# NilanEkanayake/TiTok-Video

Measured on AMD Instinct MI355X. Metric: video clips/sec encode+decode (whole node), higher is better.
Workload: dtype bf16

## Files before the change

### include/titok_hip.h

```cpp
#ifndef TITOK_HIP_H
#define TITOK_HIP_H

#include <stdint.h>

#ifdef __cplusplus
extern "C" {
#endif

#define TTV_OK 0
#define TTV_ERR_INVALID 1
#define TTV_ERR_LAUNCH 2
#define TTV_ERR_UNSUPPORTED 3

#define TTV_BF16 0
#define TTV_F32 1

#define TTV_ENCODER 0
#define TTV_DECODER 1

#define TTV_MAX_FSQ 8
#define TTV_MAX_TOKEN 64
#define TTV_MAX_CLIPS_PER_LAUNCH 64

const char* ttv_error_string(void);
// ... 18 lines not shown
int64_t ttv_vq_workspace_bytes(int rows);
int ttv_vq_l2_argmin(const void* z, int dtype, int ldz, const void* codebook, int ldc, const float* cnorm, int rows, int N, int C,
                     int32_t* indices, float* best_dist, void* workspace, int64_t workspace_bytes, void* stream);
int ttv_vq_lookup(const void* codebook, int dtype, int ldc, const int32_t* indices, int rows, int C, void* codes, int ldo, void* stream);
int ttv_vq_lookup_backward(const void* dcodes, int dtype, int ld, const int32_t* indices, int rows, int C, float* dcodebook, int ldc, void* stream);

int ttv_quant_rows_fp8(const void* in, int dtype, int ld_in, const float* gain, float eps, void* out, int ld_out, float* scales, int rows,
                       int width, void* stream);
int ttv_linear_fp8(const void* xq, int ldx, const float* x_scale, const void* wq, int ldw, const float* w_scale, void* y, int ldy, int M, int N,
                   int K, int epilogue, const float* rope_cs, int d_model, int gqa_dim, void* stream);

int ttv_split3_pack(const float* w, int ldw, void* out, int ldo, int rows, int K, void* stream);
int ttv_linear_split3(const float* x, int ldx, const void* w_image, int ldw, const float* bias, float* y, int ldy, int M, int N, int K, void* stream);

int64_t ttv_mx_scale_bytes_per_row(int width);
int ttv_quant_mx_fp8(const void* in, int dtype, int ld_in, void* out, int ld_out, void* mx, float* row_scales, int rows, int width, void* stream);
int ttv_linear_fp8_mx(const void* xq, int ldx, const void* x_mx, const float* x_row_scale, const void* wq, int ldw, const void* w_mx,
                      const float* w_row_scale, void* y, int ldy, int M, int N, int K, int epilogue, const float* rope_cs, int d_model,
                      int gqa_dim, const void* resid, int ldr, float alpha, void* stream);


int ttv_rmsnorm(const void* in, int in_dtype, int ld_in, const int32_t* src_rows, void* out, int out_dtype, int ld_out,
                const int32_t* dst_rows, const float* gain, int rows, int width, float eps, void* stream);

int ttv_rope_apply(void* x, int dtype, int ld, int rows, int heads, const float* rope_cs, void* stream);

int ttv_linear(const void* x, int ldx, const void* w, int ldw, const void* bias, const float* add_scalar, void* y, int ldy,
               int M, int N, int K, int dtype, void* stream);

int ttv_linear_qkv_rope(const void* x, int ldx, const void* w, int ldw, void* y, int ldy, int M, int d_model, int gqa_dim,
                        const float* rope_cs, int dtype, void* stream);
int ttv_linear_geglu(const void* x, int ldx, const void* w, int ldw, void* y, int ldy, int M, int I, int K, int dtype,
                     void* stream);
int ttv_linear_residual(const void* x, int ldx, const void* w, int ldw, const void* resid, int ldr, float alpha, void* y,
                        int ldy, int y_f32, int M, int N, int K, int dtype, void* stream);

int ttv_linear_residual_norm(const void* x, int ldx, const void* w, int ldw, const void* resid, int ldr, float alpha,
                             const float* gain, float eps, void* y, int ldy, int M, int N, int K, int dtype, void* stream);

int64_t ttv_mlp_pack_bytes(int inner, int next_qkv_rows);
int ttv_mlp_pack(const void* w12_folded, const void* w3, const void* out_proj, const void* next_qkv_folded, int next_qkv_rows, int inner,
                 int width, int dtype, void* mlp_packed, void* stream);
int ttv_mlp_fused(const void* x, int ldx, const void* mlp_packed, int inner, void* y, int ldy, const float* post_gain, float alpha,
                  float eps, int M, int width, int dtype, void* stream);
typedef struct ttv_next_qkv {
  void* qkv; int32_t ld;
  const float* rope_cs;
  int32_t rows;
  int32_t rope_q_end, rope_k_begin, rope_k_end;
} ttv_next_qkv;
int ttv_layer_tail_fused(const void* ao, int ldao, const float* attn_post_gain, float attn_alpha, const void* x, int ldx,
                         const void* mlp_packed, int inner, void* y, int ldy, const float* ffd_post_gain, float ffd_alpha, float eps,
                         int M, int width, int dtype, const ttv_next_qkv* next, void* stream);

int ttv_fill_const_rows(void* x, int dtype, int ld, const int32_t* rows_map, int rows, int width, const float* mask_token,
                        const float* gain, float eps, void* stream);
int ttv_decoder_embed(const void* codes, int token_size, const void* w, const void* bias, const float* mask_token, const float* gain,
                      void* x, int dtype, int ld, const int32_t* rows_map, int rows, int width, float eps, void* stream);

#define TTV_ATTN_GATE 1
#define TTV_ATTN_PAIRED 2
#define TTV_ATTN_QSCALED 4
#define TTV_ATTN_ALLFULL 8
#define TTV_ATTN_PIPE 16
#define TTV_ATTN_SPLIT3 32
#define TTV_ATTN_SPLIT_OUT 64
#define TTV_ATTN_SPLIT_IN 128
int ttv_attention(const void* qkvg, int ld, void* out, int ldo, const int32_t* cu_seqlens, const int32_t* qblocks,
                  int n_qblocks, int q_heads, int kv_heads, int head_dim, int flags, int dtype, void* stream);
int ttv_attention64(const void* qkvg, int ld, void* out, int ldo, const int32_t* cu_seqlens, const int32_t* items, int n_items,
                    int q_heads, int kv_heads, int head_dim, int flags, int dtype, void* stream);

int ttv_patch_gather(const void* const* clips, const int32_t* clip_desc, int clip0, int n_clips, int patch_t, int patch_h,
                     int patch_w, int channels, void* patches, int ld, int dtype, int max_patches_per_clip, void* stream);
int ttv_patch_scatter(const void* patches, int ld, const int32_t* clip_desc, int clip0, int n_clips, int patch_t, int patch_h,
                      int patch_w, int channels, void* const* clips, int dtype, int max_patches_per_clip, void* stream);

typedef struct ttv_tower_dims {
  int32_t kind;
  int32_t dtype;
  int32_t width;
  int32_t layers;
  int32_t q_heads, kv_heads, head_dim;
  int32_t inner;
  int32_t patch_t, patch_h, patch_w;
  int32_t pix_channels;
  int32_t token_size;
  float eps;
  float alpha;
} ttv_tower_dims;

typedef struct ttv_layer_weights {
  const float* pre_ln;
  const void* to_qkv;
  const void* out_proj;
  const float* ffd_norm;
  const void* w12;
  const void* w3;
  const float* attn_post_ln;
  const float* ffd_post_ln;
  const void* to_qkv_pn;
  const void* w12_pn;
  const void* mlp_pack;
  int32_t mlp_pack_qkv_rows;
  int32_t qkv_q_prescaled;
  const void* to_qkv_qs;
// ... 214 lines not shown
  const void* pool_proj_w; const void* pool_proj_b;
  const float* pool_norm2_w; const float* pool_norm2_b;
  const void* pool_fc1_w; const void* pool_fc1_b;
  const void* pool_fc2_w; const void* pool_fc2_b;
} ttv_vjepa_weights;

int ttv_jedi_preprocess(void* const* clips, const int32_t* dims, int n_clips, int dtype, void* out, void* stream);
int64_t ttv_vjepa_workspace_bytes(int n);
int ttv_vjepa_features(const ttv_vjepa_weights* w, const void* x, int n, float* feats, int finetuned, void* workspace,
                       int64_t workspace_bytes, void* stream);

#define TTV_VJEPA_EPI_STORE 0
#define TTV_VJEPA_EPI_GELU 1
#define TTV_VJEPA_EPI_RESID 2
int ttv_vjepa_layernorm(const float* x, int ldx, int rows, int width, const float* w1, const float* b1, float eps1, const float* w2,
                        const float* b2, float eps2, float* y32, int ld32, void* y16, int ld16, void* stream);
int ttv_vjepa_linear(const void* x, int ldx, const void* w, int ldw, const void* bias, int M, int N, int K, int epilogue,
                     const float* resid, int ldr, int resid_rows, void* y, int ldy, void* stream);
int ttv_vjepa_pool_attention(const void* q, const void* kv, int n, int rows, void* out, void* stream);

#define TTV_KC_ATTENTION 1
#define TTV_KC_GEMM_QKV 2
#define TTV_KC_GEMM_GEGLU 3
#define TTV_KC_GEMM_RESID 4
#define TTV_KC_GEMM_STORE 5
#define TTV_KC_RMSNORM 6
#define TTV_KC_PATCH 7
#define TTV_KC_ROWS 8
int ttv_prof_begin(int kernel_class, int max_records);
enum {
  TTV_DBG_NO_STORES = 1,
  TTV_DBG_K256_NO_PANEL_DMA = 2,
  TTV_DBG_MLP_NO_WEIGHT_DMA = 2,
  TTV_DBG_K256_NO_TILE_RELOAD = 4,
  TTV_DBG_MLP_NO_GEGLU = 4,
  TTV_DBG_K256_NO_EPILOGUE_MATH = 8,
  TTV_DBG_MLP_TILES8 = 8,
  TTV_DBG_MLP_NO_P2 = 16,
  TTV_DBG_MLP_PAIRS_ONLY = 32,
  TTV_DBG_MLP_TILES4 = 64,
  TTV_DBG_GEMM_TILE160 = 128,
  TTV_DBG_GEMM_TILE128 = 256,
  TTV_DBG_GEMM_T256 = 512,
  TTV_DBG_MLP_TILES9 = 512,
  TTV_DBG_GEMM_NO_T256 = 1024,
  TTV_DBG_MX_UNFUSED_QUANT = 2048,
  TTV_DBG_SPLIT3_NO_IMAGES = 4096,
  TTV_DBG_SPLIT3_NO_DMA = 8192,
  TTV_DBG_K256_GENERAL = 16384,
  TTV_DBG_QKV256_OFF = 32768,
  TTV_DBG_QKV256_WS = 131072,
  TTV_DBG_ENC_ALL_ROWS = 524288,
  TTV_DBG_ATTN_NO_SWP = 1048576,
  TTV_DBG_DEC_ALL_BLOCKS = 2097152
};
int ttv_debug_set(int flags);
int ttv_debug_stamps(void* device_buffer);
int ttv_prof_end(double* total_ms, int* count);

#ifdef __cplusplus
}
#endif
#endif
```

### titok_video_amd/_lib.py

```python
from __future__ import annotations

import ctypes as C
import os
import threading

import torch

from . import switches

TTV_BF16, TTV_F32 = 0, 1
TTV_ENCODER, TTV_DECODER = 0, 1
TTV_MAX_FSQ = 8
TTV_MAX_TOKEN = 64
TTV_MAX_CLIPS_PER_LAUNCH = 64
TTV_DISC_HEAD_GENERATOR, TTV_DISC_HEAD_DISCRIMINATOR = 0, 1

DBG_NO_STORES = 1
DBG_K256_NO_PANEL_DMA = 2
DBG_MLP_NO_WEIGHT_DMA = 2
DBG_K256_NO_TILE_RELOAD = 4
DBG_MLP_NO_GEGLU = 4
DBG_K256_NO_EPILOGUE_MATH = 8
DBG_MLP_TILES8 = 8
DBG_MLP_NO_P2 = 16
DBG_MLP_PAIRS_ONLY = 32
DBG_MLP_TILES4 = 64
DBG_GEMM_TILE160 = 128
DBG_GEMM_TILE128 = 256
DBG_GEMM_T256 = 512
DBG_MLP_TILES9 = 512
DBG_GEMM_NO_T256 = 1024
DBG_MX_UNFUSED_QUANT = 2048
DBG_SPLIT3_NO_IMAGES = 4096
DBG_SPLIT3_NO_DMA = 8192
DBG_K256_GENERAL = 16384
DBG_QKV256_OFF = 32768
DBG_QKV256_WS = 131072
DBG_ENC_ALL_ROWS = 524288
DBG_ATTN_NO_SWP = 1048576
DBG_DEC_ALL_BLOCKS = 2097152

_HERE = os.path.dirname(os.path.abspath(__file__))
LIB_PATH = switches.text("TTV_LIB_PATH") or os.path.join(_HERE, "libtitok_hip.so")

i32, i64, f32, vp = C.c_int32, C.c_int64, C.c_float, C.c_void_p


class FsqParams(C.Structure):
    _fields_ = [("n", i32), ("levels", i32 * TTV_MAX_FSQ), ("basis", i32 * TTV_MAX_FSQ),
                ("half_l", f32 * TTV_MAX_FSQ), ("offset", f32 * TTV_MAX_FSQ), ("shift", f32 * TTV_MAX_FSQ),
                ("half_width", f32 * TTV_MAX_FSQ)]


class TowerDims(C.Structure):
    _fields_ = [("kind", i32), ("dtype", i32), ("width", i32), ("layers", i32), ("q_heads", i32), ("kv_heads", i32),
                ("head_dim", i32), ("inner", i32), ("patch_t", i32), ("patch_h", i32), ("patch_w", i32),
                ("pix_channels", i32), ("token_size", i32), ("eps", f32), ("alpha", f32)]


class NextQkv(C.Structure):
    _fields_ = [("qkv", vp), ("ld", i32), ("rope_cs", vp), ("rows", i32), ("rope_q_end", i32), ("rope_k_begin", i32), ("rope_k_end", i32)]


class LayerWeights(C.Structure):
    _fields_ = [("pre_ln", vp), ("to_qkv", vp), ("out_proj", vp), ("ffd_norm", vp), ("w12", vp), ("w3", vp),
                ("attn_post_ln", vp), ("ffd_post_ln", vp), ("to_qkv_pn", vp), ("w12_pn", vp), ("mlp_pack", vp), ("mlp_pack_qkv_rows", i32), ("qkv_q_prescaled", i32),
                ("to_qkv_qs", vp), ("to_qkv_f8", vp), ("to_qkv_f8_scale", vp), ("w12_f8", vp), ("w12_f8_scale", vp),
                ("to_qkv_mx", vp), ("w12_mx", vp), ("out_proj_f8", vp), ("out_proj_f8_scale", vp), ("out_proj_mx", vp),
                ("w3_f8", vp), ("w3_f8_scale", vp), ("w3_mx", vp)]


class TowerWeights(C.Structure):
    _fields_ = [("proj_in_w", vp), ("proj_in_b", vp), ("mask_token", vp), ("ln_pre_t", vp), ("ln_pre_p", vp),
                ("ln_post", vp), ("proj_out_w", vp), ("proj_out_b", vp), ("layers", C.POINTER(LayerWeights)), ("proj_out_pn", vp),
                ("f32_split3", i32)]


class Batch(C.Structure):
    _fields_ = [("n_clips", i32), ("total_rows", i32), ("sum_tokens", i32), ("sum_patches", i32),
                ("max_patches_per_clip", i32), ("n_qblocks", i32), ("cu_seqlens", vp), ("latent_rows", vp),
                ("patch_rows", vp), ("clip_desc", vp), ("qblocks", vp), ("rope_cs", vp), ("blocks64", vp), ("row_seq", vp),
                ("n_blocks64", i32), ("qblocks_paired", i32), ("qblocks_all_full", i32), ("items64", vp), ("n_items64", i32),
                ("rope_ids", vp), ("rope_base", vp), ("qblocks_latent", vp), ("n_qblocks_latent", i32), ("qblocks_patch", vp),
                ("n_qblocks_patch", i32)]


class LayerWeightsT(C.Structure):
    _fields_ = [("to_qkv_t", vp), ("out_proj_t", vp), ("w12_t", vp), ("w3_t", vp)]


class TowerWeightsT(C.Structure):
    _fields_ = [("proj_in_t", vp), ("proj_out_t", vp), ("layers", C.POINTER(LayerWeightsT))]

# ... 21 lines not shown


TTV_VJEPA_WIDTH = 1024
TTV_VJEPA_TOKENS = 1568
TTV_VJEPA_PATCH_K = 1536
TTV_VJEPA_EPI_STORE, TTV_VJEPA_EPI_GELU, TTV_VJEPA_EPI_RESID = 0, 1, 2


class VjepaLayer(C.Structure):
    _fields_ = [("norm1_w", vp), ("norm1_b", vp), ("qkv_w", vp), ("qkv_b", vp), ("proj_w", vp), ("proj_b", vp), ("norm2_w", vp),
                ("norm2_b", vp), ("fc1_w", vp), ("fc1_b", vp), ("fc2_w", vp), ("fc2_b", vp)]


class VjepaWeights(C.Structure):
    _fields_ = [("width", i32), ("heads", i32), ("depth", i32), ("patch_w", vp), ("patch_b", vp), ("pos_embed", vp),
                ("layers", C.POINTER(VjepaLayer)), ("norm_w", vp), ("norm_b", vp), ("query_tokens", vp), ("pool_q", vp),
                ("pool_norm1_w", vp), ("pool_norm1_b", vp), ("pool_kv_w", vp), ("pool_kv_b", vp), ("pool_proj_w", vp),
                ("pool_proj_b", vp), ("pool_norm2_w", vp), ("pool_norm2_b", vp), ("pool_fc1_w", vp), ("pool_fc1_b", vp),
                ("pool_fc2_w", vp), ("pool_fc2_b", vp)]


_lib = None
_lock = threading.Lock()

SYMBOLS = {
    "ttv_error_string": (C.c_char_p, []),
    "ttv_version": (C.c_int, []),
    "ttv_fsq_forward": (C.c_int, [C.POINTER(FsqParams), vp, C.c_int, C.c_int, vp, C.c_int, vp, vp, vp]),
    "ttv_fsq_indices_to_codes": (C.c_int, [C.POINTER(FsqParams), vp, C.c_int, vp, C.c_int, vp]),
    "ttv_vq_codebook_norms": (C.c_int, [vp, C.c_int, C.c_int, C.c_int, C.c_int, vp, vp]),
    "ttv_vq_workspace_bytes": (C.c_int64, [C.c_int]),
    "ttv_vq_l2_argmin": (C.c_int, [vp, C.c_int, C.c_int, vp, C.c_int, vp, C.c_int, C.c_int, C.c_int, vp, vp, vp, C.c_int64, vp]),
    "ttv_vq_lookup": (C.c_int, [vp, C.c_int, C.c_int, vp, C.c_int, C.c_int, vp, C.c_int, vp]),
    "ttv_vq_lookup_backward": (C.c_int, [vp, C.c_int, C.c_int, vp, C.c_int, C.c_int, vp, C.c_int, vp]),
    "ttv_quant_rows_fp8": (C.c_int, [vp, C.c_int, C.c_int, vp, f32, vp, C.c_int, vp, C.c_int, C.c_int, vp]),
    "ttv_linear_fp8": (C.c_int, [vp, C.c_int, vp, vp, C.c_int, vp, vp, C.c_int, C.c_int, C.c_int, C.c_int, C.c_int, vp, C.c_int, C.c_int, vp]),
    "ttv_split3_pack": (C.c_int, [vp, C.c_int, vp, C.c_int, C.c_int, C.c_int, vp]),
    "ttv_linear_split3": (C.c_int, [vp, C.c_int, vp, C.c_int, vp, vp, C.c_int, C.c_int, C.c_int, C.c_int, vp]),
    "ttv_mx_scale_bytes_per_row": (C.c_int64, [C.c_int]),
    "ttv_quant_mx_fp8": (C.c_int, [vp, C.c_int, C.c_int, vp, C.c_int, vp, vp, C.c_int, C.c_int, vp]),
    "ttv_linear_fp8_mx": (C.c_int, [vp, C.c_int, vp, vp, vp, C.c_int, vp, vp, vp, C.c_int, C.c_int, C.c_int, C.c_int, C.c_int, vp, C.c_int, C.c_int,
                                    vp, C.c_int, f32, vp]),
    "ttv_rmsnorm": (C.c_int, [vp, C.c_int, C.c_int, vp, vp, C.c_int, C.c_int, vp, vp, C.c_int, C.c_int, f32, vp]),
    "ttv_rope_apply": (C.c_int, [vp, C.c_int, C.c_int, C.c_int, C.c_int, vp, vp]),
    "ttv_linear": (C.c_int, [vp, C.c_int, vp, C.c_int, vp, vp, vp, C.c_int, C.c_int, C.c_int, C.c_int, C.c_int, vp]),
    "ttv_linear_qkv_rope": (C.c_int, [vp, C.c_int, vp, C.c_int, vp, C.c_int, C.c_int, C.c_int, C.c_int, vp, C.c_int, vp]),
    "ttv_linear_geglu": (C.c_int, [vp, C.c_int, vp, C.c_int, vp, C.c_int, C.c_int, C.c_int, C.c_int, C.c_int, vp]),
    "ttv_linear_residual": (C.c_int, [vp, C.c_int, vp, C.c_int, vp, C.c_int, f32, vp, C.c_int, C.c_int, C.c_int, C.c_int,
                                      C.c_int, C.c_int, vp]),
    "ttv_linear_residual_norm": (C.c_int, [vp, C.c_int, vp, C.c_int, vp, C.c_int, f32, vp, f32, vp, C.c_int, C.c_int, C.c_int,
                                           C.c_int, C.c_int, vp]),
    "ttv_mlp_pack_bytes": (C.c_int64, [C.c_int, C.c_int]),
    "ttv_mlp_pack": (C.c_int, [vp, vp, vp, vp, C.c_int, C.c_int, C.c_int, C.c_int, vp, vp]),
    "ttv_layer_tail_fused": (C.c_int, [vp, C.c_int, vp, f32, vp, C.c_int, vp, C.c_int, vp, C.c_int, vp, f32, f32, C.c_int, C.c_int,
                                       C.c_int, vp, vp]),
    "ttv_mlp_fused": (C.c_int, [vp, C.c_int, vp, C.c_int, vp, C.c_int, vp, f32, f32, C.c_int, C.c_int, C.c_int, vp]),
    "ttv_fill_const_rows": (C.c_int, [vp, C.c_int, C.c_int, vp, C.c_int, C.c_int, vp, vp, f32, vp]),
    "ttv_decoder_embed": (C.c_int, [vp, C.c_int, vp, vp, vp, vp, vp, C.c_int, C.c_int, vp, C.c_int, C.c_int, f32, vp]),
    "ttv_attention": (C.c_int, [vp, C.c_int, vp, C.c_int, vp, vp, C.c_int, C.c_int, C.c_int, C.c_int, C.c_int, C.c_int, vp]),
    "ttv_attention64": (C.c_int, [vp, C.c_int, vp, C.c_int, vp, vp, C.c_int, C.c_int, C.c_int, C.c_int, C.c_int, C.c_int, vp]),
    "ttv_patch_gather": (C.c_int, [C.POINTER(vp), vp, C.c_int, C.c_int, C.c_int, C.c_int, C.c_int, C.c_int, vp, C.c_int,
                                   C.c_int, C.c_int, vp]),
    "ttv_patch_scatter": (C.c_int, [vp, C.c_int, vp, C.c_int, C.c_int, C.c_int, C.c_int, C.c_int, C.c_int, C.POINTER(vp),
                                    C.c_int, C.c_int, vp]),
    "ttv_tower_workspace_bytes": (i64, [C.POINTER(TowerDims), C.POINTER(Batch)]),
    "ttv_encoder_forward": (C.c_int, [C.POINTER(TowerDims), C.POINTER(TowerWeights), C.POINTER(Batch), C.POINTER(vp),
                                      C.POINTER(FsqParams), vp, vp, vp, vp, vp, i64, vp]),
    "ttv_decoder_forward": (C.c_int, [C.POINTER(TowerDims), C.POINTER(TowerWeights), C.POINTER(Batch), vp, C.POINTER(vp),
                                      vp, i64, vp]),
    "ttv_tower_tape_bytes": (i64, [C.POINTER(TowerDims), C.POINTER(Batch)]),
    "ttv_tower_bwd_workspace_bytes": (i64, [C.POINTER(TowerDims), C.POINTER(Batch)]),
    "ttv_encoder_forward_train": (C.c_int, [C.POINTER(TowerDims), C.POINTER(TowerWeights), C.POINTER(Batch), C.POINTER(vp), vp, vp,
                                            i64, vp]),
    "ttv_encoder_backward": (C.c_int, [C.POINTER(TowerDims), C.POINTER(TowerWeights), C.POINTER(TowerWeightsT), C.POINTER(Batch), vp,
                                       vp, C.POINTER(TowerGrads), C.POINTER(vp), vp, i64, vp]),
    "ttv_decoder_forward_train": (C.c_int, [C.POINTER(TowerDims), C.POINTER(TowerWeights), C.POINTER(Batch), vp, C.POINTER(vp), vp,
                                            i64, vp, i64, vp]),
    "ttv_decoder_backward": (C.c_int, [C.POINTER(TowerDims), C.POINTER(TowerWeights), C.POINTER(TowerWeightsT), C.POINTER(Batch), vp,
                                       C.POINTER(vp), vp, C.POINTER(TowerGrads), vp, vp, i64, vp]),
    "ttv_fsq_backward": (C.c_int, [C.POINTER(FsqParams), vp, vp, C.c_int, vp, C.c_int, vp]),
    "ttv_rmsnorm_backward_chain": (C.c_int, [vp, C.c_int, vp, C.c_int, vp, vp, vp, C.c_int, vp, C.c_int, vp, vp, C.c_float, vp, C.c_int,
                                              C.c_int, C.c_int, C.c_float, C.c_int, vp]),
    "ttv_opt_grad_sumsq": (C.c_int, [vp, vp, C.c_int, C.c_int, vp, vp]),
    "ttv_opt_adamw_step": (C.c_int, [vp, vp, C.c_int, C.c_int, vp, C.c_int] + [C.c_float] * 8 + [vp, vp]),
    "ttv_opt_param_norms": (C.c_int, [vp, vp, C.c_int, C.c_int, vp, vp, vp]),
    "ttv_linear_wgrad_workspace_bytes": (C.c_int64, [C.c_int, C.c_int, C.c_int]),
    "ttv_linear_wgrad": (C.c_int, [vp, C.c_int, vp, C.c_int, vp, C.c_int, C.c_int, C.c_int, C.c_int, C.c_int, vp, C.c_int64, vp]),
    "ttv_rmsnorm_backward": (C.c_int, [vp, C.c_int, vp, C.c_int, vp, vp, C.c_int, vp, C.c_int, C.c_int, f32, C.c_int, vp]),
    "ttv_attention_backward": (C.c_int, [vp, C.c_int, vp, C.c_int, vp, C.c_int, vp, vp, vp, vp, C.c_int, vp, vp, C.c_int, vp, C.c_int,
                                         C.c_int, C.c_int, C.c_int, vp, vp]),
    "ttv_attention_lse": (C.c_int, [vp, C.c_int, vp, C.c_int, vp, vp, C.c_int, C.c_int, C.c_int, C.c_int, C.c_int, C.c_int, vp, vp]),
    "ttv_codebook_histogram": (C.c_int, [vp, C.c_int, vp, C.c_int, vp]),
    "ttv_rope_table_build": (C.c_int, [vp, vp, C.c_int, C.c_int, vp, vp, vp, vp, C.c_int, vp]),
    "ttv_l1_loss": (C.c_int, [vp, vp, vp, vp, C.c_int, C.c_int, vp, vp]),
    "ttv_clip_from_u8": (C.c_int, [vp, C.c_int, C.c_int, C.c_int, vp, C.c_int, vp]),
    "ttv_clip_resample_u8": (C.c_int, [vp, vp, vp, C.c_int, C.c_int, vp]),
    "ttv_recon_panels_u8": (C.c_int, [vp, vp, vp, C.c_int, C.c_int, vp, vp]),
    "ttv_sq_err_accumulate": (C.c_int, [vp, vp, vp, C.c_int, C.c_int, C.c_int, vp, vp]),
    "ttv_ssim_workspace_bytes": (C.c_int64, [vp, C.c_int]),
    "ttv_ssim_accumulate": (C.c_int, [vp, vp, vp, C.c_int, C.c_int, C.c_int, vp, vp, C.c_int64, vp]),
    "ttv_lpips_tape_bytes": (C.c_int64, [C.c_int, C.c_int, C.c_int, C.c_int]),
    "ttv_lpips_workspace_bytes": (C.c_int64, [C.c_int, C.c_int, C.c_int, C.c_int]),
    "ttv_lpips_forward": (C.c_int, [C.POINTER(LpipsWeights), vp, vp, C.c_int, C.c_int, C.c_int, C.c_int, vp, vp, vp, vp, C.c_int64, vp]),
    "ttv_lpips_backward": (C.c_int, [C.POINTER(LpipsWeights), vp, C.c_int, C.c_int, C.c_int, C.c_int, vp, vp, vp, vp, C.c_int64, vp]),
    "ttv_lpips_conv_workspace_bytes": (C.c_int64, [C.c_int] * 6),
    "ttv_lpips_conv3x3": (C.c_int, [vp, C.c_int, C.c_int, C.c_int, C.c_int, C.c_int, vp, vp, C.c_int, vp, vp, C.c_int, vp, C.c_int64, vp]),
# ... 77 lines not shown
```

### titok_video_amd/csrc/ttv_api.hip

```cpp
#include <stdarg.h>
#include <stdio.h>
#include <stdlib.h>
#include <string.h>

#include "ttv_common.h"
#include "ttv_kernels.h"

static thread_local char g_err[512] = "";

void ttv_set_error(const char* fmt, ...) {
  va_list ap;
  va_start(ap, fmt);
  vsnprintf(g_err, sizeof(g_err), fmt, ap);
  va_end(ap);
}

int g_ttv_prof_class = 0;
bool ttv_sw_enc_latent_last() { static const bool v = ttv_env_flag("TTV_ENC_LATENT_LAST", true); return v; }
bool ttv_sw_keel_f32sum() { static const bool v = ttv_env_flag("TTV_KEEL_F32SUM", false); return v; }
bool ttv_sw_fused_patch() { static const bool v = ttv_env_flag("TTV_FUSED_PATCH", true); return v; }
bool ttv_sw_attn_pipe() { static const bool v = ttv_env_flag("TTV_ATTN_PIPE", false); return v; }
float ttv_sw_attn_thr() { static const float v = ttv_env_float("TTV_ATTN_THR", 8.0f); return v; }
thread_local int g_ttv_debug = 0;
long long* g_ttv_stamps = nullptr;
static hipEvent_t* g_prof_start = nullptr;
static hipEvent_t* g_prof_stop = nullptr;
static int g_prof_cap = 0, g_prof_n = 0;

TtvProfScope::TtvProfScope(int cls, hipStream_t stream) : slot(-1), s(stream) {
  if (g_ttv_prof_class != 0 && cls == g_ttv_prof_class && g_prof_n < g_prof_cap) {
    slot = g_prof_n++;
    (void)hipEventRecord(g_prof_start[slot], s);
  }
}
TtvProfScope::~TtvProfScope() {
  if (slot >= 0) (void)hipEventRecord(g_prof_stop[slot], s);
}

#define TTV_TRY(expr)            \
  do {                           \
    int rc__ = (expr);           \
    if (rc__ != TTV_OK) return rc__; \
  } while (0)

static inline int esize(int dtype) { return dtype == TTV_BF16 ? 2 : 4; }
static inline int64_t align_up(int64_t v) { return (v + 255) & ~(int64_t)255; }

struct TowerWs {
  char *x, *xn, *qkv, *ao, *h, *pa, *pb;
  char *xl, *aol;
  char *f8, *f8mx;
  float* y32;
  float* rstd;
  int64_t total;
};

static TowerWs carve(const ttv_tower_dims* d, const ttv_batch* b, char* base) {
  const int64_t e = esize(d->dtype);
  const int64_t L = b->total_rows, P = b->sum_patches;
  const int64_t g = (int64_t)d->kv_heads * d->head_dim;
  const int64_t pd = (int64_t)d->pix_channels * d->patch_t * d->patch_h * d->patch_w;
  int64_t off = 0;
  TowerWs w;
  auto take = [&](int64_t bytes) { char* p = base ? base + off : nullptr; off += align_up(bytes); return p; };
  w.x = take(L * d->width * e);
  w.xn = take(L * d->width * e);
  w.qkv = take(L * (2 * d->width + 2 * g) * e);
  w.ao = take(L * d->width * e);
  w.y32 = (float*)take(L * d->width * 4);
  w.h = take(L * d->inner * e);
  w.pa = take(P * pd * e);
  w.pb = take(P * d->width * e);
  w.rstd = (float*)take(L * 4);
  w.xl = take((int64_t)b->sum_tokens * d->width * e);
  w.aol = take((int64_t)b->sum_tokens * d->width * e);
  w.f8 = w.f8mx = nullptr;
  if (d->dtype == TTV_BF16 && d->width != 256 && d->width % 128 == 0) {
    const int64_t wide = d->width > d->inner ? d->width : d->inner;
    w.f8 = take(L * wide);
    w.f8mx = take(L * (wide / 128 + 4) * 4);
  }
  w.total = off;
  return w;
}

static int check_dims(const ttv_tower_dims* d, const ttv_batch* b) {
  TTV_CHECK_ARG(d && b, "null dims/batch");
  TTV_CHECK_ARG(d->dtype == TTV_BF16 || d->dtype == TTV_F32, "bad dtype %d", d->dtype);
  TTV_CHECK_ARG(d->head_dim == 64 && d->width == d->q_heads * 64, "width must be q_heads*64");
  TTV_CHECK_ARG(d->width % 64 == 0 && d->width <= 1024, "width %d unsupported", d->width);
  TTV_CHECK_ARG(d->inner % 32 == 0, "GEGLU inner dim must be a multiple of 32");
  TTV_CHECK_ARG(d->token_size >= 1 && d->token_size <= TTV_MAX_TOKEN, "token_size out of range");
  TTV_CHECK_ARG(((int64_t)d->pix_channels * d->patch_t * d->patch_h * d->patch_w) % 8 == 0, "patch vector length must be a multiple of 8");
  TTV_CHECK_ARG(b->n_clips > 0 && b->total_rows == b->sum_tokens + b->sum_patches, "inconsistent batch");
  return TTV_OK;
}

static int run_layer_mx(const ttv_tower_dims* d, const ttv_layer_weights& lw, const ttv_batch* b, const TowerWs& ws, int i, bool& rstd_valid,
                        bool& xq_valid, bool attn_pipe, hipStream_t s) {
  const int L = b->total_rows, dm = d->width, g = d->kv_heads * d->head_dim, dt = d->dtype, nq = 2 * dm + 2 * g, I = d->inner;
  static const bool fused_env = ttv_env_flag("TTV_MX_FUSED_QUANT", true);
  const bool fused_q = fused_env && !(g_ttv_debug & TTV_DBG_MX_UNFUSED_QUANT);
  if (!rstd_valid) TTV_TRY(ttvk_row_rstd(ws.x, dt, dm, ws.rstd, L, dm, d->eps, s));
  if (!xq_valid) TTV_TRY(ttvk_quant_mx_fp8(ws.x, dt, dm, ws.f8, dm, ws.f8mx, nullptr, L, dm, s));
  xq_valid = false;
  GemmArgs a = {};
  a.dtype = dt; a.x = ws.f8; a.ldx = dm; a.w = lw.to_qkv_f8; a.ldw = dm; a.M = L; a.N = nq; a.K = dm; a.y = ws.qkv; a.ldy = nq;
  a.rope_cs = b->rope_cs; a.rope_q_end = dm; a.rope_k_begin = 2 * dm; a.rope_k_end = 2 * dm + g;
  TTV_TRY(ttvk_gemm_fp8(EPI_QKV_ROPE, a, ws.rstd, lw.to_qkv_f8_scale, s, ws.f8mx, lw.to_qkv_mx));
  const bool q_scaled = lw.qkv_q_prescaled != 0;
  if (fused_q && q_scaled && !b->qblocks_paired && !attn_pipe && d->head_dim == 64) {
    TTV_TRY(ttvk_attention_mxout(ws.qkv, nq, ws.f8, ws.f8mx, (int)ttvk_mx_scale_ld(dm), b->cu_seqlens, b->qblocks, b->n_qblocks, d->q_heads,
                                 d->kv_heads, s));
  } else {
    TTV_TRY(ttvk_attention(ws.qkv, nq, ws.ao, dm, b->cu_seqlens, b->qblocks, b->n_qblocks, d->q_heads, d->kv_heads, d->head_dim,
                           TTV_ATTN_GATE | (b->qblocks_paired ? TTV_ATTN_PAIRED : 0) | (q_scaled ? TTV_ATTN_QSCALED : 0) |
                               ((b->qblocks_all_full && attn_pipe) ? TTV_ATTN_ALLFULL : 0) | (attn_pipe ? TTV_ATTN_PIPE : 0), dt, s));
    TTV_TRY(ttvk_quant_mx_fp8(ws.ao, dt, dm, ws.f8, dm, ws.f8mx, nullptr, L, dm, s));
  }
  GemmArgs o = {};
  o.dtype = dt; o.x = ws.f8; o.ldx = dm; o.w = lw.out_proj_f8; o.ldw = dm; o.M = L; o.N = dm; o.K = dm; o.resid = ws.x; o.ldr = dm;
  o.alpha = i == 0 ? 1.f : d->alpha; o.y = ws.x; o.ldy = dm;
  TTV_TRY(ttvk_gemm_fp8(EPI_RESID_T, o, nullptr, lw.out_proj_f8_scale, s, ws.f8mx, lw.out_proj_mx));
  if (i > 0) {
    TTV_TRY(ttvk_rmsnorm(ws.x, dt, dm, nullptr, ws.x, dt, dm, nullptr, lw.attn_post_ln, L, dm, d->eps, s, ws.rstd, fused_q ? ws.f8 : nullptr,
                         fused_q ? ws.f8mx : nullptr));
    if (!fused_q) TTV_TRY(ttvk_quant_mx_fp8(ws.x, dt, dm, ws.f8, dm, ws.f8mx, nullptr, L, dm, s));
  } else {
    TTV_TRY(ttvk_row_rstd(ws.x, dt, dm, ws.rstd, L, dm, d->eps, s));
    TTV_TRY(ttvk_quant_mx_fp8(ws.x, dt, dm, ws.f8, dm, ws.f8mx, nullptr, L, dm, s));
  }
  GemmArgs f = {};
  f.dtype = dt; f.x = ws.f8; f.ldx = dm; f.w = lw.w12_f8; f.ldw = dm; f.M = L; f.N = I; f.K = dm; f.y = ws.h; f.ldy = I;
  char* const hq = ws.h;
  char* const hq_mx = ws.xn;
  const bool h_fused = fused_q && (int64_t)ttvk_mx_scale_ld(I) <= (int64_t)dm * 2;
  if (h_fused) { f.yq = hq; f.yq_mx = hq_mx; }
  TTV_TRY(ttvk_gemm_fp8(EPI_GEGLU, f, ws.rstd, lw.w12_f8_scale, s, ws.f8mx, lw.w12_mx));
  GemmArgs f3 = {};
  if (h_fused) {
    f3.x = hq;
  } else {
    TTV_TRY(ttvk_quant_mx_fp8(ws.h, dt, I, ws.f8, I, ws.f8mx, nullptr, L, I, s));
    f3.x = ws.f8;
  }
  f3.dtype = dt; f3.ldx = I; f3.w = lw.w3_f8; f3.ldw = I; f3.M = L; f3.N = dm; f3.K = I; f3.resid = ws.x; f3.ldr = dm;
  f3.alpha = i == 0 ? 1.f : d->alpha; f3.y = ws.x; f3.ldy = dm;
  TTV_TRY(ttvk_gemm_fp8(EPI_RESID_T, f3, nullptr, lw.w3_f8_scale, s, h_fused ? hq_mx : ws.f8mx, lw.w3_mx));
  rstd_valid = false;
  if (i > 0) {
    TTV_TRY(ttvk_rmsnorm(ws.x, dt, dm, nullptr, ws.x, dt, dm, nullptr, lw.ffd_post_ln, L, dm, d->eps, s, ws.rstd, fused_q ? ws.f8 : nullptr,
                         fused_q ? ws.f8mx : nullptr));
    rstd_valid = true;
    xq_valid = fused_q;
  }
  return TTV_OK;
}

static bool rows_f8(int dt, int dm, const void* img, const void* row_scale, const void* mx, const void* folded) {
  return dt == TTV_BF16 && img && row_scale && !mx && dm % 128 == 0 && !(dm == 256 && folded);
}

struct LayerCtx {
  const ttv_tower_dims* d; const ttv_batch* b; const TowerWs& ws; hipStream_t s;
  int split3, s3img;
  bool gen_ok;
};

struct PreNormW { const float* gain; const void *w, *w_pn, *w_f8; const float* w_f8_scale; bool f8; };

static int prenorm_proj(const LayerCtx& c, GemmEpilogue epi, const char* x, int rows, const PreNormW& p, int N, char* y, int y_image,
                        bool rstd_valid) {
  const ttv_tower_dims* d = c.d;
  const TowerWs& ws = c.ws;
  const int dm = d->width, dt = d->dtype;
  GemmArgs a = {};
  a.dtype = dt; a.ldx = dm; a.ldw = dm; a.M = rows; a.N = N; a.K = dm; a.y = y; a.ldy = N;
  if (epi == EPI_QKV_ROPE) {
    a.rope_cs = c.b->rope_cs; a.rope_q_end = dm; a.rope_k_begin = 2 * dm; a.rope_k_end = 2 * dm + d->kv_heads * d->head_dim;
  }
  if (p.f8) {
    float* const f8_scales = reinterpret_cast<float*>(ws.xn + (((size_t)c.b->total_rows * dm + 255) & ~(size_t)255));
    TTV_TRY(ttvk_quant_rows_fp8(x, dt, dm, p.gain, d->eps, ws.xn, dm, f8_scales, rows, dm, c.s));
    a.x = ws.xn; a.w = p.w_f8;
    return ttvk_gemm_fp8(epi, a, f8_scales, p.w_f8_scale, c.s);
  }
  const bool fold256 = dt == TTV_BF16 && dm == 256 && p.w_pn;
  const bool fold_gen = c.gen_ok && p.w_pn;
  const bool fold = fold256 || fold_gen;
  if (fold_gen && !rstd_valid) TTV_TRY(ttvk_row_rstd(x, dt, dm, ws.rstd, rows, dm, d->eps, c.s));
  if (!fold) TTV_TRY(ttvk_rmsnorm(x, dt, dm, nullptr, ws.xn, dt, dm, nullptr, p.gain, rows, dm, d->eps, c.s, nullptr, nullptr, nullptr, c.s3img));
  a.split3 = c.split3; a.x_image = c.s3img && !fold; a.y_image = y_image;
  a.prenorm = fold256; a.eps = d->eps;
  a.row_scale = fold_gen ? ws.rstd : nullptr;
  a.x = fold ? x : ws.xn; a.w = fold ? p.w_pn : p.w;
  if (epi == EPI_QKV_ROPE) { a.rope_ids = c.b->rope_ids; a.rope_base = c.b->rope_ids ? c.b->rope_base : nullptr; }
  return ttvk_gemm(epi, a, c.s);
}

static int keel_tail(const LayerCtx& c, GemmArgs o, int layer, const float* post_gain, char* cx, bool want_rstd, bool& rstd_valid) {
  const ttv_tower_dims* d = c.d;
  const int dm = d->width, dt = d->dtype;
  static const bool keel_f32sum = ttv_sw_keel_f32sum();
  o.alpha = layer == 0 ? 1.f : d->alpha; o.y = cx; o.ldy = dm;
  if (layer == 0) return ttvk_gemm(EPI_RESID_T, o, c.s);
  if (ttvk_gemm_supports_resid_norm(dt, dm, o.K)) {
    o.norm_gain = post_gain; o.eps = d->eps;
    return ttvk_gemm(EPI_RESID_NORM, o, c.s);
  }
  float* const next_rstd = want_rstd ? c.ws.rstd : nullptr;
  if (dt == TTV_BF16 && !keel_f32sum) {
    TTV_TRY(ttvk_gemm(EPI_RESID_T, o, c.s));
    TTV_TRY(ttvk_rmsnorm(cx, dt, dm, nullptr, cx, dt, dm, nullptr, post_gain, o.M, dm, d->eps, c.s, next_rstd));
  } else {
    o.y = c.ws.y32;
    TTV_TRY(ttvk_gemm(EPI_RESID_F32, o, c.s));
    TTV_TRY(ttvk_rmsnorm(c.ws.y32, TTV_F32, dm, nullptr, cx, dt, dm, nullptr, post_gain, o.M, dm, d->eps, c.s, next_rstd));
  }
  rstd_valid = want_rstd;
  return TTV_OK;
}

static int run_layers(const ttv_tower_dims* d, const ttv_tower_weights* w, const ttv_batch* b, const TowerWs& ws, hipStream_t s) {
  const int L = b->total_rows, dm = d->width, g = d->kv_heads * d->head_dim, dt = d->dtype;
  const int split3 = (dt == TTV_F32 && w->f32_split3) ? 1 : 0;
  const bool gen_ok = (dt == TTV_BF16 && dm != 256) || split3;
  static const bool s3img_env = ttv_env_flag("TTV_SPLIT3_IMAGES", true);
  const int s3img = (split3 && s3img_env && !(g_ttv_debug & TTV_DBG_SPLIT3_NO_IMAGES)) ? 1 : 0;
  const int nq = 2 * dm + 2 * g;
  bool qkv_ready = false;
  bool rstd_valid = false;
  bool xq_valid = false;
  static const bool attn_pipe = ttv_sw_attn_pipe();
  static const bool lat_env = ttv_sw_enc_latent_last();
  const bool lat_last = lat_env && !(g_ttv_debug & TTV_DBG_ENC_ALL_ROWS) && d->kind == TTV_ENCODER && b->qblocks_latent && b->n_qblocks_latent > 0 &&
                        b->latent_rows && b->sum_tokens > 0 && b->sum_tokens < L;
  static const bool pat_env = ttv_env_flag("TTV_DEC_PATCH_LAST", true);
  const bool pat_last = pat_env && !(g_ttv_debug & TTV_DBG_DEC_ALL_BLOCKS) && d->kind == TTV_DECODER && d->layers >= 2 && b->qblocks_patch &&
                        b->n_qblocks_patch > 0 && !split3 && !b->qblocks_paired;
  bool compacted = false;
  const LayerCtx ctx = {d, b, ws, s, split3, s3img, gen_ok};
  for (int i = 0; i < d->layers; ++i) {
    const ttv_layer_weights& lw = w->layers[i];
    static const bool keel_f32 = ttv_sw_keel_f32sum();
    if (dt == TTV_BF16 && dm != 256 && dm % 128 == 0 && d->inner % 128 == 0 && !keel_f32 && lw.to_qkv_f8 && lw.to_qkv_mx && lw.w12_f8 && lw.w12_mx &&
        lw.out_proj_f8 && lw.out_proj_mx && lw.w3_f8 && lw.w3_mx &&
        !(lat_last && i == d->layers - 1)) {
      TTV_TRY(run_layer_mx(d, lw, b, ws, i, rstd_valid, xq_valid, attn_pipe, s));
      qkv_ready = false;
      continue;
    }
    xq_valid = false;
    const bool f8_qkv = rows_f8(dt, dm, lw.to_qkv_f8, lw.to_qkv_f8_scale, lw.to_qkv_mx, lw.to_qkv_pn);
    const bool f8_w12 = rows_f8(dt, dm, lw.w12_f8, lw.w12_f8_scale, lw.w12_mx, lw.w12_pn);
    if (!qkv_ready) {
      const void* w_plain = (dt == TTV_BF16 && lw.to_qkv_qs) ? lw.to_qkv_qs : lw.to_qkv;
      const PreNormW qw = {lw.pre_ln, w_plain, lw.to_qkv_pn, lw.to_qkv_f8, lw.to_qkv_f8_scale, f8_qkv};
      TTV_TRY(prenorm_proj(ctx, EPI_QKV_ROPE, ws.x, L, qw, nq, ws.qkv, s3img ? 2 : 0, rstd_valid));
    }
    const bool q_scaled = dt == TTV_BF16 && (lw.to_qkv_pn ? lw.qkv_q_prescaled != 0 : lw.to_qkv_qs != nullptr);
    rstd_valid = false;
    qkv_ready = false;
    const bool lat_now = lat_last && i == d->layers - 1;
    if (lat_now)
      TTV_TRY(ttvk_attention(ws.qkv, nq, ws.ao, dm, b->cu_seqlens, b->qblocks_latent, b->n_qblocks_latent, d->q_heads, d->kv_heads, d->head_dim,
                             TTV_ATTN_GATE | (b->qblocks_all_full ? TTV_ATTN_ALLFULL : 0) | (q_scaled ? TTV_ATTN_QSCALED : 0) | (split3 ? TTV_ATTN_SPLIT3 : 0) |
                                 (s3img ? (TTV_ATTN_SPLIT_OUT | TTV_ATTN_SPLIT_IN) : 0), dt, s));
    else if (pat_last && i == d->layers - 1 && dt == TTV_BF16 && !attn_pipe)
      TTV_TRY(ttvk_attention(ws.qkv, nq, ws.ao, dm, b->cu_seqlens, b->qblocks_patch, b->n_qblocks_patch, d->q_heads, d->kv_heads, d->head_dim,
                             TTV_ATTN_GATE | (b->qblocks_all_full ? TTV_ATTN_ALLFULL : 0) | (q_scaled ? TTV_ATTN_QSCALED : 0), dt, s));
    else if (q_scaled && b->items64 && b->n_items64 > 0 && d->head_dim == 64)
      TTV_TRY(ttvk_attention64(ws.qkv, nq, ws.ao, dm, b->cu_seqlens, b->items64, b->n_items64, d->q_heads, d->kv_heads,
                               TTV_ATTN_GATE | TTV_ATTN_QSCALED, s));
    else
    TTV_TRY(ttvk_attention(ws.qkv, nq, ws.ao, dm, b->cu_seqlens, b->qblocks, b->n_qblocks, d->q_heads, d->kv_heads, d->head_dim,
                           TTV_ATTN_GATE | (b->qblocks_paired ? TTV_ATTN_PAIRED : 0) | (q_scaled ? TTV_ATTN_QSCALED : 0) |
                               (b->qblocks_all_full ? TTV_ATTN_ALLFULL : 0) | (attn_pipe ? TTV_ATTN_PIPE : 0) | (split3 ? TTV_ATTN_SPLIT3 : 0) |
                               (s3img ? (TTV_ATTN_SPLIT_OUT | TTV_ATTN_SPLIT_IN) : 0), dt, s));
    char* cx = ws.x;
    char* cao = ws.ao;
    int Lc = L;
    if (lat_now) {
      const int64_t rb = (int64_t)dm * esize(dt);
      TTV_TRY(ttvk_copy_rows(ws.x, (int64_t)dm * esize(dt), b->latent_rows, ws.xl, (int64_t)dm * esize(dt), nullptr, b->sum_tokens, dm * (int)esize(dt), s));
      TTV_TRY(ttvk_copy_rows(ws.ao, rb, b->latent_rows, ws.aol, rb, nullptr, b->sum_tokens, (int)rb, s));
      cx = ws.xl; cao = ws.aol; Lc = b->sum_tokens;
      compacted = true;
    }
    static const bool use_fused_mlp = ttv_env_flag("TTV_FUSED_MLP", true);
    static const bool use_fused_qkv = ttv_env_flag("TTV_FUSED_QKV", false);
    if (use_fused_mlp && ttvk_mlp_fused_supported(dt, dm, d->inner) && lw.mlp_pack) {
      MlpNextQkv nx = {};
      const bool back = use_fused_qkv && i + 1 < d->layers && lw.mlp_pack_qkv_rows == nq && nq % 64 == 0 && dm % 64 == 0 && g % 64 == 0;
      if (back) { nx.qkv = ws.qkv; nx.ld = nq; nx.rope_cs = b->rope_cs; nx.rows = nq; nx.rope_q_end = dm; nx.rope_k_begin = 2 * dm; nx.rope_k_end = 2 * dm + g; }
      TTV_TRY(ttvk_mlp_fused(cao, dm, i == 0 ? nullptr : lw.attn_post_ln, i == 0 ? 1.f : d->alpha, cx, dm, lw.mlp_pack, d->inner,
                             cx, dm, i == 0 ? nullptr : lw.ffd_post_ln, i == 0 ? 1.f : d->alpha, d->eps, Lc, back ? &nx : nullptr, s));
      qkv_ready = back;
      continue;
    }
    GemmArgs o = {};
    o.dtype = dt; o.split3 = split3; o.x_image = s3img;
    o.x = cao; o.ldx = dm; o.w = lw.out_proj; o.ldw = dm; o.M = Lc; o.N = dm; o.K = dm; o.resid = cx; o.ldr = dm;
    TTV_TRY(keel_tail(ctx, o, i, lw.attn_post_ln, cx, gen_ok && lw.w12_pn && !f8_w12, rstd_valid));
    const PreNormW fw = {lw.ffd_norm, lw.w12, lw.w12_pn, lw.w12_f8, lw.w12_f8_scale, f8_w12};
    TTV_TRY(prenorm_proj(ctx, EPI_GEGLU, cx, Lc, fw, d->inner, ws.h, s3img, rstd_valid));
    rstd_valid = false;
    GemmArgs f3 = {};
    f3.dtype = dt; f3.split3 = split3; f3.x_image = s3img;
    f3.x = ws.h; f3.ldx = d->inner; f3.w = lw.w3; f3.ldw = d->inner; f3.M = Lc; f3.N = dm; f3.K = d->inner; f3.resid = cx; f3.ldr = dm;
    const bool next_rstd = gen_ok && i + 1 < d->layers && w->layers[i + 1].to_qkv_pn &&
                           !rows_f8(dt, dm, w->layers[i + 1].to_qkv_f8, w->layers[i + 1].to_qkv_f8_scale, w->layers[i + 1].to_qkv_mx, w->layers[i + 1].to_qkv_pn);
    TTV_TRY(keel_tail(ctx, f3, i, lw.ffd_post_ln, cx, next_rstd, rstd_valid));
  }
  if (compacted)
    TTV_TRY(ttvk_copy_rows(ws.xl, (int64_t)dm * esize(dt), nullptr, ws.x, (int64_t)dm * esize(dt), b->latent_rows, b->sum_tokens, dm * (int)esize(dt), s));
  return TTV_OK;
}

extern "C" {

const char* ttv_error_string(void) { return g_err; }
int ttv_version(void) { return 100; }

int ttv_fsq_forward(const ttv_fsq_params* p, const void* z, int z_dtype, int rows, void* codes, int codes_dtype, int32_t* indices,
                    float* bounded, void* stream) {
  TTV_CHECK_ARG(rows >= 0 && (rows == 0 || (z && codes && indices)), "fsq_forward: null buffer");
  return ttvk_fsq_forward(p, z, z_dtype, rows, codes, codes_dtype, indices, bounded, (hipStream_t)stream);
}

int ttv_fsq_indices_to_codes(const ttv_fsq_params* p, const int32_t* indices, int rows, void* codes, int codes_dtype, void* stream) {
  TTV_CHECK_ARG(rows >= 0 && (rows == 0 || (indices && codes)), "fsq_indices_to_codes: null buffer");
  return ttvk_fsq_indices_to_codes(p, indices, rows, codes, codes_dtype, (hipStream_t)stream);
}

int ttv_vq_codebook_norms(const void* codebook, int dtype, int ld, int N, int C, float* cnorm, void* stream) {
  TTV_CHECK_ARG(N == 0 || (codebook && cnorm), "vq_codebook_norms: null buffer");
  return ttvk_vq_norms(codebook, dtype, ld, N, C, cnorm, (hipStream_t)stream);
}

int64_t ttv_vq_workspace_bytes(int rows) { return ttvk_vq_workspace_bytes(rows); }

int ttv_vq_l2_argmin(const void* z, int dtype, int ldz, const void* codebook, int ldc, const float* cnorm, int rows, int N, int C,
                     int32_t* indices, float* best_dist, void* workspace, int64_t workspace_bytes, void* stream) {
  TTV_CHECK_ARG(rows == 0 || (z && codebook && cnorm && indices), "vq_l2_argmin: null buffer");
  TTV_CHECK_ARG(ldz >= C && ldc >= C, "vq_l2_argmin: leading dims smaller than the codebook dim");
  return ttvk_vq_l2_argmin(z, dtype, ldz, codebook, ldc, cnorm, rows, N, C, indices, best_dist, workspace, workspace_bytes, (hipStream_t)stream);
}

int ttv_vq_lookup(const void* codebook, int dtype, int ldc, const int32_t* indices, int rows, int C, void* codes, int ldo, void* stream) {
// ... 42 lines not shown
  a.dtype = TTV_BF16; a.x = xq; a.ldx = ldx; a.w = wq; a.ldw = ldw; a.M = M; a.N = N; a.K = K; a.y = y; a.ldy = ldy;
  if (epilogue == 1) {
    TTV_CHECK_ARG(rope_cs && N == 2 * d_model + 2 * gqa_dim, "linear_fp8_mx: qkv epilogue needs rope_cs and N = 2 d_model + 2 gqa_dim");
    a.rope_cs = rope_cs; a.rope_q_end = d_model; a.rope_k_begin = 2 * d_model; a.rope_k_end = 2 * d_model + gqa_dim;
  }
  if (epilogue == 3) { a.resid = resid; a.ldr = ldr; a.alpha = alpha; }
  return ttvk_gemm_fp8(epilogue == 0 ? EPI_STORE : epilogue == 1 ? EPI_QKV_ROPE : epilogue == 2 ? EPI_GEGLU : EPI_RESID_T, a, x_row_scale,
                       w_row_scale, (hipStream_t)stream, x_mx, w_mx);
}

int ttv_linear_fp8(const void* xq, int ldx, const float* x_scale, const void* wq, int ldw, const float* w_scale, void* y, int ldy, int M, int N,
                   int K, int epilogue, const float* rope_cs, int d_model, int gqa_dim, void* stream) {
  TTV_CHECK_ARG(M == 0 || (xq && wq && y), "linear_fp8: null buffer");
  TTV_CHECK_ARG(epilogue >= 0 && epilogue <= 2, "linear_fp8: epilogue 0 (store), 1 (qkv + rotary) or 2 (GEGLU)");
  GemmArgs a = {};
  a.dtype = TTV_BF16; a.x = xq; a.ldx = ldx; a.w = wq; a.ldw = ldw; a.M = M; a.N = N; a.K = K; a.y = y; a.ldy = ldy;
  if (epilogue == 1) {
    TTV_CHECK_ARG(rope_cs && N == 2 * d_model + 2 * gqa_dim, "linear_fp8: qkv epilogue needs rope_cs and N = 2 d_model + 2 gqa_dim");
    a.rope_cs = rope_cs; a.rope_q_end = d_model; a.rope_k_begin = 2 * d_model; a.rope_k_end = 2 * d_model + gqa_dim;
  }
  return ttvk_gemm_fp8(epilogue == 0 ? EPI_STORE : epilogue == 1 ? EPI_QKV_ROPE : EPI_GEGLU, a, x_scale, w_scale, (hipStream_t)stream);
}

int ttv_rmsnorm(const void* in, int in_dtype, int ld_in, const int32_t* src_rows, void* out, int out_dtype, int ld_out,
                const int32_t* dst_rows, const float* gain, int rows, int width, float eps, void* stream) {
  TTV_CHECK_ARG(rows >= 0 && (rows == 0 || (in && out && gain)), "rmsnorm: null buffer");
  return ttvk_rmsnorm(in, in_dtype, ld_in, src_rows, out, out_dtype, ld_out, dst_rows, gain, rows, width, eps, (hipStream_t)stream);
}

int ttv_rope_apply(void* x, int dtype, int ld, int rows, int heads, const float* rope_cs, void* stream) {
  TTV_CHECK_ARG(rows == 0 || (x && rope_cs), "rope_apply: null buffer");
  TTV_CHECK_ARG(ld % 4 == 0 && ld >= heads * 64, "rope_apply: bad leading dim");
  return ttvk_rope_apply(x, dtype, ld, rows, heads, rope_cs, (hipStream_t)stream);
}

int ttv_linear(const void* x, int ldx, const void* w, int ldw, const void* bias, const float* add_scalar, void* y, int ldy, int M,
               int N, int K, int dtype, void* stream) {
  TTV_CHECK_ARG(M == 0 || (x && w && y), "linear: null buffer");
  GemmArgs a = {};
  a.dtype = dtype; a.x = x; a.ldx = ldx; a.w = w; a.ldw = ldw; a.M = M; a.N = N; a.K = K; a.y = y; a.ldy = ldy;
  a.bias = bias; a.add_scalar = add_scalar;
  return ttvk_gemm(EPI_STORE, a, (hipStream_t)stream);
}

int ttv_linear_qkv_rope(const void* x, int ldx, const void* w, int ldw, void* y, int ldy, int M, int d_model, int gqa_dim,
                        const float* rope_cs, int dtype, void* stream) {
  TTV_CHECK_ARG(M == 0 || (x && w && y && rope_cs), "linear_qkv_rope: null buffer");
  GemmArgs a = {};
  a.dtype = dtype; a.x = x; a.ldx = ldx; a.w = w; a.ldw = ldw; a.M = M; a.N = 2 * d_model + 2 * gqa_dim; a.K = d_model;
  a.y = y; a.ldy = ldy; a.rope_cs = rope_cs; a.rope_q_end = d_model; a.rope_k_begin = 2 * d_model; a.rope_k_end = 2 * d_model + gqa_dim;
  return ttvk_gemm(EPI_QKV_ROPE, a, (hipStream_t)stream);
}

int ttv_linear_geglu(const void* x, int ldx, const void* w, int ldw, void* y, int ldy, int M, int I, int K, int dtype, void* stream) {
  TTV_CHECK_ARG(M == 0 || (x && w && y), "linear_geglu: null buffer");
  GemmArgs a = {};
  a.dtype = dtype; a.x = x; a.ldx = ldx; a.w = w; a.ldw = ldw; a.M = M; a.N = I; a.K = K; a.y = y; a.ldy = ldy;
  return ttvk_gemm(EPI_GEGLU, a, (hipStream_t)stream);
}

int ttv_linear_residual(const void* x, int ldx, const void* w, int ldw, const void* resid, int ldr, float alpha, void* y, int ldy,
                        int y_f32, int M, int N, int K, int dtype, void* stream) {
  TTV_CHECK_ARG(M == 0 || (x && w && y && resid), "linear_residual: null buffer");
  GemmArgs a = {};
  a.dtype = dtype; a.x = x; a.ldx = ldx; a.w = w; a.ldw = ldw; a.M = M; a.N = N; a.K = K; a.y = y; a.ldy = ldy;
  a.resid = resid; a.ldr = ldr; a.alpha = alpha;
  return ttvk_gemm(y_f32 ? EPI_RESID_F32 : EPI_RESID_T, a, (hipStream_t)stream);
}

int ttv_linear_residual_norm(const void* x, int ldx, const void* w, int ldw, const void* resid, int ldr, float alpha,
                             const float* gain, float eps, void* y, int ldy, int M, int N, int K, int dtype, void* stream) {
  TTV_CHECK_ARG(M == 0 || (x && w && y && resid && gain), "linear_residual_norm: null buffer");
  GemmArgs a = {};
  a.dtype = dtype; a.x = x; a.ldx = ldx; a.w = w; a.ldw = ldw; a.M = M; a.N = N; a.K = K; a.y = y; a.ldy = ldy;
  a.resid = resid; a.ldr = ldr; a.alpha = alpha; a.norm_gain = gain; a.eps = eps;
  if (!ttvk_gemm_supports_resid_norm(dtype, N, K)) {
    ttv_set_error("linear_residual_norm: only bf16 with N == 256 has a fused kernel");
    return TTV_ERR_UNSUPPORTED;
  }
  return ttvk_gemm(EPI_RESID_NORM, a, (hipStream_t)stream);
}

int64_t ttv_mlp_pack_bytes(int inner, int next_qkv_rows) { return ttvk_mlp_pack_bytes(inner, next_qkv_rows); }

int ttv_mlp_pack(const void* w12_folded, const void* w3, const void* out_proj, const void* next_qkv_folded, int next_qkv_rows, int inner,
                 int width, int dtype, void* packed, void* stream) {
  if (!ttvk_mlp_fused_supported(dtype, width, inner)) {
    ttv_set_error("mlp_pack: only bf16, width 256, inner %% 32 == 0");
    return TTV_ERR_UNSUPPORTED;
  }
  return ttvk_mlp_pack(w12_folded, w3, out_proj, next_qkv_folded, next_qkv_rows, inner, packed, (hipStream_t)stream);
}

int ttv_mlp_fused(const void* x, int ldx, const void* mlp_packed, int inner, void* y, int ldy, const float* post_gain, float alpha,
                  float eps, int M, int width, int dtype, void* stream) {
  if (!ttvk_mlp_fused_supported(dtype, width, inner)) {
    ttv_set_error("mlp_fused: only bf16, width 256, inner %% 32 == 0");
    return TTV_ERR_UNSUPPORTED;
  }
  return ttvk_mlp_fused(nullptr, 0, nullptr, 1.f, x, ldx, mlp_packed, inner, y, ldy, post_gain, alpha, eps, M, nullptr, (hipStream_t)stream);
}

int ttv_layer_tail_fused(const void* ao, int ldao, const float* attn_post_gain, float attn_alpha, const void* x, int ldx,
                         const void* mlp_packed, int inner, void* y, int ldy, const float* ffd_post_gain, float ffd_alpha, float eps,
                         int M, int width, int dtype, const ttv_next_qkv* next, void* stream) {
  if (!ttvk_mlp_fused_supported(dtype, width, inner)) {
    ttv_set_error("layer_tail_fused: only bf16, width 256, inner %% 32 == 0");
    return TTV_ERR_UNSUPPORTED;
  }
  TTV_CHECK_ARG(ao, "layer_tail_fused: null attention output");
  MlpNextQkv nx = {};
  if (next) { nx.qkv = next->qkv; nx.ld = next->ld; nx.rope_cs = next->rope_cs; nx.rows = next->rows; nx.rope_q_end = next->rope_q_end;
              nx.rope_k_begin = next->rope_k_begin; nx.rope_k_end = next->rope_k_end; }
  return ttvk_mlp_fused(ao, ldao, attn_post_gain, attn_alpha, x, ldx, mlp_packed, inner, y, ldy, ffd_post_gain, ffd_alpha, eps, M,
                        next ? &nx : nullptr, (hipStream_t)stream);
}

int ttv_fill_const_rows(void* x, int dtype, int ld, const int32_t* rows_map, int rows, int width, const float* mask_token,
                        const float* gain, float eps, void* stream) {
  TTV_CHECK_ARG(rows == 0 || (x && rows_map && mask_token && gain), "fill_const_rows: null buffer");
  return ttvk_fill_const_rows(x, dtype, ld, rows_map, rows, width, mask_token, gain, eps, (hipStream_t)stream);
}

int ttv_decoder_embed(const void* codes, int token_size, const void* w, const void* bias, const float* mask_token, const float* gain,
                      void* x, int dtype, int ld, const int32_t* rows_map, int rows, int width, float eps, void* stream) {
  TTV_CHECK_ARG(rows == 0 || (codes && w && bias && mask_token && gain && x && rows_map), "decoder_embed: null buffer");
  return ttvk_dec_embed(codes, token_size, w, bias, mask_token, gain, x, dtype, ld, rows_map, rows, width, eps, (hipStream_t)stream);
}

int ttv_attention(const void* qkvg, int ld, void* out, int ldo, const int32_t* cu_seqlens, const int32_t* qblocks, int n_qblocks,
                  int q_heads, int kv_heads, int head_dim, int flags, int dtype, void* stream) {
  TTV_CHECK_ARG(n_qblocks == 0 || (qkvg && out && cu_seqlens && qblocks), "attention: null buffer");
  return ttvk_attention(qkvg, ld, out, ldo, cu_seqlens, qblocks, n_qblocks, q_heads, kv_heads, head_dim, flags, dtype, (hipStream_t)stream);
}
int ttv_attention64(const void* qkvg, int ld, void* out, int ldo, const int32_t* cu_seqlens, const int32_t* items, int n_items, int q_heads,
                    int kv_heads, int head_dim, int flags, int dtype, void* stream) {
  TTV_CHECK_ARG(dtype == TTV_BF16 && head_dim == 64, "attention64: bf16, head_dim 64 only");
  return ttvk_attention64(qkvg, ld, out, ldo, cu_seqlens, items, n_items, q_heads, kv_heads, flags, (hipStream_t)stream);
}

int ttv_patch_gather(const void* const* clips, const int32_t* clip_desc, int clip0, int n_clips, int patch_t, int patch_h, int patch_w,
                     int channels, void* patches, int ld, int dtype, int max_patches_per_clip, void* stream) {
  TTV_CHECK_ARG(n_clips == 0 || (clips && clip_desc && patches), "patch_gather: null buffer");
  return ttvk_patch_copy(false, (void* const*)clips, clip_desc, clip0, n_clips, patch_t, patch_h, patch_w, channels, patches, ld, dtype, max_patches_per_clip, (hipStream_t)stream);
}

int ttv_patch_scatter(const void* patches, int ld, const int32_t* clip_desc, int clip0, int n_clips, int patch_t, int patch_h, int patch_w,
                      int channels, void* const* clips, int dtype, int max_patches_per_clip, void* stream) {
  TTV_CHECK_ARG(n_clips == 0 || (clips && clip_desc && patches), "patch_scatter: null buffer");
  return ttvk_patch_copy(true, clips, clip_desc, clip0, n_clips, patch_t, patch_h, patch_w, channels, (void*)patches, ld, dtype, max_patches_per_clip, (hipStream_t)stream);
}

int64_t ttv_tower_workspace_bytes(const ttv_tower_dims* dims, const ttv_batch* batch) {
  if (check_dims(dims, batch) != TTV_OK) return -1;
  return carve(dims, batch, nullptr).total;
}

int ttv_encoder_forward(const ttv_tower_dims* d, const ttv_tower_weights* w, const ttv_batch* b, const void* const* clips,
                        const ttv_fsq_params* fsq, float* z, void* codes, int32_t* indices, float* bounded, void* workspace,
                        int64_t workspace_bytes, void* stream) {
  TTV_TRY(check_dims(d, b));
  TTV_CHECK_ARG(d->kind == TTV_ENCODER, "encoder_forward: dims.kind is not TTV_ENCODER");
  TTV_CHECK_ARG(w && w->layers && clips && workspace, "encoder_forward: null argument");
  TTV_CHECK_ARG(fsq || z, "encoder_forward: neither fsq nor z requested");
  TTV_CHECK_ARG(!fsq || (codes && indices), "encoder_forward: fsq needs codes and indices buffers");
  hipStream_t s = (hipStream_t)stream;
  TowerWs ws = carve(d, b, (char*)workspace);
  TTV_CHECK_ARG(ws.total <= workspace_bytes, "encoder_forward: workspace too small (%lld < %lld)", (long long)workspace_bytes, (long long)ws.total);
// ... 260 lines not shown
```

### titok_video_amd/csrc/ttv_common.h

```cpp
#pragma once
#include <hip/hip_runtime.h>
#include <stdint.h>
#include <stdlib.h>

#include "../../include/titok_hip.h"

typedef __bf16 bf16_t;
typedef __attribute__((ext_vector_type(8))) __bf16 bf16x8;
typedef __attribute__((ext_vector_type(4))) __bf16 bf16x4;
typedef __attribute__((ext_vector_type(2))) __bf16 bf16x2;
typedef __attribute__((ext_vector_type(4))) float f32x4;
typedef __attribute__((ext_vector_type(16))) float f32x16;

#define TTV_WAVE 64

void ttv_set_error(const char* fmt, ...);
#define TTV_CHECK_ARG(cond, ...)          \
  do {                                    \
    if (!(cond)) {                        \
      ttv_set_error(__VA_ARGS__);         \
      return TTV_ERR_INVALID;             \
    }                                     \
  } while (0)
#define TTV_CHECK_LAUNCH(what)                                            \
// ... 101 lines not shown
  return __uint_as_float(b0) + __uint_as_float(b1);
}
__device__ __forceinline__ float quad16_max(float v) {
  const unsigned u = __float_as_uint(v);
  const auto a = __builtin_amdgcn_permlane16_swap(u, u, false, false);
  const unsigned a0 = a[0], a1 = a[1];
  const float s = fmaxf(__uint_as_float(a0), __uint_as_float(a1));
  const unsigned t = __float_as_uint(s);
  const auto b = __builtin_amdgcn_permlane32_swap(t, t, false, false);
  const unsigned b0 = b[0], b1 = b[1];
  return fmaxf(__uint_as_float(b0), __uint_as_float(b1));
}
__device__ __forceinline__ float pair32_sum(float v) {
  const unsigned u = __float_as_uint(v);
  const auto b = __builtin_amdgcn_permlane32_swap(u, u, false, false);
  const unsigned b0 = b[0], b1 = b[1];
  return __uint_as_float(b0) + __uint_as_float(b1);
}
__device__ __forceinline__ uint4 xchg16_pair(uint2 p0, uint2 p1) {
  const auto x = __builtin_amdgcn_permlane16_swap(p0.x, p1.x, false, false);
  const auto y = __builtin_amdgcn_permlane16_swap(p0.y, p1.y, false, false);
  const unsigned x0 = x[0], x1 = x[1], y0 = y[0], y1 = y[1];
  return make_uint4(x0, y0, x1, y1);
}

extern int g_ttv_prof_class;
extern thread_local int g_ttv_debug;
extern long long* g_ttv_stamps;
struct TtvProfScope {
  int slot;
  hipStream_t s;
  TtvProfScope(int cls, hipStream_t stream);
  ~TtvProfScope();
};

static inline int ttv_cdiv(int a, int b) { return (a + b - 1) / b; }

static inline bool ttv_env_flag(const char* name, bool default_on) {
  const char* v = getenv(name);
  return default_on ? !(v && v[0] == '0') : (v && v[0] == '1');
}
static inline int ttv_env_int(const char* name, int dflt) {
  const char* v = getenv(name);
  return v ? atoi(v) : dflt;
}
static inline float ttv_env_float(const char* name, float dflt) {
  const char* v = getenv(name);
  return v ? (float)atof(v) : dflt;
}
bool ttv_sw_enc_latent_last();
bool ttv_sw_keel_f32sum();
bool ttv_sw_fused_patch();
bool ttv_sw_attn_pipe();
float ttv_sw_attn_thr();

__device__ __forceinline__ float ttv_cubic_src(int dst, float scale) { return fmaf(scale, (float)dst + 0.5f, -0.5f); }
__device__ __forceinline__ int ttv_cubic_floor(int dst, float scale) { return (int)floorf(ttv_cubic_src(dst, scale)); }
__device__ __forceinline__ void cubic_taps(int dst, int n_in, int n_out, int (&idx)[4], float (&w)[4]) {
  const float scale = (float)n_in / (float)n_out;
  const float src = ttv_cubic_src(dst, scale);
  const float fl = floorf(src);
  const float t = src - fl;
  const int i0 = (int)fl;
  constexpr float A = -0.75f;
  auto c1 = [](float x) { return ((A + 2.f) * x - (A + 3.f)) * x * x + 1.f; };
  auto c2 = [](float x) { return ((A * x - 5.f * A) * x + 8.f * A) * x - 4.f * A; };
  w[0] = c2(t + 1.f); w[1] = c1(t); w[2] = c1(1.f - t); w[3] = c2(2.f - t);
#pragma unroll
  for (int k = 0; k < 4; ++k) {
    const int j = i0 - 1 + k;
    idx[k] = j < 0 ? 0 : (j > n_in - 1 ? n_in - 1 : j);
  }
}
typedef float f32x2 __attribute__((ext_vector_type(2)));
__device__ __forceinline__ float geglu_fast(float g, float x) {
  const float gc = __builtin_amdgcn_fmed3f(g, -8.0f, 8.0f);
  const float g2 = gc * gc;
  float q = fmaf(g2, 1.014262858e-03f, -1.067757308e-01f);
  q = fmaf(q, g2, -2.301121361e+00f);
  const float e = __builtin_amdgcn_exp2f(q * gc);
  return (g * __builtin_amdgcn_rcpf(1.0f + e)) * x;
}
__device__ __forceinline__ f32x2 geglu_pair_fast(f32x2 g, f32x2 x) { return (f32x2){geglu_fast(g.x, x.x), geglu_fast(g.y, x.y)}; }

__device__ __forceinline__ void geglu_fast8(const float (&g)[8], const float (&x)[8], float (&h)[8]) {
  float a[8], e[8];
#pragma unroll
  for (int k = 0; k < 8; ++k) {
    const float gc = __builtin_amdgcn_fmed3f(g[k], -8.0f, 8.0f);
    const float g2 = gc * gc;
    float q = fmaf(g2, 1.014262858e-03f, -1.067757308e-01f);
    q = fmaf(q, g2, -2.301121361e+00f);
    a[k] = q * gc;
  }
  __builtin_amdgcn_sched_barrier(0);
#pragma unroll
  for (int k = 0; k < 8; ++k) e[k] = __builtin_amdgcn_exp2f(a[k]);
  __builtin_amdgcn_sched_barrier(0);
#pragma unroll
  for (int k = 0; k < 8; ++k) e[k] = 1.0f + e[k];
  __builtin_amdgcn_sched_barrier(0);
#pragma unroll
  for (int k = 0; k < 8; ++k) e[k] = __builtin_amdgcn_rcpf(e[k]);
  __builtin_amdgcn_sched_barrier(0);
#pragma unroll
  for (int k = 0; k < 8; ++k) h[k] = (g[k] * e[k]) * x[k];
// ... 2 lines not shown
```

### titok_video_amd/csrc/ttv_gemm.hip

```cpp
#include <stdlib.h>

#include "ttv_common.h"
#include "ttv_kernels.h"

struct GemmDev {
  const void* x; const void* w; void* y;
  const void* bias; const float* add_scalar; const void* resid; const float* rope_cs;
  int ldx, ldw, ldy, ldr;
  int M, N, K;
  int w_rows;
  float alpha;
  int rope_q_end, rope_k_begin, rope_k_end;
  float eps;
  int debug;
  const float* norm_gain;
  ClipPtrs clips;
  const int* clip_desc; const int* patch_rows; const int* row_seq;
  const int* x_rows;
  const float* row_scale;
  const int* rope_ids; const float* rope_base;
  const float* x_scale; const float* w_scale;
  float* sum_f32; int ld_sum;
  void* y2; int ldy2; const float* norm_gain2;
  int split3;
  int x_image, y_image;
  const uint8_t* x_mx; const uint8_t* w_mx;
  int ld_mx;
  uint8_t* yq; uint8_t* yq_mx; int ld_yq_mx, yq_nkp;
  int clip0, pt_shift, ph_shift;
  long long* stamps;
  int resid_rows;
};

struct PatchDst {
  bf16_t* base;
  int thw, hw, w;
};

__device__ __forceinline__ float gelu_erf(float v) { return 0.5f * v * (1.0f + erff(v * 0.70710678118654752440f)); }
__device__ __forceinline__ float gelu_erf_as(float v) {
  const float x = fabsf(v) * 0.70710678118654752440f;
  const float t = __builtin_amdgcn_rcpf(fmaf(0.3275911f, x, 1.0f));
  const float poly = t * fmaf(t, fmaf(t, fmaf(t, fmaf(t, 1.061405429f, -1.453152027f), 1.421413741f), -0.284496736f), 0.254829592f);
  const float e = __builtin_amdgcn_exp2f(x * x * -1.44269504088896340736f);
  const float erf_abs = fmaf(-poly, e, 1.0f);
  return 0.5f * v * (1.0f + __builtin_copysignf(erf_abs, v));
}

__device__ __forceinline__ uint2 pack_bf16x4(f32x4 v) {
  bf16x4 b = {(bf16_t)v[0], (bf16_t)v[1], (bf16_t)v[2], (bf16_t)v[3]};
  return __builtin_bit_cast(uint2, b);
}

__device__ __forceinline__ uint4 split4_bf16(uint4 v) {
  const float x0 = __uint_as_float(v.x), x1 = __uint_as_float(v.y), x2 = __uint_as_float(v.z), x3 = __uint_as_float(v.w);
  const bf16_t h0 = (bf16_t)x0, h1 = (bf16_t)x1, h2 = (bf16_t)x2, h3 = (bf16_t)x3;
  const bf16_t l0 = (bf16_t)(x0 - (float)h0), l1 = (bf16_t)(x1 - (float)h1), l2 = (bf16_t)(x2 - (float)h2), l3 = (bf16_t)(x3 - (float)h3);
  const bf16x4 hv = {h0, h1, h2, h3}, lv = {l0, l1, l2, l3};
  const uint2 hp = __builtin_bit_cast(uint2, hv), lp = __builtin_bit_cast(uint2, lv);
  return make_uint4(hp.x, hp.y, lp.x, lp.y);
}

template <int EPI, typename T, int NI, int NJ>
__device__ __forceinline__ void epilogue_tile(const GemmDev& p, const int (&tok)[NJ], const int (&feat)[NI],
                                              f32x4 (&acc)[NI][NJ], f32x4 (&acc2)[NI][NJ], int kq, const PatchDst* pd = nullptr) {
  if (p.debug & TTV_DBG_NO_STORES) {
#pragma unroll
    for (int i = 0; i < NI; ++i)
#pragma unroll
      for (int j = 0; j < NJ; ++j) asm volatile("" ::"v"(acc[i][j][0]), "v"(acc[i][j][3]), "v"(acc2[i][j][1]));
    return;
  }
  int tc[NJ], fc[NI];
  bool tv[NJ], fv[NI];
#pragma unroll
  for (int j = 0; j < NJ; ++j) { tv[j] = tok[j] < p.M; tc[j] = tv[j] ? tok[j] : p.M - 1; }
#pragma unroll
  for (int i = 0; i < NI; ++i) { fv[i] = feat[i] < p.N; fc[i] = fv[i] ? feat[i] : p.N - 4; }

  if (p.row_scale) {
#pragma unroll
    for (int j = 0; j < NJ; ++j) {
      const float rs = p.row_scale[tc[j]];
#pragma unroll
// ... 1735 lines not shown
#pragma unroll
  for (int j = 0; j < NJ; ++j) tok[j] = tbase + wt * (16 * NJ) + j * 16 + l15;
  if (DUAL) {
    int feat[2];
    f32x4 ax[2][NJ], ag[2][NJ];
#pragma unroll
    for (int i = 0; i < 2; ++i) {
      feat[i] = fbase + wf * 32 + i * 16 + kq * 4;
#pragma unroll
      for (int j = 0; j < NJ; ++j) { ax[i][j] = acc[i][j]; ag[i][j] = acc[i + 2][j]; }
    }
    epilogue_tile<EPI, float, 2, NJ>(p, tok, feat, ax, ag, kq);
  } else {
    int feat[4];
#pragma unroll
    for (int i = 0; i < 4; ++i) feat[i] = fbase + wf * 64 + i * 16 + kq * 4;
    epilogue_tile<EPI, float, 4, NJ>(p, tok, feat, acc, acc, kq);
  }
}

static int gemm_token_tile(int M, int nf, int debug) {
  if (debug & TTV_DBG_GEMM_TILE160) return 160;
  if (debug & TTV_DBG_GEMM_TILE128) return 128;
  const long cost128 = (long)ttv_cdiv(nf * ttv_cdiv(M, 128), 512) * 128, cost160 = (long)ttv_cdiv(nf * ttv_cdiv(M, 160), 512) * 160;
  return cost160 < cost128 ? 160 : 128;
}

template <int EPI>
static int launch(const GemmDev& d, int dtype, bool prenorm, hipStream_t s) {
  if (dtype == TTV_BF16 && d.K == 256 && d.N % 8 == 0 && !((d.debug & TTV_DBG_K256_GENERAL) && !prenorm && EPI != EPI_STORE_PATCH)) {
    const int fo = (EPI == EPI_GEGLU) ? 32 : 64;
    const int n_panels = ttv_cdiv(d.N, fo), n_tiles = ttv_cdiv(d.M, K256_TT);
    const int total = n_panels * n_tiles;
    static const int grid_env = ttv_env_int("TTV_K256_GRID", 0);
    int grid = total < 512 ? total : 512;
    if (grid_env > 0) grid = total < grid_env ? total : grid_env;
    else if (total > 512)
      for (int g = 512; g >= 416; --g)
        if (total % g == 0) { grid = g; break; }
    static const int qkv256_env = ttv_env_int("TTV_QKV256", 1);
    if constexpr (EPI == EPI_QKV_ROPE) {
      const int n_groups = (n_panels + 3) / 4;
      if (qkv256_env && !(d.debug & TTV_DBG_QKV256_OFF) && d.N % 64 == 0 && d.rope_q_end % 64 == 0 && d.rope_k_begin % 64 == 0 && d.rope_k_end % 64 == 0 &&
          !d.row_scale && !d.bias && !d.add_scalar && (uint64_t)d.w_rows * (uint64_t)d.ldw * 2u < (1ull << 32)) {
        if ((qkv256_env >= 2 || (d.debug & TTV_DBG_QKV256_WS)) && n_groups <= 32) {
          const int tgs = ttv_cdiv(d.M, 32), per_xcd = ttv_cdiv(tgs, 8);
          int q = n_groups * ttv_cdiv(per_xcd, 8);
          q = q > 32 ? 32 : q;
          if (prenorm) hipLaunchKernelGGL((k_qkv256ws<true>), dim3(8 * q), dim3(512), 0, s, d, n_panels, n_groups);
          else hipLaunchKernelGGL((k_qkv256ws<false>), dim3(8 * q), dim3(512), 0, s, d, n_panels, n_groups);
          TTV_CHECK_LAUNCH("qkv256ws");
          return TTV_OK;
        }
        if (prenorm) hipLaunchKernelGGL((k_qkv256<true>), dim3(grid), dim3(256), 0, s, d, n_panels, total);
        else hipLaunchKernelGGL((k_qkv256<false>), dim3(grid), dim3(256), 0, s, d, n_panels, total);
        TTV_CHECK_LAUNCH("qkv256");
        return TTV_OK;
      }
    }
    if (prenorm) hipLaunchKernelGGL((k_gemm_k256<EPI, true>), dim3(grid), dim3(256), 0, s, d, n_panels, total);
    else hipLaunchKernelGGL((k_gemm_k256<EPI, false>), dim3(grid), dim3(256), 0, s, d, n_panels, total);
    TTV_CHECK_LAUNCH("gemm_k256");
    return TTV_OK;
  }
  if (prenorm || EPI == EPI_STORE_PATCH) {
    ttv_set_error("gemm: folded pre-norm / patch scatter need the bf16 K=256 kernel");
    return TTV_ERR_UNSUPPORTED;
  }
  if (dtype == TTV_BF16) {
    const int ft = (EPI == EPI_GEGLU) ? 64 : TF;
    const int nf = ttv_cdiv(d.N, ft), nt = ttv_cdiv(d.M, TT), nt160 = ttv_cdiv(d.M, 160);
    const bool t160 = gemm_token_tile(d.M, nf, d.debug) == 160;
    static const bool use_dma = ttv_env_flag("TTV_GEMM_DMA", true);
    const bool dma_ok = use_dma && d.K % BK == 0 && (uint64_t)d.M * (uint64_t)d.ldx * 2u < (1ull << 32) && (uint64_t)d.w_rows * (uint64_t)d.ldw * 2u < (1ull << 32);
    static const int t256_env = ttv_env_int("TTV_GEMM_T256", -1);
    if constexpr (EPI == EPI_STORE || EPI == EPI_QKV_ROPE || EPI == EPI_GEGLU || EPI == EPI_RESID_T || EPI == EPI_RESID_F32) {
      const int fo = (EPI == EPI_GEGLU) ? 128 : T256_F;
      const long tiles256 = (long)ttv_cdiv(d.N, fo) * ttv_cdiv(d.M, T256_T);
      const bool forced = (d.debug & TTV_DBG_GEMM_T256) || t256_env == 1;
      const bool ok256 = dma_ok && d.N % fo == 0 && d.K >= 2 * BK && !(d.debug & TTV_DBG_GEMM_NO_T256) && (forced || tiles256 >= 256);
      if (ok256 && (forced || (t256_env < 0 && T256_DEFAULT))) {
        hipLaunchKernelGGL((k_gemm_bf16_t256<EPI>), dim3((unsigned)tiles256), dim3(512), 0, s, d, ttv_cdiv(d.N, fo));
        TTV_CHECK_LAUNCH("gemm_t256");
        return TTV_OK;
      }
    }
    if (t160) {
      if (dma_ok) hipLaunchKernelGGL((k_gemm_bf16_dma<EPI, 5>), dim3(nf * nt160), dim3(256), 0, s, d, nf);
      else hipLaunchKernelGGL((k_gemm_bf16<EPI, false, 5>), dim3(nf * nt160), dim3(256), 0, s, d, nf);
    } else {
      if (dma_ok) hipLaunchKernelGGL((k_gemm_bf16_dma<EPI, 4>), dim3(nf * nt), dim3(256), 0, s, d, nf);
      else hipLaunchKernelGGL((k_gemm_bf16<EPI>), dim3(nf * nt), dim3(256), 0, s, d, nf);
    }
  } else {
    if ((uint64_t)d.M * (uint64_t)d.ldx >= (1ull << 31) || (uint64_t)d.w_rows * (uint64_t)d.ldw >= (1ull << 31)) {
      ttv_set_error("gemm (fp32): operand too large for 32-bit element offsets");
      return TTV_ERR_UNSUPPORTED;
    }
    const int nf = ttv_cdiv(d.N, (EPI == EPI_GEGLU) ? 64 : F_TF), nt = ttv_cdiv(d.M, F_TT), nt160 = ttv_cdiv(d.M, 160);
    const bool t160 = gemm_token_tile(d.M, nf, d.debug) == 160;
    static const bool s3dma_env = ttv_env_flag("TTV_SPLIT3_DMA", true);
    const bool s3dma = d.split3 && d.x_image && s3dma_env && !(d.debug & TTV_DBG_SPLIT3_NO_DMA) && d.K % 32 == 0 && d.ldx % 4 == 0 && d.ldw % 4 == 0 &&
                       (uint64_t)d.M * (uint64_t)d.ldx * 4u < (1ull << 32) && (uint64_t)d.w_rows * (uint64_t)d.ldw * 4u < (1ull << 32);
    if (s3dma) {
      if (t160) hipLaunchKernelGGL((k_gemm_split_dma<EPI, 5>), dim3(nf * nt160), dim3(256), 0, s, d, nf);
      else hipLaunchKernelGGL((k_gemm_split_dma<EPI, 4>), dim3(nf * nt), dim3(256), 0, s, d, nf);
    } else if (d.split3) {
      if (t160) hipLaunchKernelGGL((k_gemm_f32<EPI, true, 5>), dim3(nf * nt160), dim3(256), 0, s, d, nf);
// ... 35 lines not shown
    TTV_CHECK_ARG(mx && epi == EPI_GEGLU && a.yq_mx && a.N % 128 == 0 && (uintptr_t)a.yq % 4 == 0, "gemm_fp8: the fp8 GEGLU output needs block-scaled operands, its scale buffer and N %% 128 == 0");
    d.yq = (uint8_t*)a.yq; d.yq_mx = (uint8_t*)a.yq_mx; d.yq_nkp = (a.N / 128 + 3) / 4 * 4; d.ld_yq_mx = 4 * d.yq_nkp;
  }
  if (epi == EPI_QKV_ROPE) TTV_CHECK_ARG(a.rope_cs && a.rope_q_end % 128 == 0 && a.rope_k_begin % 128 == 0 && a.rope_k_end % 128 == 0, "gemm_fp8: rotary ranges must be multiples of 128 columns");
  const int ft = (epi == EPI_GEGLU) ? 64 : TF;
  const int nf = ttv_cdiv(d.N, ft), nt = ttv_cdiv(d.M, TT), nt160 = ttv_cdiv(d.M, 160);
  const bool t160 = gemm_token_tile(d.M, nf, 0) == 160;
  const int kc = epi == EPI_STORE ? TTV_KC_GEMM_STORE : epi == EPI_QKV_ROPE ? TTV_KC_GEMM_QKV : epi == EPI_GEGLU ? TTV_KC_GEMM_GEGLU : TTV_KC_GEMM_RESID;
  TtvProfScope prof(kc, s);
#define F8_LAUNCH(E_, MX_)                                                                                         \
  do {                                                                                                              \
    if (t160) hipLaunchKernelGGL((k_gemm_fp8_dma<E_, 5, MX_>), dim3(nf * nt160), dim3(256), 0, s, d, nf);           \
    else hipLaunchKernelGGL((k_gemm_fp8_dma<E_, 4, MX_>), dim3(nf * nt), dim3(256), 0, s, d, nf);                   \
  } while (0)
  if (mx) {
    if (epi == EPI_STORE) F8_LAUNCH(EPI_STORE, true); else if (epi == EPI_QKV_ROPE) F8_LAUNCH(EPI_QKV_ROPE, true);
    else if (epi == EPI_GEGLU) F8_LAUNCH(EPI_GEGLU, true); else F8_LAUNCH(EPI_RESID_T, true);
  } else {
    if (epi == EPI_STORE) F8_LAUNCH(EPI_STORE, false); else if (epi == EPI_QKV_ROPE) F8_LAUNCH(EPI_QKV_ROPE, false); else F8_LAUNCH(EPI_GEGLU, false);
  }
#undef F8_LAUNCH
  TTV_CHECK_LAUNCH("gemm_fp8");
  return TTV_OK;
}

bool ttvk_gemm_supports_resid_norm(int dtype, int N, int K) { return dtype == TTV_BF16 && N == 256 && K % 8 == 0; }

int ttvk_gemm(GemmEpilogue epi, const GemmArgs& a, hipStream_t s) {
  if (a.M == 0 || a.N == 0) return TTV_OK;
  const int esz = a.dtype == TTV_BF16 ? 2 : 4;
  const int vec = 16 / esz;
  TTV_CHECK_ARG(a.dtype == TTV_BF16 || a.dtype == TTV_F32, "gemm: bad dtype %d", a.dtype);
  TTV_CHECK_ARG(a.K > 0 && a.K % vec == 0, "gemm: K=%d must be a multiple of %d", a.K, vec);
  TTV_CHECK_ARG(a.N % 4 == 0, "gemm: N=%d must be a multiple of 4", a.N);
  TTV_CHECK_ARG(a.ldx % vec == 0 && a.ldw % vec == 0 && a.ldy % vec == 0, "gemm: leading dims must keep 16-byte row alignment");
  TTV_CHECK_ARG(((uintptr_t)a.x % 16 == 0) && ((uintptr_t)a.w % 16 == 0) && ((uintptr_t)a.y % 16 == 0), "gemm: pointers must be 16-byte aligned");
  GemmDev d;
  d.x = a.x; d.w = a.w; d.y = a.y; d.bias = a.bias; d.add_scalar = a.add_scalar; d.resid = a.resid; d.rope_cs = a.rope_cs; d.rope_ids = a.rope_ids; d.rope_base = a.rope_base;
  d.ldx = a.ldx; d.ldw = a.ldw; d.ldy = a.ldy; d.ldr = a.ldr;
  d.M = a.M; d.N = a.N; d.K = a.K; d.alpha = a.alpha;
  d.w_rows = (epi == EPI_GEGLU) ? 2 * a.N : a.N;
  d.rope_q_end = a.rope_q_end; d.rope_k_begin = a.rope_k_begin; d.rope_k_end = a.rope_k_end;
  d.eps = a.eps;
  d.debug = g_ttv_debug;
  d.sum_f32 = a.sum_f32; d.ld_sum = a.ld_sum; d.y2 = a.y2; d.ldy2 = a.ldy2; d.norm_gain2 = a.norm_gain2;
  d.split3 = (a.split3 && a.dtype == TTV_F32) ? 1 : 0;
  d.x_image = d.split3 && a.x_image; d.y_image = d.split3 ? a.y_image : 0;
  TTV_CHECK_ARG(!d.y_image || (d.y_image == 1 && (epi == EPI_STORE || epi == EPI_GEGLU)) || (d.y_image == 2 && epi == EPI_QKV_ROPE),
                "gemm: a split-image output is a STORE / GEGLU option (y_image 1) or the to_qkv layout (y_image 2)");
  d.x_mx = d.w_mx = nullptr; d.ld_mx = 0;
  d.norm_gain = a.norm_gain;
  d.clip_desc = a.clip_desc; d.patch_rows = a.patch_rows; d.row_seq = a.row_seq; d.clip0 = 0; d.pt_shift = d.ph_shift = 0;
  d.x_rows = a.x_rows;
  d.x_scale = nullptr; d.w_scale = nullptr;
  d.row_scale = a.row_scale;
  d.stamps = g_ttv_stamps;
  d.resid_rows = a.resid_rows;
  TTV_CHECK_ARG(!a.row_scale || ((a.dtype == TTV_BF16 || a.split3) && (epi == EPI_STORE || epi == EPI_QKV_ROPE || epi == EPI_GEGLU)),
                "gemm: row_scale is a STORE / QKV_ROPE / GEGLU option of the bf16 and the split-bf16 kernels");
  TTV_CHECK_ARG(!a.x_rows || (a.dtype == TTV_BF16 && a.K == 256 && a.N % 8 == 0 && epi != EPI_RESID_NORM), "gemm: x_rows needs the bf16 K=256 kernel");
  if (epi == EPI_STORE_PATCH || a.gather) {
    auto lg2 = [](int v) { int s = 0; while ((1 << s) < v) ++s; return (1 << s) == v ? s : -1; };
    TTV_CHECK_ARG(a.dtype == TTV_BF16 && (a.gather || a.K == 256) && a.patch_w == 8 && lg2(a.patch_t) >= 0 && lg2(a.patch_h) >= 0,
                  "gemm: patch gather/scatter needs bf16, patch_w == 8 and power-of-two patch_t / patch_h (scatter: K == 256)");
    TTV_CHECK_ARG(!a.gather || (epi == EPI_STORE && a.K % 64 == 0 && a.K != 256), "gemm: patch gather is an EPI_STORE option of the general-K kernel");
    TTV_CHECK_ARG(a.clips && a.n_clips > 0 && a.n_clips <= TTV_MAX_CLIPS_PER_LAUNCH && a.clip_desc && a.patch_rows && a.row_seq,
                  "gemm: patch scatter needs clips (<= %d), clip_desc, patch_rows and row_seq", TTV_MAX_CLIPS_PER_LAUNCH);
    for (int i = 0; i < a.n_clips; ++i) d.clips.p[i] = a.clips[i];
    d.pt_shift = lg2(a.patch_t); d.ph_shift = lg2(a.patch_h);
  }
  const bool pn = a.prenorm != 0;
  const int kc = (epi == EPI_STORE || epi == EPI_STORE_PATCH) ? TTV_KC_GEMM_STORE : epi == EPI_QKV_ROPE ? TTV_KC_GEMM_QKV : epi == EPI_GEGLU ? TTV_KC_GEMM_GEGLU : TTV_KC_GEMM_RESID;
  TtvProfScope prof(kc, s);
  switch (epi) {
    case EPI_STORE:
      if (a.gather) {
        const int nf = ttv_cdiv(d.N, TF), nt = ttv_cdiv(d.M, TT), nt160 = ttv_cdiv(d.M, 160);
        if (gemm_token_tile(d.M, nf, d.debug) == 160)
          hipLaunchKernelGGL((k_gemm_bf16<EPI_STORE, true, 5>), dim3(nf * nt160), dim3(256), 0, s, d, nf);
        else
          hipLaunchKernelGGL((k_gemm_bf16<EPI_STORE, true>), dim3(nf * nt), dim3(256), 0, s, d, nf);
        TTV_CHECK_LAUNCH("gemm_gather");
        return TTV_OK;
      }
      return launch<EPI_STORE>(d, a.dtype, pn, s);
    case EPI_STORE_PATCH: return launch<EPI_STORE_PATCH>(d, a.dtype, pn, s);
    case EPI_QKV_ROPE:
      TTV_CHECK_ARG(a.rope_cs && a.rope_q_end % 128 == 0 && a.rope_k_begin % 128 == 0 && a.rope_k_end % 128 == 0, "gemm: rotary ranges must be multiples of 128 columns");
      return launch<EPI_QKV_ROPE>(d, a.dtype, pn, s);
    case EPI_GEGLU: return launch<EPI_GEGLU>(d, a.dtype, pn, s);
    case EPI_RESID_T:
      TTV_CHECK_ARG(a.resid && a.ldr % 4 == 0, "gemm: residual missing");
      return launch<EPI_RESID_T>(d, a.dtype, pn, s);
    case EPI_RESID_F32:
      TTV_CHECK_ARG(a.resid && a.ldr % 4 == 0, "gemm: residual missing");
      return launch<EPI_RESID_F32>(d, a.dtype, pn, s);
    case EPI_BIAS_PLAIN:
    case EPI_BIAS_GELU:
    case EPI_BIAS_RESID_F32R: {
      TTV_CHECK_ARG(a.dtype == TTV_BF16 && a.K % BK == 0 && a.bias && (uintptr_t)a.bias % 8 == 0, "gemm: V-JEPA epilogues need bf16, K %% 64 == 0 and a bias");
      TTV_CHECK_ARG(!a.add_scalar && !a.row_scale, "gemm: V-JEPA epilogues take no scalar / row scale");
      TTV_CHECK_ARG(epi != EPI_BIAS_RESID_F32R || (a.resid && a.ldr % 4 == 0 && (uintptr_t)a.resid % 16 == 0 && a.resid_rows >= 0),
                    "gemm: fp32 residual missing or unaligned");
      TTV_CHECK_ARG((uint64_t)a.M * (uint64_t)a.ldx * 2u < (1ull << 32) && (uint64_t)a.N * (uint64_t)a.ldw * 2u < (1ull << 32),
                    "gemm: operand too large for 32-bit byte offsets");
      if (d.N % T256_F == 0 && d.K >= 2 * BK) {
// ... 35 lines not shown
```

### titok_video_amd/csrc/ttv_kernels.h

```cpp
#pragma once
#include <hip/hip_runtime.h>
#include <stdint.h>

#include "../../include/titok_hip.h"

int ttvk_rmsnorm(const void* in, int in_dtype, int ld_in, const int* src_rows, void* out, int out_dtype, int ld_out,
                 const int* dst_rows, const float* gain, int rows, int d, float eps, hipStream_t s, float* next_rstd = nullptr,
                 void* mx_q = nullptr, void* mx_s = nullptr,
                 int split_image = 0);
int ttvk_row_rstd(const void* in, int dtype, int ld_in, float* rstd, int rows, int d, float eps, hipStream_t s);
int ttvk_copy_rows(const void* src, int64_t ld_src_bytes, const int* src_rows, void* dst, int64_t ld_dst_bytes, const int* dst_rows, int rows,
                   int row_bytes, hipStream_t s);
int ttvk_fill_const_rows(void* x, int dtype, int ld, const int* rows_map, int rows, int d, const float* mask_token,
                         const float* gain, float eps, hipStream_t s);
int ttvk_dec_embed(const void* codes, int C, const void* w, const void* bias, const float* mask_token, const float* gain,
                   void* x, int dtype, int ld, const int* rows_map, int rows, int d, float eps, hipStream_t s);
int ttvk_fsq_forward(const ttv_fsq_params* p, const void* z, int z_dtype, int rows, void* codes, int codes_dtype, int* indices,
                     float* bounded, hipStream_t s);
int ttvk_fsq_indices_to_codes(const ttv_fsq_params* p, const int* indices, int rows, void* codes, int codes_dtype, hipStream_t s);
int ttvk_enc_tail(const void* x, int dtype, int ld, const int* rows_map, int rows, int d, const float* gain, float eps,
                  const void* w, const void* bias, int C, const ttv_fsq_params* fsq, float* z_out, void* codes, int* indices,
                  float* bounded, hipStream_t s);
int ttvk_patch_copy(bool scatter, void* const* clips, const int* clip_desc, int clip0, int n_clips, int pt, int ph, int pw,
                    int C, void* patches, int ld, int dtype, int max_patches, hipStream_t s);
// ... 4 lines not shown

int ttvk_split3_pack(const float* w, int ldw, void* out, int ldo, int rows, int K, hipStream_t s);
int64_t ttvk_mx_scale_ld(int d);
int ttvk_quant_mx_fp8(const void* in, int in_dtype, int ld_in, void* out, int ld_out, void* mx, float* row_scales, int rows, int d, hipStream_t s);

int ttvk_clip_from_u8(const void* frames, long long n_pix, void* clip, int dtype, hipStream_t s);

int ttvk_clip_resample_u8(void* const* src, void* const* dst, const int32_t* geom, int n_clips, int dtype, hipStream_t s);

enum GemmEpilogue {
  EPI_STORE = 0,
  EPI_QKV_ROPE,
  EPI_GEGLU,
  EPI_RESID_T,
  EPI_RESID_F32,
  EPI_RESID_NORM,
  EPI_STORE_PATCH,
  EPI_BIAS_PLAIN,
  EPI_BIAS_GELU,
  EPI_BIAS_RESID_F32R,
};

struct GemmArgs {
  const void* x; int ldx;
  const void* w; int ldw;
  int M, N, K;
  void* y; int ldy;
  const void* bias;
  const float* add_scalar;
  const void* resid; int ldr;
  float alpha;
  const float* rope_cs;
  const int* rope_ids; const float* rope_base;
  int rope_q_end, rope_k_begin, rope_k_end;
  int dtype;
  const float* norm_gain;
  float* sum_f32; int ld_sum;
  void* y2; int ldy2; const float* norm_gain2;
  void* yq; void* yq_mx;
  int split3;
  int x_image, y_image;
  int prenorm;
  const float* row_scale;
  const int* x_rows;
  float eps;
  int gather;
  void* const* clips;
  int n_clips;
  const int* clip_desc;
  const int* patch_rows;
  const int* row_seq;
  int patch_t, patch_h, patch_w;
  int resid_rows;
};
struct ClipPtrs { void* p[TTV_MAX_CLIPS_PER_LAUNCH]; };
int ttvk_gemm(GemmEpilogue epi, const GemmArgs& a, hipStream_t s);
int ttvk_gemm_fp8(GemmEpilogue epi, const GemmArgs& a, const float* x_scale, const float* w_scale, hipStream_t s, const void* x_mx = nullptr,
                  const void* w_mx = nullptr);
bool ttvk_gemm_supports_resid_norm(int dtype, int N, int K);

int ttvk_attention(const void* qkvg, int ld, void* out, int ldo, const int* cu_seqlens, const int* qblocks, int n_qblocks,
                   int q_heads, int kv_heads, int head_dim, int flags, int dtype, hipStream_t s, float* lse_out = nullptr,
                   void* out_raw = nullptr);

int ttvk_attention_swp(const void* qkvg, int ld, void* out, int ldo, const int* cu_seqlens, const int* qblocks, int n_qblocks,
                       int q_heads, int kv_heads, int gate_mul, hipStream_t s);
int ttvk_attention_mxout(const void* qkvg, int ld, void* out_q, void* out_mx, int ld_mx, const int* cu_seqlens, const int* qblocks,
                         int n_qblocks, int q_heads, int kv_heads, hipStream_t s);

int ttvk_attention64(const void* qkvg, int ld, void* out, int ldo, const int* cu_seqlens, const int* items, int n_items, int q_heads,
                     int kv_heads, int flags, hipStream_t s);

int ttvk_vq_norms(const void* cb, int dtype, int ld, int N, int C, float* cnorm, hipStream_t s);
int64_t ttvk_vq_workspace_bytes(int rows);
int ttvk_vq_l2_argmin(const void* z, int dtype, int ldz, const void* cb, int ldc, const float* cnorm, int rows, int N, int C, int* indices,
                      float* best_dist, void* workspace, int64_t workspace_bytes, hipStream_t s);
int ttvk_vq_lookup(const void* cb, int dtype, int ldc, const int* indices, int rows, int C, void* codes, int ldo, hipStream_t s);
int ttvk_vq_lookup_bwd(const void* dcodes, int dtype, int ld, const int* indices, int rows, int C, float* dcb, int ldc, hipStream_t s);

bool ttvk_mlp_fused_supported(int dtype, int width, int inner);
struct MlpNextQkv {
  void* qkv; int ld;
  const float* rope_cs;
  int rows;
  int rope_q_end, rope_k_begin, rope_k_end;
};
int64_t ttvk_mlp_pack_bytes(int inner, int next_qkv_rows);
int ttvk_mlp_pack(const void* w12_folded, const void* w3, const void* wo, const void* next_qkv_folded, int next_qkv_rows, int inner,
                  void* packed, hipStream_t s);
int ttvk_mlp_fused(const void* ao, int ldao, const float* front_gain, float front_alpha, const void* x, int ldx, const void* packed,
                   int inner, void* y, int ldy, const float* post_gain, float alpha, float eps, int M, const MlpNextQkv* nq, hipStream_t s);

int ttvk_l1_loss(void* const* recon, void* const* target, void* const* grad, const int* sizes, int n_clips, int total_clips, int dtype,
                 float* loss, hipStream_t s);
int ttvk_sq_err(void* const* recon, void* const* target, const int* sizes, int n_clips, int dtype, int clamp, double* acc2, hipStream_t s);
int ttvk_rmsnorm_bwd_chain(const void* x, int ldx, const void* dy, int lddy, const float* gain1, float* dgain1, float* dx, int lddx,
                           const void* y, int y_dt, int ldy, const float* gain2, float* dgain2, float out_scale, void* cast_out, int ldc, int rows,
                           int d, float eps, int dt, hipStream_t s);
int ttvk_rmsnorm_bwd(const void* x, int x_dt, int ldx, const int* xr, const void* dy, int dy_dt, int lddy, const int* dyr,
                     const float* gain, void* dx, int dx_dt, int lddx, const int* dxr, int acc, float* dgain, int rows, int d, float eps,
                     hipStream_t s);
int ttvk_colsum(const void* a, int dt, int lda, const int* rows_map, int rows, int n, float* out, hipStream_t s);
int ttvk_sumall(const void* a, int dt, int lda, const int* rows_map, int rows, int n, const float* colw, float scale, float* out, hipStream_t s);
int ttvk_gate_fwd(const void* a, int lda, const void* gate, int ldg, void* ag, int ldo, int rows, int d, int dt, hipStream_t s);
int ttvk_gate_bwd(const void* dag, int ldd, const void* a, int lda, const void* gate, int ldg, void* da, int ldda, void* dgate, int lddg,
                  int rows, int d, int dt, float* delta, hipStream_t s);
int ttvk_geglu_fwd(const void* u, int ldu, void* h, int ldh, int rows, int I, int dt, hipStream_t s);
int ttvk_geglu_bwd(const void* u, int ldu, const void* dh, int lddh, void* du, int lddu, int rows, int I, int dt, hipStream_t s);
int ttvk_scale_cast(const float* a, float alpha, float* b, void* c, int dt, long n, hipStream_t s);
int ttvk_to_f32(const void* a, int dt, float* b, long n, int accumulate, hipStream_t s);
int ttvk_fsq_bwd(const ttv_fsq_params* fp, const float* z, const void* dcodes, int dt, float* dz, int rows, hipStream_t s);
#define TTV_WGRAD_BATCH 6
struct WgradBatch {
  int n = 0;
  int64_t used_bytes = 0;
  struct Entry { const float* part; float* dw; int splits, lddw, N, K, tiles_n, tiles; } e[TTV_WGRAD_BATCH];
};
int ttvk_wgrad(const void* dy, int lddy, const void* x, int ldx, float* dw, int lddw, int L, int N, int K, int dt, float* part,
               int64_t part_bytes, hipStream_t s, WgradBatch* batch = nullptr);
int ttvk_wgrad_flush(WgradBatch* batch, hipStream_t s);
int64_t ttvk_wgrad_ws_bytes(int L, int N, int K);
int ttvk_outer_small(const void* a, int a_dt, int lda, int C, const void* b, int b_dt, int ldb, const int* b_rows, float* dw, int lddw,
                     int transpose_out, int rows, int d, hipStream_t s);
int ttvk_expand_small(const void* a, int a_dt, int lda, int C, const void* w, int w_dt, int ldw, int w_cf, void* out, int o_dt, int ldo,
                      int rows, int d, hipStream_t s);
int ttvk_reduce_small(const void* a, int a_dt, int lda, const int* a_rows, const void* w, int w_dt, int ldw, int C, float* out, int ldo,
                      int rows, int d, hipStream_t s);
int ttvk_attention_bwd(const void* qkvg, int ld, const void* o, int ldo, const void* dout, int ldd, const float* lse, float* delta,
                       const int* cu, const int* blocks64, int n_blocks64, const int* row_seq, void* dqkvg, int ldg, float* dkv_scratch,
                       int total_rows, int hq, int hkv, int dt, const float* rope_cs, hipStream_t s, int delta_ready = 0, const int* qlim_desc = nullptr);
int ttvk_rope_apply_dir(void* x, int dtype, int ld, int rows, int heads, const float* cs, int conj, hipStream_t s);
int ttvk_dec_embed_ex(const void* codes, int C, const void* w, const void* bias, const float* mask_token, const float* gain, void* x,
                      int dtype, int ld, const int* rows_map, int rows, int d, float eps, void* hpre, hipStream_t s);
int ttvk_const_rows_bwd(const float* colsum, const float* mask_token, const float* gain, int dt, float eps, float* dgain, float* dmask,
                        int d, hipStream_t s);
int ttvk_rope_build(const float* base_cos, const float* base_sin, int n_ids, int F, const int* clip_desc, const int* cu, const int* row_seq,
                    float* out, int total_rows, hipStream_t s);

int64_t ttvk_ssim_workspace_bytes(const int32_t* dims, int n_clips);
int ttvk_ssim(void* const* recon, void* const* target, const int32_t* dims, int n_clips, int dtype, int clamp, double* acc2, void* workspace,
              int64_t workspace_bytes, hipStream_t s);

int ttvk_lpips_crops_forward(void* const* recon, void* const* target, const int32_t* clip_dims, int n_clips, const int32_t* crops, int n_crops,
                             int size, void* recon_crops, void* target_crops, int dtype, hipStream_t s);
// ... 33 lines not shown
```

### titok_video_amd/csrc/ttv_mlp.hip

```cpp
#include "ttv_common.h"
#include "ttv_kernels.h"

#define MLP_W12_CHUNKS 2048
#define MLP_W3_CHUNKS 1024
#define MLP_PANEL_CHUNKS (MLP_W12_CHUNKS + MLP_W3_CHUNKS)
#define MLP_WO_CHUNKS (4 * MLP_W12_CHUNKS)

struct MlpDev {
  const bf16_t* x; int ldx;
  const uint4* pack;
  const bf16_t* ao; int ldao;
  const float* front_gain;
  float front_alpha;
  bf16_t* qkv; int ldq;
  const float* rope_cs;
  int nqp, rope_q_end, rope_k_begin, rope_k_end;
  int I;
  bf16_t* y; int ldy;
  const float* post_gain;
  float alpha, eps;
  int M, n_tiles, debug;
  long long* stamps;
};

__global__ void k_mlp_pack(const bf16_t* __restrict__ w12f, const bf16_t* __restrict__ w3, const bf16_t* __restrict__ wo,
                           const bf16_t* __restrict__ wq, int nq_rows, int I, uint4* __restrict__ out) {
  const int np = I / 32;
  const int nqp = (nq_rows + 63) / 64;
  const int o = blockIdx.x * blockDim.x + threadIdx.x;
  if (o >= np * MLP_PANEL_CHUNKS + MLP_WO_CHUNKS + nqp * MLP_W12_CHUNKS) return;
  if (o >= np * MLP_PANEL_CHUNKS + MLP_WO_CHUNKS) {
    const int c = o - np * MLP_PANEL_CHUNKS - MLP_WO_CHUNKS, qp = c / MLP_W12_CHUNKS, cc = c - qp * MLP_W12_CHUNKS;
    const int r = cc >> 5, cp = cc & 31;
    const int ch = (cp & 16) | ((cp & 15) ^ (r & 15));
    int srow = qp * 64 + r;
    srow = srow < nq_rows ? srow : nq_rows - 1;
    const bf16_t* src = wq + (size_t)srow * 256 + (ch >> 2) * 32 + (ch & 3) * 4;
    const uint2 lo = *reinterpret_cast<const uint2*>(src), hi = *reinterpret_cast<const uint2*>(src + 16);
    out[o] = make_uint4(lo.x, lo.y, hi.x, hi.y);
    return;
  }
  if (o >= np * MLP_PANEL_CHUNKS) {
    const int c = o - np * MLP_PANEL_CHUNKS, wp = c / MLP_W12_CHUNKS, cc = c - wp * MLP_W12_CHUNKS;
    const int r = cc >> 5, cp = cc & 31;
    const int ch = (cp & 16) | ((cp & 15) ^ (r & 15));
    out[o] = wo ? *reinterpret_cast<const uint4*>(wo + (size_t)(wp * 64 + r) * 256 + ch * 8) : make_uint4(0, 0, 0, 0);
    return;
  }
  const int pn = o / MLP_PANEL_CHUNKS, c = o - pn * MLP_PANEL_CHUNKS;
  if (c < MLP_W12_CHUNKS) {
    const int r = c >> 5, cp = c & 31;
    const int ch = (cp & 16) | ((cp & 15) ^ (r & 15));
    const int srow = r < 32 ? pn * 32 + r : I + pn * 32 + (r - 32);
    const bf16_t* src = w12f + (size_t)srow * 256 + (ch >> 2) * 32 + (ch & 3) * 4;
    const uint2 lo = *reinterpret_cast<const uint2*>(src), hi = *reinterpret_cast<const uint2*>(src + 16);
    out[o] = make_uint4(lo.x, lo.y, hi.x, hi.y);
  } else {
    const int c3 = c - MLP_W12_CHUNKS, kq = c3 >> 8, row = c3 & 255;
    bf16x8 v;
#pragma unroll
    for (int j = 0; j < 8; ++j) v[j] = w3[(size_t)row * I + pn * 32 + (j < 4 ? 4 * kq + j : 16 + 4 * kq + (j - 4))];
    out[o] = __builtin_bit_cast(uint4, v);
  }
}

typedef uint32_t u32x2_t __attribute__((ext_vector_type(2)));
typedef uint32_t u32x4_t __attribute__((ext_vector_type(4)));
__device__ __forceinline__ f32x4 cvt4(bf16x4 b) { return (f32x4){(float)b[0], (float)b[1], (float)b[2], (float)b[3]}; }
#define MLP_LD12(img_, t_, s8_)                                                                                    \
  __builtin_bit_cast(bf16x8, (img_)[((t_) * 16 + l15) * 32 + ((((s8_) * 4 + kq) & 16) | ((((s8_) * 4 + kq) & 15) ^ l15))])
#define MLP_GLDS_4(src_, dst_)                                                                                     \
  do {                                                                                                             \
    unsigned keep__;                                                                                               \
    asm volatile("s_mov_b32 %0, m0\n\t"                                                                            \
                 "s_mov_b32 m0, %6\n\ts_nop 0\n\tglobal_load_lds_dwordx4 %1, %5\n\t"                               \
                 "s_add_u32 m0, %6, 0x2000\n\ts_nop 0\n\tglobal_load_lds_dwordx4 %2, %5\n\t"                       \
                 "s_add_u32 m0, %6, 0x4000\n\ts_nop 0\n\tglobal_load_lds_dwordx4 %3, %5\n\t"                       \
                 "s_add_u32 m0, %6, 0x6000\n\ts_nop 0\n\tglobal_load_lds_dwordx4 %4, %5\n\t"                       \
                 "s_mov_b32 m0, %0"                                                                                \
                 : "=&s"(keep__)                                                                                   \
                 : "v"(lane16), "v"(lane16 + 8192u), "v"(lane16 + 16384u), "v"(lane16 + 24576u), "s"(src_), "s"(dst_) \
                 : "memory", "scc");                                                                               \
  } while (0)
#define MLP_GLDS_2(src_, dst_)                                                                                     \
  do {                                                                                                             \
    unsigned keep__;                                                                                               \
    asm volatile("s_mov_b32 %0, m0\n\t"                                                                            \
                 "s_mov_b32 m0, %4\n\ts_nop 0\n\tglobal_load_lds_dwordx4 %1, %3\n\t"                               \
                 "s_add_u32 m0, %4, 0x2000\n\ts_nop 0\n\tglobal_load_lds_dwordx4 %2, %3\n\t"                       \
                 "s_mov_b32 m0, %0"                                                                                \
                 : "=&s"(keep__)                                                                                   \
                 : "v"(lane16), "v"(lane16 + 8192u), "s"(src_), "s"(dst_)                                          \
                 : "memory", "scc");                                                                               \
  } while (0)
#ifdef MLP_STAMPS
#define MLP_STAMP()                                                                                                \
  do {                                                                                                             \
    if (p.stamps && blockIdx.x == 0 && (wave & 3) == 0 && lane == 0 && n_stamp < 64)                               \
      p.stamps[(wave >> 2) * 64 + n_stamp++] = (long long)__builtin_readcyclecounter();                            \
  } while (0)
#else
#define MLP_STAMP() do { (void)n_stamp; } while (0)
#endif

template <int TPB, int T1, int T2, bool GELU_FIRST, bool KEEL, bool FRONT, bool BACK>
__device__ __forceinline__ void mlp_wave(const MlpDev& p, uint4* l12, uint4* l3, uint4* hb, const float* gl, int tile, int wave, int lane,
                                         int P1F, int P2F, int& n_stamp) {
  constexpr int T1A = T1 > 0 ? T1 : 1, T2A = T2 > 0 ? T2 : 1;
  const int l15 = lane & 15, kq = lane >> 4;
  const int np = p.I / 32;
  const uint32_t lane16 = lane * 16;
  const uint32_t lds_l12 = (uint32_t)(uintptr_t)(__attribute__((address_space(3))) void*)l12;
  const uint32_t lds_l3 = (uint32_t)(uintptr_t)(__attribute__((address_space(3))) void*)l3;
#define GLDS_W12(pn_, buf_)                                                                                        \
  do {                                                                                                             \
    const uint4* src__ = p.pack + ((size_t)(pn_) * MLP_PANEL_CHUNKS + wave * 64);                                  \
    const uint32_t dst__ = lds_l12 + ((buf_) * MLP_W12_CHUNKS + wave * 64) * 16;                                   \
    MLP_GLDS_4(src__, dst__);                                                                                      \
  } while (0)
#define GLDS_W3(pn_, buf_)                                                                                         \
  do {                                                                                                             \
    const uint4* src__ = p.pack + ((size_t)(pn_) * MLP_PANEL_CHUNKS + MLP_W12_CHUNKS + wave * 64);                 \
    const uint32_t dst__ = lds_l3 + ((buf_) * MLP_W3_CHUNKS + wave * 64) * 16;                                     \
    MLP_GLDS_2(src__, dst__);                                                                                      \
  } while (0)

  const int tok0 = tile * (16 * TPB) + l15;
  typedef __attribute__((address_space(1))) char gchar;
  typedef __attribute__((address_space(1))) const char gcchar;
  gcchar* const gx = (gcchar*)p.x;
  gcchar* const gao = (gcchar*)p.ao;
  gchar* const gy = (gchar*)p.y;

  MLP_STAMP();
  __syncthreads();

  bf16x8 bfr[T1A][8];
  float rstd[T1A];
  if (FRONT) {
#define GLDS_WO(wp_, buf_)                                                                                         \
  do {                                                                                                             \
    const uint4* src__ = p.pack + ((size_t)np * MLP_PANEL_CHUNKS + (wp_) * MLP_W12_CHUNKS + wave * 64);            \
    const uint32_t dst__ = lds_l12 + ((buf_) * MLP_W12_CHUNKS + wave * 64) * 16;                                   \
    MLP_GLDS_4(src__, dst__);                                                                                      \
  } while (0)
    GLDS_WO(0, 0);
    bf16x8 abf[T1A][8];
#pragma unroll
    for (int j = 0; j < T1; ++j) {
      const int t = tok0 + 16 * (P1F + j);
      const int tc = t < p.M ? t : p.M - 1;
      const uint32_t aoff = ((uint32_t)tc * (uint32_t)p.ldao + kq * 8) * 2u;
#pragma unroll
      for (int s8 = 0; s8 < 8; ++s8) abf[j][s8] = *(const __attribute__((address_space(1))) bf16x8*)(gao + aoff + s8 * 64);
    }
    f32x4 facc[16][T1A];
    __builtin_amdgcn_s_waitcnt(0x0F70);
    __syncthreads();
#pragma unroll
    for (int wp = 0; wp < 4; ++wp) {
      if (wp + 1 < 4) GLDS_WO(wp + 1, (wp + 1) & 1);
      const uint4* img = l12 + (wp & 1) * MLP_W12_CHUNKS;
      bf16x8 a[2][4];
      if constexpr (T1 > 0) {
#pragma unroll
      for (int i = 0; i < 4; ++i) a[0][i] = MLP_LD12(img, i, 0);
#pragma unroll
      for (int s8 = 0; s8 < 8; ++s8) {
        if (s8 + 1 < 8) {
#pragma unroll
          for (int i = 0; i < 4; ++i) a[(s8 + 1) & 1][i] = MLP_LD12(img, i, s8 + 1);
        }
#pragma unroll
        for (int i = 0; i < 4; ++i)
#pragma unroll
          for (int j = 0; j < T1; ++j)
            facc[4 * wp + i][j] = __builtin_amdgcn_mfma_f32_16x16x32_bf16(a[s8 & 1][i], abf[j][s8],
                                                                           s8 ? facc[4 * wp + i][j] : (f32x4){0.f, 0.f, 0.f, 0.f}, 0, 0, 0);
        if (s8 + 1 < 8) __builtin_amdgcn_sched_group_barrier(0x100, 4, 0);
        __builtin_amdgcn_sched_group_barrier(0x008, 4 * T1A, 0);
        __builtin_amdgcn_sched_barrier(0);
      }
      }
      __builtin_amdgcn_s_waitcnt(0x0F70);
      __syncthreads();
    }
#undef GLDS_WO
    GLDS_W12(0, 0);
#pragma unroll
    for (int j = 0; j < T1; ++j) {
      const int t = tok0 + 16 * (P1F + j);
      const int tc = t < p.M ? t : p.M - 1;
      const uint32_t roff = ((uint32_t)tc * (uint32_t)p.ldx + kq * 4) * 2u;
      float ss = 0.f;
#pragma unroll
      for (int m = 0; m < 16; ++m) {
        facc[m][j] += p.front_alpha * cvt4(*(const __attribute__((address_space(1))) bf16x4*)(gx + roff + m * 32));
#pragma unroll
        for (int e = 0; e < 4; ++e) ss = fmaf(facc[m][j][e], facc[m][j][e], ss);
      }
      float scale = 1.0f;
      if (p.front_gain) {
        ss = quad16_sum(ss);
        scale = 1.0f / sqrtf(ss * (1.0f / 256.0f) + p.eps);
      }
      float ss2 = 0.f;
#pragma unroll
      for (int s8 = 0; s8 < 8; ++s8) {
        bf16x4 q[2];
#pragma unroll
        for (int u = 0; u < 2; ++u) {
// ... 272 lines not shown
      f32x4 qa[4][T2A];
      bf16x8 a[2][4];
#pragma unroll
      for (int i = 0; i < 4; ++i) a[0][i] = MLP_LD12(img, i, 0);
#pragma unroll
      for (int s8 = 0; s8 < 8; ++s8) {
        if (s8 + 1 < 8) {
#pragma unroll
          for (int i = 0; i < 4; ++i) a[(s8 + 1) & 1][i] = MLP_LD12(img, i, s8 + 1);
        }
#pragma unroll
        for (int i = 0; i < 4; ++i)
#pragma unroll
          for (int j = 0; j < T2; ++j)
            qa[i][j] = __builtin_amdgcn_mfma_f32_16x16x32_bf16(a[s8 & 1][i], xq[j][s8], s8 ? qa[i][j] : (f32x4){0.f, 0.f, 0.f, 0.f}, 0, 0, 0);
        if (s8 + 1 < 8) __builtin_amdgcn_sched_group_barrier(0x100, 4, 0);
        __builtin_amdgcn_sched_group_barrier(0x008, 4 * T2A, 0);
        __builtin_amdgcn_sched_barrier(0);
      }
      __builtin_amdgcn_s_waitcnt(0x0F70);
      __syncthreads();
      const int f_first = qp * 64;
      const bool rot = f_first < p.rope_q_end || (f_first >= p.rope_k_begin && f_first < p.rope_k_end);
#pragma unroll
      for (int j = 0; j < T2; ++j) {
        const bool odd = kq & 1;
        gchar* const qrow = gq + (qoff[j] - (uint32_t)(kq * 4) * 2u) + (uint32_t)(f_first + (odd ? 16 + kq * 4 - 4 : kq * 4)) * 2u;
#pragma unroll
        for (int ip = 0; ip < 2; ++ip) {
          uint2 pk[2];
#pragma unroll
          for (int u = 0; u < 2; ++u) {
            const int i = 2 * ip + u;
            f32x4 v = qa[i][j] * rstdq[j];
            if (rot)
              v = (f32x4){v[0] * rc[i][j].x - v[1] * rs[i][j].x, v[0] * rs[i][j].x + v[1] * rc[i][j].x,
                          v[2] * rc[i][j].y - v[3] * rs[i][j].y, v[2] * rs[i][j].y + v[3] * rc[i][j].y};
            const bf16x4 q = {(bf16_t)v[0], (bf16_t)v[1], (bf16_t)v[2], (bf16_t)v[3]};
            pk[u] = __builtin_bit_cast(uint2, q);
          }
          const uint4 ox = xchg16_pair(pk[0], pk[1]);
          const u32x4_t ov = {ox.x, ox.y, ox.z, ox.w};
          if (qv[j]) *(__attribute__((address_space(1))) u32x4_t*)(qrow + ip * 64) = ov;
        }
      }
    }
#undef GLDS_WQ
    MLP_STAMP();
  }
#undef GLDS_W12
#undef GLDS_W3
}

template <int TILES, bool KEEL, bool FRONT, bool BACK>
__global__ __launch_bounds__(512, 1) void k_mlp256(MlpDev p) {
  extern __shared__ __attribute__((aligned(16))) uint4 smem[];
  uint4* const l12 = smem;
  uint4* const l3 = smem + 2 * MLP_W12_CHUNKS;
  uint4* const hb = l3 + 2 * MLP_W3_CHUNKS;
  float* const gl = reinterpret_cast<float*>(hb + 2 * TILES * 64);
  if (threadIdx.x < 256) {
    gl[threadIdx.x] = p.post_gain ? p.post_gain[threadIdx.x] : 1.0f;
    gl[256 + threadIdx.x] = (FRONT && p.front_gain) ? p.front_gain[threadIdx.x] : 1.0f;
  }
  const int lane = threadIdx.x & 63;
  const int wave = __builtin_amdgcn_readfirstlane(threadIdx.x >> 6);
  int n_stamp = 0;
  const int tile = blockIdx.x;
  if constexpr (TILES == 9) {
    if (wave < 4) mlp_wave<9, 2, 0, false, KEEL, FRONT, BACK>(p, l12, l3, hb, gl, tile, wave, lane, 2 * wave, 0, n_stamp);
    else if (wave < 6) mlp_wave<9, 0, 3, false, KEEL, FRONT, BACK>(p, l12, l3, hb, gl, tile, wave, lane, 0, 3 * (wave - 4), n_stamp);
    else if (wave == 6) mlp_wave<9, 1, 1, false, KEEL, FRONT, BACK>(p, l12, l3, hb, gl, tile, wave, lane, 8, 6, n_stamp);
    else mlp_wave<9, 0, 2, false, KEEL, FRONT, BACK>(p, l12, l3, hb, gl, tile, wave, lane, 0, 7, n_stamp);
  } else {
    constexpr int NT = TILES / 4;
    constexpr int TA = NT - NT / 2;
    const int g0 = (wave & 3) * NT;
    if (wave < 4) mlp_wave<TILES, TA, NT - TA, false, KEEL, FRONT, BACK>(p, l12, l3, hb, gl, tile, wave, lane, g0, g0 + TA, n_stamp);
    else mlp_wave<TILES, NT - TA, TA, false, KEEL, FRONT, BACK>(p, l12, l3, hb, gl, tile, wave, lane, g0 + TA, g0, n_stamp);
  }
}
#undef MLP_LD12
#undef MLP_GLDS_4
#undef MLP_GLDS_2
#undef MLP_STAMP

bool ttvk_mlp_fused_supported(int dtype, int width, int inner) { return dtype == TTV_BF16 && width == 256 && inner % 32 == 0 && inner > 0; }

int64_t ttvk_mlp_pack_bytes(int inner, int next_qkv_rows) {
  if (inner <= 0 || inner % 32 != 0 || next_qkv_rows < 0) return 0;
  return ((int64_t)(inner / 32) * MLP_PANEL_CHUNKS + MLP_WO_CHUNKS + (int64_t)((next_qkv_rows + 63) / 64) * MLP_W12_CHUNKS) * 16;
}

int ttvk_mlp_pack(const void* w12_folded, const void* w3, const void* wo, const void* next_qkv_folded, int next_qkv_rows, int inner,
                  void* packed, hipStream_t s) {
  TTV_CHECK_ARG(w12_folded && w3 && packed, "mlp_pack: null buffer");
  TTV_CHECK_ARG(inner > 0 && inner % 32 == 0, "mlp_pack: inner %% 32");
  TTV_CHECK_ARG((next_qkv_folded != nullptr) == (next_qkv_rows > 0), "mlp_pack: next_qkv weight and row count must come together");
  TTV_CHECK_ARG(((uintptr_t)w12_folded % 16 == 0) && ((uintptr_t)packed % 16 == 0) && ((uintptr_t)wo % 16 == 0) &&
                    ((uintptr_t)next_qkv_folded % 16 == 0), "mlp_pack: 16-byte alignment");
  const int total = inner / 32 * MLP_PANEL_CHUNKS + MLP_WO_CHUNKS + (next_qkv_rows + 63) / 64 * MLP_W12_CHUNKS;
  hipLaunchKernelGGL(k_mlp_pack, dim3(ttv_cdiv(total, 256)), dim3(256), 0, s, (const bf16_t*)w12_folded, (const bf16_t*)w3,
                     (const bf16_t*)wo, (const bf16_t*)next_qkv_folded, next_qkv_rows, inner, (uint4*)packed);
  TTV_CHECK_LAUNCH("mlp_pack");
  return TTV_OK;
}

int ttvk_mlp_fused(const void* ao, int ldao, const float* front_gain, float front_alpha, const void* x, int ldx, const void* packed,
                   int inner, void* y, int ldy, const float* post_gain, float alpha, float eps, int M, const MlpNextQkv* nq, hipStream_t s) {
  if (M == 0) return TTV_OK;
  TTV_CHECK_ARG(x && packed && y, "mlp_fused: null buffer");
  TTV_CHECK_ARG(inner % 32 == 0 && ldx % 8 == 0 && ldy % 8 == 0 && (!ao || ldao % 8 == 0), "mlp_fused: inner %% 32, leading dims %% 8");
  TTV_CHECK_ARG(((uintptr_t)x % 16 == 0) && ((uintptr_t)packed % 16 == 0) && ((uintptr_t)y % 16 == 0) && ((uintptr_t)ao % 16 == 0),
                "mlp_fused: 16-byte alignment");
  MlpDev d;
  d.x = (const bf16_t*)x; d.ldx = ldx; d.pack = (const uint4*)packed; d.I = inner;
  d.ao = (const bf16_t*)ao; d.ldao = ldao; d.front_gain = front_gain; d.front_alpha = front_alpha;
  d.y = (bf16_t*)y; d.ldy = ldy; d.post_gain = post_gain; d.alpha = alpha; d.eps = eps; d.M = M; d.debug = g_ttv_debug; d.stamps = g_ttv_stamps;
  d.qkv = nullptr; d.ldq = 0; d.rope_cs = nullptr; d.nqp = 0; d.rope_q_end = d.rope_k_begin = d.rope_k_end = 0;
  if (nq) {
    TTV_CHECK_ARG(nq->qkv && nq->rope_cs && nq->rows > 0 && nq->rows % 64 == 0 && nq->ld >= nq->rows && nq->ld % 4 == 0 &&
                      (uintptr_t)nq->qkv % 8 == 0, "mlp_fused: bad next-qkv arguments (rows %% 64, ld %% 4, 8-byte aligned)");
    TTV_CHECK_ARG(nq->rope_q_end % 64 == 0 && nq->rope_k_begin % 64 == 0 && nq->rope_k_end % 64 == 0, "mlp_fused: rotary ranges must be whole heads");
    d.qkv = (bf16_t*)nq->qkv; d.ldq = nq->ld; d.rope_cs = nq->rope_cs; d.nqp = nq->rows / 64;
    d.rope_q_end = nq->rope_q_end; d.rope_k_begin = nq->rope_k_begin; d.rope_k_end = nq->rope_k_end;
  }
  const int cus = 256;
  int tiles = 4;
  long best = -1;
  for (int c = 1; c <= 3; ++c) {
    const long cost = (long)ttv_cdiv(ttv_cdiv(M, 64 * c), cus) * (16 + 19 * c);
    if (best < 0 || cost < best) { best = cost; tiles = 4 * c; }
  }
  if (!nq && !(g_ttv_debug & TTV_DBG_MLP_PAIRS_ONLY)) {
    const long cost9 = (long)ttv_cdiv(ttv_cdiv(M, 144), cus) * (16 + 14 * 3);
    if (cost9 < best) { best = cost9; tiles = 9; }
  }
  if ((g_ttv_debug & TTV_DBG_MLP_TILES9) && !nq) tiles = 9;
  if (g_ttv_debug & TTV_DBG_MLP_TILES8) tiles = 8;
  if (g_ttv_debug & TTV_DBG_MLP_TILES4) tiles = 4;
  d.n_tiles = ttv_cdiv(M, 16 * tiles);
  const int grid = d.n_tiles;
  const size_t smem = (size_t)(2 * MLP_W12_CHUNKS + 2 * MLP_W3_CHUNKS + 2 * tiles * 64) * sizeof(uint4) + 2048;
  TtvProfScope prof(TTV_KC_GEMM_GEGLU, s);
#define LAUNCH_MLP(TILES_, KEEL_, FRONT_, BACK_)                                                                    \
  do {                                                                                                              \
    (void)hipFuncSetAttribute((const void*)k_mlp256<TILES_, KEEL_, FRONT_, BACK_>, hipFuncAttributeMaxDynamicSharedMemorySize, (int)smem); \
    hipLaunchKernelGGL((k_mlp256<TILES_, KEEL_, FRONT_, BACK_>), dim3(grid), dim3(512), smem, s, d);                \
  } while (0)
#define LAUNCH_MLP_F(TILES_, KEEL_)                                                                                 \
  do {                                                                                                              \
    if (ao && nq) LAUNCH_MLP(TILES_, KEEL_, true, true);                                                            \
    else if (ao) LAUNCH_MLP(TILES_, KEEL_, true, false);                                                            \
    else LAUNCH_MLP(TILES_, KEEL_, false, false);                                                                   \
  } while (0)
#define LAUNCH_MLP_9(KEEL_)                                                                                         \
  do {                                                                                                              \
    if (ao) LAUNCH_MLP(9, KEEL_, true, false);                                                                      \
    else LAUNCH_MLP(9, KEEL_, false, false);                                                                        \
  } while (0)
  TTV_CHECK_ARG(!nq || ao, "mlp_fused: the next-qkv part needs the out_proj front (ttv_layer_tail_fused)");
  if (post_gain) {
    if (tiles == 9) LAUNCH_MLP_9(true); else if (tiles == 12) LAUNCH_MLP_F(12, true); else if (tiles == 8) LAUNCH_MLP_F(8, true); else LAUNCH_MLP_F(4, true);
  } else {
    if (tiles == 9) LAUNCH_MLP_9(false); else if (tiles == 12) LAUNCH_MLP_F(12, false); else if (tiles == 8) LAUNCH_MLP_F(8, false); else LAUNCH_MLP_F(4, false);
  }
#undef LAUNCH_MLP_9
#undef LAUNCH_MLP_F
#undef LAUNCH_MLP
  TTV_CHECK_LAUNCH("mlp_fused");
  return TTV_OK;
}
```

### titok_video_amd/csrc/ttv_qkv256.inc

```
#ifdef QKV_STAMPS
#define QK_STAMP_DECL unsigned long long qst_prev__ = 0, qst_acc__[8] = {0, 0, 0, 0, 0, 0, 0, 0}
#define QK_STAMP_START()                                                                                     \
  do {                                                                                                       \
    __builtin_amdgcn_sched_barrier(0);                                                                       \
    asm volatile("s_memtime %0\n\ts_waitcnt lgkmcnt(0)" : "=s"(qst_prev__)::"memory");                       \
    __builtin_amdgcn_sched_barrier(0);                                                                       \
  } while (0)
#define QK_STAMP(seg_)                                                                                       \
  do {                                                                                                       \
    unsigned long long t__;                                                                                  \
    __builtin_amdgcn_sched_barrier(0);                                                                       \
    asm volatile("s_memtime %0\n\ts_waitcnt lgkmcnt(0)" : "=s"(t__)::"memory");                              \
    __builtin_amdgcn_sched_barrier(0);                                                                       \
    qst_acc__[seg_] += t__ - qst_prev__;                                                                     \
    qst_prev__ = t__;                                                                                        \
  } while (0)
#else
#define QK_STAMP_DECL
#define QK_STAMP_START()
#define QK_STAMP(seg_)
#endif
typedef unsigned qk_u32x4 __attribute__((ext_vector_type(4)));
typedef unsigned qk_u32x2 __attribute__((ext_vector_type(2)));
template <bool PRENORM>
__global__ __launch_bounds__(256, 2) void k_qkv256(GemmDev p, int n_panels, int total_items) {
  __shared__ uint4 wl[2][K256_ROWS * 32];

  const int tid = threadIdx.x, lane = tid & 63;
  const int wave = __builtin_amdgcn_readfirstlane(tid >> 6);
  const int r = lane & 31, h = lane >> 5;
  const int lb = xcd_remap(blockIdx.x, gridDim.x);
  const int it0 = (int)((long)total_items * lb / gridDim.x);
  const int it1 = (int)((long)total_items * (lb + 1) / gridDim.x);
  if (it0 >= it1) return;
  const bf16_t* X = (const bf16_t*)p.x;

  const uint32_t wl_lds = (uint32_t)(uintptr_t)(__attribute__((address_space(3))) void*)&wl[0][0];
  const uint32_t dchunk0 = (uint32_t)(((lane & 16) | ((lane & 15) ^ h)) * 16);
  const uint32_t drow0 = (uint32_t)h * (uint32_t)p.ldw * 2u;
  const uint32_t dstride = (uint32_t)p.ldw * 4u;
#define QK_DMA_PIECE(dc_, i_, src_, dst_)                                                                       \
  do {                                                                                                       \
    unsigned keep__;                                                                                         \
    const uint32_t voff__ = ((dc_) ^ (uint32_t)((i_) << 5)) + drow0;                                            \
    asm volatile("s_mov_b32 %0, m0\n\ts_mov_b32 m0, %3\n\ts_nop 0\n\tglobal_load_lds_dwordx4 %1, %2\n\ts_mov_b32 m0, %0" \
                 : "=&s"(keep__) : "v"(voff__), "s"((src_) + (size_t)(i_) * dstride), "s"((dst_) + (i_) * 1024) : "memory"); \
  } while (0)
#define QK_PANEL_SRC(panel_) (reinterpret_cast<const char*>(p.w) + ((size_t)(panel_) * 64 + wave * 16) * (size_t)p.ldw * 2)
#define QK_PANEL_DST(buf_) (wl_lds + (buf_) * (K256_ROWS * 512) + wave * (16 * 512))

  const int r15 = r & 15;
  const char* const wl_base = reinterpret_cast<const char*>(&wl[0][0]);
  const uint32_t aoff0 = (uint32_t)(r * 32 + (h ^ r15)) * 16u;
#define QK_AFRAG(buf_, t_, ks_) \
  (*reinterpret_cast<const bf16x8*>(wl_base + (a0__ ^ (uint32_t)(((ks_) & 7) << 5)) + (buf_) * (K256_ROWS * 512) + (t_) * (32 * 512) + (((ks_) >> 3) & 1) * 256))

  bf16x8 bfr[16];
  float rstd = 1.f;
  float2 rcs[2][4][2];
  char* ytok = nullptr;
  uint2 idp = make_uint2(0u, 0u);
  int tk = 0;
  bool tok_ok = true, wave_full = true;
  int cur_tile = -1;
  int pend = 0;
  int pend_panel = 0;
  const f32x16 zero16 = {0.f, 0.f, 0.f, 0.f, 0.f, 0.f, 0.f, 0.f, 0.f, 0.f, 0.f, 0.f, 0.f, 0.f, 0.f, 0.f};

#define QK_ROT(acc_, ROT_, G_)                                                                               \
  do {                                                                                                       \
    const int t__ = (G_) >> 2, g__ = (G_) & 3;                                                               \
    const float a0__ = acc_[t__][4 * g__], a1__ = acc_[t__][4 * g__ + 1], a2__ = acc_[t__][4 * g__ + 2], a3__ = acc_[t__][4 * g__ + 3]; \
    if (ROT_) {                                                                                              \
      const float2 k0__ = rcs[t__][g__][0], k1__ = rcs[t__][g__][1];                                         \
      o_[0] = a0__ * k0__.x - a1__ * k0__.y; o_[1] = a0__ * k0__.y + a1__ * k0__.x;                          \
      o_[2] = a2__ * k1__.x - a3__ * k1__.y; o_[3] = a2__ * k1__.y + a3__ * k1__.x;                          \
    } else {                                                                                                 \
      o_[0] = a0__ * rstd; o_[1] = a1__ * rstd; o_[2] = a2__ * rstd; o_[3] = a3__ * rstd;                    \
    }                                                                                                        \
    asm volatile("" : "+v"(o_[0]), "+v"(o_[1]), "+v"(o_[2]), "+v"(o_[3]));                                   \
  } while (0)
#define QK_PACK(G_)                                                                                          \
  do {                                                                                                       \
    const int g__ = (G_) & 3;                                                                                \
    const bf16x4 b__ = {(bf16_t)o_[0], (bf16_t)o_[1], (bf16_t)o_[2], (bf16_t)o_[3]};                         \
    pk_[g__ & 1] = __builtin_bit_cast(qk_u32x2, b__);                                                        \
    if (g__ & 1) {                                                                                           \
      const auto sx__ = __builtin_amdgcn_permlane32_swap(pk_[0].x, pk_[1].x, false, false);                  \
      const auto sy__ = __builtin_amdgcn_permlane32_swap(pk_[0].y, pk_[1].y, false, false);                  \
      out_ = (qk_u32x4){sx__[0], sy__[0], sx__[1], sy__[1]};                                                 \
      asm volatile("" : "+v"(out_));                                                                         \
    } else {                                                                                                 \
      asm volatile("" : "+v"(pk_[0]));                                                                       \
    }                                                                                                        \
  } while (0)
#define QK_STORE_CHUNK(c_, panel_)                                                                           \
  do {                                                                                                       \
    if (tok_ok && !(p.debug & TTV_DBG_NO_STORES)) *reinterpret_cast<qk_u32x4*>(ytok + (size_t)(panel_) * 128 + (c_) * 32) = out_; \
  } while (0)
#define QK_EPILOGUE(acc_, ROT_, panel_)                                                                      \
  do {                                                                                                       \
// ... 43 lines not shown
              const float2 sn__ = *reinterpret_cast<const float2*>(c__ + 32 + 16 * t__ + 4 * g__);           \
              rcs[t__][g__][0] = make_float2(cc__.x, sn__.x);                                                \
              rcs[t__][g__][1] = make_float2(cc__.y, sn__.y);                                                \
            }                                                                                                \
        }                                                                                                    \
      }                                                                                                      \
      __builtin_amdgcn_sched_barrier(0);                                                                     \
      if (ks__ + 1 < 16) {                                                                                   \
        af__[(ks__ + 1) & 1][0] = QK_AFRAG(buf_, 0, ks__ + 1);                                               \
        af__[(ks__ + 1) & 1][1] = QK_AFRAG(buf_, 1, ks__ + 1);                                               \
      }                                                                                                      \
      cur_[0] = __builtin_amdgcn_mfma_f32_32x32x16_bf16(af__[ks__ & 1][0], bfr[ks__], ks__ ? cur_[0] : zero16, 0, 0, 0); \
      cur_[1] = __builtin_amdgcn_mfma_f32_32x32x16_bf16(af__[ks__ & 1][1], bfr[ks__], ks__ ? cur_[1] : zero16, 0, 0, 0); \
      if (MODE_) {                                                                                           \
        if ((ks__ & 1) == 0) QK_ROT(prev_, MODE_ == 2, ks__ >> 1); else QK_PACK(ks__ >> 1);                  \
      } else if (PRENORM) {                                                                                  \
        const bf16x8 v__ = bfr[ks__];                                                                        \
        ss0__ = __builtin_amdgcn_fdot2_f32_bf16((bf16x2){v__[0], v__[1]}, (bf16x2){v__[0], v__[1]}, ss0__, false); \
        ss1__ = __builtin_amdgcn_fdot2_f32_bf16((bf16x2){v__[2], v__[3]}, (bf16x2){v__[2], v__[3]}, ss1__, false); \
        ss0__ = __builtin_amdgcn_fdot2_f32_bf16((bf16x2){v__[4], v__[5]}, (bf16x2){v__[4], v__[5]}, ss0__, false); \
        ss1__ = __builtin_amdgcn_fdot2_f32_bf16((bf16x2){v__[6], v__[7]}, (bf16x2){v__[6], v__[7]}, ss1__, false); \
        asm volatile("" : "+v"(ss0__), "+v"(ss1__));                                                         \
      }                                                                                                      \
      if (ks__ + 1 < 16) __builtin_amdgcn_sched_group_barrier(0x100, 2, 0);                                  \
      __builtin_amdgcn_sched_group_barrier(0x008, 1, 0);                                                     \
      if (MODE_) { if ((ks__ & 1) || MODE_ != 2) __builtin_amdgcn_sched_group_barrier(0x002, 2, 0); else __builtin_amdgcn_sched_group_barrier(0x002, 4, 0); } \
      else if (PRENORM) __builtin_amdgcn_sched_group_barrier(0x002, 2, 0);                                   \
      __builtin_amdgcn_sched_group_barrier(0x008, 1, 0);                                                     \
      if (MODE_) { if ((ks__ & 1) || MODE_ != 2) __builtin_amdgcn_sched_group_barrier(0x002, 2, 0); else __builtin_amdgcn_sched_group_barrier(0x002, 4, 0); } \
      else if (PRENORM) __builtin_amdgcn_sched_group_barrier(0x002, 2, 0);                                   \
      __builtin_amdgcn_sched_barrier(0);                                                                     \
      if (MODE_ && (ks__ & 3) == 3) {                                                                        \
        QK_STORE_CHUNK(ks__ >> 2, pend_panel);                                                               \
        __builtin_amdgcn_sched_barrier(0);                                                                   \
      }                                                                                                      \
    }                                                                                                        \
    if (MODE_ == 0) {                                                                                        \
      if (PRENORM) {                                                                                         \
        float ss__ = ss0__ + ss1__;                                                                          \
        ss__ = pair32_sum(ss__);                                                                    \
        rstd = 1.0f / sqrtf(ss__ * (1.0f / 256.0f) + p.eps);                                                 \
      }                                                                                                      \
      _Pragma("unroll") for (int t__ = 0; t__ < 2; ++t__)                                                    \
        _Pragma("unroll") for (int g__ = 0; g__ < 4; ++g__)                                                  \
          _Pragma("unroll") for (int e__ = 0; e__ < 2; ++e__)                                                \
            rcs[t__][g__][e__] = make_float2(rcs[t__][g__][e__].x * rstd, rcs[t__][g__][e__].y * rstd);      \
    }                                                                                                        \
  } while (0)

#define QK_STEP(cur_, prev_, it_)                                                                            \
  do {                                                                                                       \
    const int it__ = (it_);                                                                                  \
    const int buf__ = (it__ - it0) & 1;                                                                      \
    const int tile__ = it__ / n_panels, panel__ = it__ - tile__ * n_panels;                                  \
    if (tile__ != cur_tile) {                                                                                \
      cur_tile = tile__;                                                                                     \
       \
                                                                               \
      const int t0__ = tile__ * K256_TT + wave * 32;                                                         \
      int ntk__ = t0__ + r;                                                                                  \
      const bool nok__ = ntk__ < p.M;                                                                        \
      ntk__ = nok__ ? ntk__ : p.M - 1;                                                                       \
      const bf16_t* xr__ = X + (size_t)(p.x_rows ? p.x_rows[ntk__] : ntk__) * p.ldx + h * 8;                 \
      _Pragma("unroll") for (int ks__ = 0; ks__ < 16; ++ks__) bfr[ks__] = *reinterpret_cast<const bf16x8*>(xr__ + ks__ * 16); \
      uint2 nidp__ = make_uint2(0u, 0u);                                                                     \
      if (p.rope_ids) nidp__ = *reinterpret_cast<const uint2*>(p.rope_ids + 2 * (size_t)ntk__);              \
      if (pend == 2) QK_EPILOGUE(prev_, true, pend_panel); else if (pend == 1) QK_EPILOGUE(prev_, false, pend_panel); \
      pend = 0;                                                                                              \
       \
       \
       \
      _Pragma("unroll") for (int ks__ = 0; ks__ < 16; ++ks__) asm volatile("" : "+v"(bfr[ks__]));            \
      tk = ntk__; tok_ok = nok__; idp = nidp__;                                                              \
      wave_full = t0__ + 32 <= p.M;                                                                          \
      ytok = reinterpret_cast<char*>((bf16_t*)p.y + (size_t)tk * p.ldy) + h * 16;                            \
      rstd = 1.f;                                                                                            \
    }                                                                                                        \
    QK_STAMP(0);                                                                                             \
    if (it__ == it0) {                                                                                       \
      asm volatile("s_waitcnt vmcnt(0)" ::: "memory");                                                       \
      __syncthreads();                                                                                       \
    }                                                                                                        \
    QK_STAMP(1);                                                                                             \
    const bool has_next__ = it__ + 1 < it1;                                                                  \
    const char* nsrc__ = QK_PANEL_SRC((it__ + 1) % n_panels);                                                \
    const uint32_t ndst__ = QK_PANEL_DST(buf__ ^ 1);                                                         \
    const int f_first__ = panel__ * 64;                                                                      \
    const int rot__ = (f_first__ < p.rope_q_end || (f_first__ >= p.rope_k_begin && f_first__ < p.rope_k_end)) ? 2 : 1; \
    bool counted__ = false;                                                                                  \
    if (pend == 2) {                                                                                         \
      if (buf__) QK_BODY(cur_, prev_, 1, 2); else QK_BODY(cur_, prev_, 0, 2);                                \
      counted__ = wave_full && !(p.debug & TTV_DBG_NO_STORES);                                                               \
      QK_STAMP(2);                                                                                           \
    } else if (pend == 1) {                                                                                  \
      if (buf__) QK_BODY(cur_, prev_, 1, 1); else QK_BODY(cur_, prev_, 0, 1);                                \
      counted__ = wave_full && !(p.debug & TTV_DBG_NO_STORES);                                                               \
      QK_STAMP(2);                                                                                           \
    } else {                                                                                                 \
      if (buf__) QK_BODY(cur_, prev_, 1, 0); else QK_BODY(cur_, prev_, 0, 0);                                \
      QK_STAMP(3);                                                                                           \
    }                                                                                                        \
     \
    if (counted__) asm volatile("s_waitcnt vmcnt(3)" ::: "memory");                                          \
    else asm volatile("s_waitcnt vmcnt(0)" ::: "memory");                                                    \
    QK_STAMP(4);                                                                                             \
    __builtin_amdgcn_s_barrier();                                                                            \
    QK_STAMP(5);                                                                                             \
    pend = rot__;                                                                                            \
    pend_panel = panel__;                                                                                    \
  } while (0)

  f32x16 accA[2], accB[2];
  QK_STAMP_DECL;
  {
    const char* src0 = QK_PANEL_SRC(it0 % n_panels);
    const uint32_t dst0 = QK_PANEL_DST(0);
    QK_DMA_PIECE(dchunk0, 0, src0, dst0); QK_DMA_PIECE(dchunk0, 1, src0, dst0); QK_DMA_PIECE(dchunk0, 2, src0, dst0); QK_DMA_PIECE(dchunk0, 3, src0, dst0);
    QK_DMA_PIECE(dchunk0, 4, src0, dst0); QK_DMA_PIECE(dchunk0, 5, src0, dst0); QK_DMA_PIECE(dchunk0, 6, src0, dst0); QK_DMA_PIECE(dchunk0, 7, src0, dst0);
  }
  QK_STAMP_START();
  int it = it0;
  for (; it + 1 < it1; it += 2) {
    QK_STEP(accA, accB, it);
    QK_STEP(accB, accA, it + 1);
  }
  if (it < it1) {
    QK_STEP(accA, accB, it);
    if (pend == 2) QK_EPILOGUE(accA, true, pend_panel); else QK_EPILOGUE(accA, false, pend_panel);
  } else {
    if (pend == 2) QK_EPILOGUE(accB, true, pend_panel); else QK_EPILOGUE(accB, false, pend_panel);
  }
  QK_STAMP(6);
#ifdef QKV_STAMPS
  if (p.stamps && lb % 16 == 0 && lane == 0) {
    long long* dst = p.stamps + ((size_t)(lb / 16) * 4 + wave) * 8;
    for (int i = 0; i < 7; ++i) dst[i] = (long long)qst_acc__[i];
    dst[7] = it1 - it0;
  }
#endif
#undef QK_DMA_PIECE
#undef QK_PANEL_SRC
#undef QK_PANEL_DST
#undef QK_AFRAG
#undef QK_ROT
#undef QK_PACK
#undef QK_STORE_CHUNK
#undef QK_EPILOGUE
#undef QK_BODY
#undef QK_STEP
}
```

### titok_video_amd/model/base/blocks.py

```python
from __future__ import annotations

import ctypes as C
import math
from typing import List, Optional, Sequence

import torch
import torch.nn as nn

from ... import _lib, switches
from ...plan import BatchPlan, get_plan, host_ints
from .utils import LinearWeight, RMSNormWeight, geglu_inner_dim, get_model_dims


class _AttnParams(nn.Module):

    def __init__(self, dim: int, heads: Sequence[int]):
        super().__init__()
        q_heads, kv_heads = heads
        gqa = (dim // q_heads) * kv_heads
        self.pre_ln = RMSNormWeight(dim)
        self.to_qkv = LinearWeight(dim, 2 * gqa + 2 * dim, bias=False)
        self.out_proj = LinearWeight(dim, dim, bias=False)


# ... 284 lines not shown
            self.q_prescaled = 1

        def f8_mx(w, g=None, q_rows=0):
            if not use_mx:
                return None, None, None
            t = w.detach().to(device=device, dtype=torch.float32)
            t = (t * g.detach().to(device=device, dtype=torch.float32)[None, :]) if g is not None else t.clone()
            if q_rows and q_scale is not None:
                t[:q_rows] *= q_scale
            t = t.contiguous()
            n_rows, k = t.shape
            q = torch.empty((n_rows, k), dtype=torch.uint8, device=device)
            sc = torch.empty(n_rows, dtype=torch.float32, device=device)
            mx = torch.zeros((n_rows, int(_lib.lib().ttv_mx_scale_bytes_per_row(k))), dtype=torch.uint8, device=device)
            _lib.check(_lib.lib().ttv_quant_mx_fp8(t.data_ptr(), _lib.TTV_F32, k, q.data_ptr(), k, mx.data_ptr(), sc.data_ptr(), n_rows, k,
                                                   _lib.stream_ptr(device)), "ttv_quant_mx_fp8")
            keep.extend([t, q, sc, mx])
            return q.data_ptr(), sc.data_ptr(), mx.data_ptr()

        def f8_rows(w, q_rows=0):
            if not use_f8:
                return None, None
            t = w.detach().to(device=device, dtype=torch.float32).clone()
            if q_rows and q_scale is not None:
                t[:q_rows] *= q_scale
            t = t.contiguous()
            q = torch.empty(t.shape, dtype=torch.uint8, device=device)
            sc = torch.empty(t.shape[0], dtype=torch.float32, device=device)
            _lib.check(_lib.lib().ttv_quant_rows_fp8(t.data_ptr(), _lib.TTV_F32, t.shape[1], None, 0.0, q.data_ptr(), t.shape[1], sc.data_ptr(),
                                                     t.shape[0], t.shape[1], _lib.stream_ptr(device)), "ttv_quant_rows_fp8")
            keep.extend([t, q, sc])
            return q.data_ptr(), sc.data_ptr()

        def folded_tensor(w, g, q_rows=0):
            t = (w.detach().to(device=device, dtype=torch.float32) * g.detach().to(device=device, dtype=torch.float32)[None, :])
            if q_rows and q_scale is not None:
                t[:q_rows] *= q_scale
            return t.to(dtype).contiguous()

        def folded(w, g, q_rows=0):
            if self.f32_split3 and switches.flag("TTV_SPLIT3_FOLD", False):
                t = (w.detach().to(device=device, dtype=torch.float32) * g.detach().to(device=device, dtype=torch.float32)[None, :]).contiguous()
                img = torch.empty_like(t)
                _lib.check(_lib.lib().ttv_split3_pack(t.data_ptr(), t.shape[1], img.data_ptr(), t.shape[1], t.shape[0], t.shape[1], _lib.stream_ptr(device)),
                           "ttv_split3_pack")
                keep.extend([t, img])
                return img.data_ptr()
            if not (fold or fold_gen):
                return None
            t = folded_tensor(w, g, q_rows)
            keep.append(t)
            return t.data_ptr()

        def mlp_packed(w12, g, w3, wo, next_attn):
            if not fold or w3.shape[1] % 32:
                return None, 0
            w12f = folded_tensor(w12, g)
            w3c = w3.detach().to(device=device, dtype=dtype).contiguous()
            woc = wo.detach().to(device=device, dtype=dtype).contiguous()
            wq, rows = None, 0
            if next_attn is not None and next_attn.to_qkv.weight.shape[0] % 64 == 0:
                wq = folded_tensor(next_attn.to_qkv.weight, next_attn.pre_ln.weight, q_rows=tower.width)
                rows = int(wq.shape[0])
            inner = int(w3.shape[1])
            out = torch.empty(_lib.lib().ttv_mlp_pack_bytes(inner, rows), dtype=torch.uint8, device=device)
            _lib.check(_lib.lib().ttv_mlp_pack(w12f.data_ptr(), w3c.data_ptr(), woc.data_ptr(), wq.data_ptr() if wq is not None else None,
                                               rows, inner, tower.width, _lib.TTV_BF16, out.data_ptr(), _lib.stream_ptr(device)),
                       "mlp_pack")
            keep.extend([w12f, w3c, woc, wq, out])
            return out.data_ptr(), rows

        perm = tower._patch_perm_on(device)
        if tower.kind == _lib.TTV_ENCODER:
            w_in = tower.proj_in.weight.detach().to(device)[:, perm]
            b_out, w_out = tower.proj_out.bias, tower.proj_out.weight
        else:
            w_in = tower.proj_in.weight
            w_out = tower.proj_out.weight.detach().to(device)[perm, :]
            b_out = tower.proj_out.bias.detach().to(device)[perm]
        ml = tower.model_layers
        n = tower.num_layers
        self.layers = (_lib.LayerWeights * n)()
        for i in range(n):
            a, f = ml.attn_layer[i], ml.ffd_layer[i]
            pack_ptr, pack_rows = mlp_packed(f.w12.weight, f.norm.weight, f.w3.weight, a.out_proj.weight,
                                             ml.attn_layer[i + 1] if i + 1 < n else None)
            if use_mx:
                qkv8, qkv8s, qkvmx = f8_mx(a.to_qkv.weight, a.pre_ln.weight, q_rows=tower.width)
                w128, w128s, w12mx = f8_mx(f.w12.weight, f.norm.weight)
                wo8, wo8s, womx = f8_mx(a.out_proj.weight)
                w38, w38s, w3mx = f8_mx(f.w3.weight)
            else:
                qkv8, qkv8s = f8_rows(a.to_qkv.weight, q_rows=tower.width)
                w128, w128s = f8_rows(f.w12.weight)
                qkvmx = w12mx = wo8 = wo8s = womx = w38 = w38s = w3mx = None
            self.layers[i] = _lib.LayerWeights(
                to_qkv_f8=qkv8, to_qkv_f8_scale=qkv8s, w12_f8=w128, w12_f8_scale=w128s,
                to_qkv_mx=qkvmx, w12_mx=w12mx, out_proj_f8=wo8, out_proj_f8_scale=wo8s, out_proj_mx=womx,
                w3_f8=w38, w3_f8_scale=w38s, w3_mx=w3mx,
                pre_ln=gain(a.pre_ln.weight), to_qkv=lin(a.to_qkv.weight, True), out_proj=lin(a.out_proj.weight, True),
                ffd_norm=gain(f.norm.weight), w12=lin(f.w12.weight, True), w3=lin(f.w3.weight, True),
                attn_post_ln=gain(ml.attn_post_ln[i - 1].weight) if i > 0 else None,
                ffd_post_ln=gain(ml.ffd_post_ln[i - 1].weight) if i > 0 else None,
                to_qkv_pn=folded(a.to_qkv.weight, a.pre_ln.weight, q_rows=tower.width), w12_pn=folded(f.w12.weight, f.norm.weight),
                mlp_pack=pack_ptr, mlp_pack_qkv_rows=pack_rows, qkv_q_prescaled=self.q_prescaled, to_qkv_qs=lin_qs(a.to_qkv.weight))
        self.struct = _lib.TowerWeights(
            proj_in_w=lin(w_in, tower.kind == _lib.TTV_ENCODER), proj_in_b=lin(tower.proj_in.bias), mask_token=gain(tower.mask_token),
            ln_pre_t=gain(tower.ln_pre_t.weight), ln_pre_p=gain(tower.ln_pre_p.weight), ln_post=gain(tower.ln_post.weight),
            proj_out_w=lin(w_out, tower.kind == _lib.TTV_DECODER), proj_out_b=lin(b_out), layers=self.layers,
            f32_split3=1 if self.f32_split3 else 0,
            proj_out_pn=folded(w_out, tower.ln_post.weight) if (tower.kind == _lib.TTV_DECODER and fold) else None)
        self.keep = keep
        self.kind, self.n_layers = tower.kind, n
        self._t = None
        if self.device.type == "cuda":
            self.build_stream = torch.cuda.current_stream(self.device)
            self.ready = torch.cuda.Event()
            self.ready.record(self.build_stream)

    def use_on_current_stream(self) -> None:
        if self.ready is None:
            return
        cur = torch.cuda.current_stream(self.device)
        if cur != self.build_stream and cur.cuda_stream not in self.reader_streams:
            cur.wait_event(self.ready)
        self.reader_streams[cur.cuda_stream] = cur

    def transposed(self) -> "_lib.TowerWeightsT":
        if self._t is None:
            lt = self.lin_tensors
            arr = (_lib.LayerWeightsT * self.n_layers)()
            keep = []

            def tr(t):
                u = t.t().contiguous()
                keep.append(u)
                return u.data_ptr()
            for i in range(self.n_layers):
                q, o, w12, w3 = lt[4 * i: 4 * i + 4]
                arr[i] = _lib.LayerWeightsT(to_qkv_t=tr(q), out_proj_t=tr(o), w12_t=tr(w12), w3_t=tr(w3))
            proj_in_w, proj_out_w = lt[4 * self.n_layers], lt[4 * self.n_layers + 2]
            st = _lib.TowerWeightsT(proj_in_t=tr(proj_in_w) if self.kind == _lib.TTV_ENCODER else None,
                                    proj_out_t=tr(proj_out_w) if self.kind == _lib.TTV_DECODER else None, layers=arr)
            self._t = (st, arr, keep)
        return self._t[0]


class TiTokEncoder(_Tower):
    kind = _lib.TTV_ENCODER

    def __init__(self, model_size="tiny", patch_size=(4, 8, 8), in_channels=3, out_channels=5):
        super().__init__()
        mlp_ratio = self._setup(model_size, patch_size, in_channels, out_channels)
        self.in_channels = in_channels
        scale = self.width ** -0.5
        self.proj_in = LinearWeight(in_channels * math.prod(self.patch), self.width)
        self.mask_token = nn.Parameter(scale * torch.randn(1, 1))
        self.ln_pre_t = RMSNormWeight(self.width)
# ... 185 lines not shown
```

Before: 30220.

## Move attention gate projection from QKV GEMM into fused MLP tail kernel

The QKV projection kernel now skips the gate column panels. The attention kernel runs without its gate flag, and the gate projection (pre-norm folded weights packed into the MLP buffer) is computed inside the fused layer-tail MLP kernel, where it is applied to the attention output. This is meant to remove the gate columns from the QKV GEMM and stop writing and reading gate activations through the qkv buffer. In exchange the tail kernel does extra work and needs a new template variant. The path is gated on bf16, width 256, and the non-fp8 QKV path.

```diff
diff --git a/include/titok_hip.h b/include/titok_hip.h
--- a/include/titok_hip.h
+++ b/include/titok_hip.h
@@ -94,6 +94,13 @@
 int ttv_layer_tail_fused(const void* ao, int ldao, const float* attn_post_gain, float attn_alpha, const void* x, int ldx,
                          const void* mlp_packed, int inner, void* y, int ldy, const float* ffd_post_gain, float ffd_alpha, float eps,
                          int M, int width, int dtype, const ttv_next_qkv* next, void* stream);
+
+int ttv_mlp_pack_gate(const void* gate_folded, int next_qkv_rows, int inner, int width, int dtype, void* mlp_packed, void* stream);
+int ttv_layer_tail_gated(const void* ao, int ldao, const float* attn_post_gain, float attn_alpha, const void* x, int ldx,
+                         const void* mlp_packed, int next_qkv_rows, int inner, void* y, int ldy, const float* ffd_post_gain, float ffd_alpha,
+                         float eps, int M, int width, int dtype, void* stream);
+int ttv_linear_qkv_rope_prenorm(const void* x, int ldx, const void* w_folded, int ldw, void* y, int ldy, int M, int d_model, int gqa_dim,
+                                const float* rope_cs, float eps, int skip_gate, int dtype, void* stream);
 
 int ttv_fill_const_rows(void* x, int dtype, int ld, const int32_t* rows_map, int rows, int width, const float* mask_token,
                         const float* gain, float eps, void* stream);
@@ -414,7 +421,8 @@
   TTV_DBG_QKV256_WS = 131072,
   TTV_DBG_ENC_ALL_ROWS = 524288,
   TTV_DBG_ATTN_NO_SWP = 1048576,
-  TTV_DBG_DEC_ALL_BLOCKS = 2097152
+  TTV_DBG_DEC_ALL_BLOCKS = 2097152,
+  TTV_DBG_GATE_IN_QKV = 4194304
 };
 int ttv_debug_set(int flags);
 int ttv_debug_stamps(void* device_buffer);
diff --git a/titok_video_amd/_lib.py b/titok_video_amd/_lib.py
--- a/titok_video_amd/_lib.py
+++ b/titok_video_amd/_lib.py
@@ -39,6 +39,7 @@
 DBG_ENC_ALL_ROWS = 524288
 DBG_ATTN_NO_SWP = 1048576
 DBG_DEC_ALL_BLOCKS = 2097152
+DBG_GATE_IN_QKV = 4194304
 
 _HERE = os.path.dirname(os.path.abspath(__file__))
 LIB_PATH = switches.text("TTV_LIB_PATH") or os.path.join(_HERE, "libtitok_hip.so")
@@ -166,6 +167,10 @@
                                            C.c_int, C.c_int, vp]),
     "ttv_mlp_pack_bytes": (C.c_int64, [C.c_int, C.c_int]),
     "ttv_mlp_pack": (C.c_int, [vp, vp, vp, vp, C.c_int, C.c_int, C.c_int, C.c_int, vp, vp]),
+    "ttv_mlp_pack_gate": (C.c_int, [vp, C.c_int, C.c_int, C.c_int, C.c_int, vp, vp]),
+    "ttv_layer_tail_gated": (C.c_int, [vp, C.c_int, vp, f32, vp, C.c_int, vp, C.c_int, C.c_int, vp, C.c_int, vp, f32, f32, C.c_int, C.c_int,
+                                       C.c_int, vp]),
+    "ttv_linear_qkv_rope_prenorm": (C.c_int, [vp, C.c_int, vp, C.c_int, vp, C.c_int, C.c_int, C.c_int, C.c_int, vp, f32, C.c_int, C.c_int, vp]),
     "ttv_layer_tail_fused": (C.c_int, [vp, C.c_int, vp, f32, vp, C.c_int, vp, C.c_int, vp, C.c_int, vp, f32, f32, C.c_int, C.c_int,
                                        C.c_int, vp, vp]),
     "ttv_mlp_fused": (C.c_int, [vp, C.c_int, vp, C.c_int, vp, C.c_int, vp, f32, f32, C.c_int, C.c_int, C.c_int, vp]),
diff --git a/titok_video_amd/csrc/ttv_api.hip b/titok_video_amd/csrc/ttv_api.hip
--- a/titok_video_amd/csrc/ttv_api.hip
+++ b/titok_video_amd/csrc/ttv_api.hip
@@ -20,6 +20,7 @@
 bool ttv_sw_keel_f32sum() { static const bool v = ttv_env_flag("TTV_KEEL_F32SUM", false); return v; }
 bool ttv_sw_fused_patch() { static const bool v = ttv_env_flag("TTV_FUSED_PATCH", true); return v; }
 bool ttv_sw_attn_pipe() { static const bool v = ttv_env_flag("TTV_ATTN_PIPE", false); return v; }
+bool ttv_sw_gate_tail() { static const bool v = ttv_env_flag("TTV_GATE_TAIL", true); return v; }
 float ttv_sw_attn_thr() { static const float v = ttv_env_float("TTV_ATTN_THR", 8.0f); return v; }
 thread_local int g_ttv_debug = 0;
 long long* g_ttv_stamps = nullptr;
@@ -108,7 +109,7 @@
   a.dtype = dt; a.x = ws.f8; a.ldx = dm; a.w = lw.to_qkv_f8; a.ldw = dm; a.M = L; a.N = nq; a.K = dm; a.y = ws.qkv; a.ldy = nq;
   a.rope_cs = b->rope_cs; a.rope_q_end = dm; a.rope_k_begin = 2 * dm; a.rope_k_end = 2 * dm + g;
   TTV_TRY(ttvk_gemm_fp8(EPI_QKV_ROPE, a, ws.rstd, lw.to_qkv_f8_scale, s, ws.f8mx, lw.to_qkv_mx));
-  const bool q_scaled = lw.qkv_q_prescaled != 0;
+  const bool q_scaled = (lw.qkv_q_prescaled & 1) != 0;
   if (fused_q && q_scaled && !b->qblocks_paired && !attn_pipe && d->head_dim == 64) {
     TTV_TRY(ttvk_attention_mxout(ws.qkv, nq, ws.f8, ws.f8mx, (int)ttvk_mx_scale_ld(dm), b->cu_seqlens, b->qblocks, b->n_qblocks, d->q_heads,
                                  d->kv_heads, s));
@@ -170,7 +171,7 @@
 struct PreNormW { const float* gain; const void *w, *w_pn, *w_f8; const float* w_f8_scale; bool f8; };
 
 static int prenorm_proj(const LayerCtx& c, GemmEpilogue epi, const char* x, int rows, const PreNormW& p, int N, char* y, int y_image,
-                        bool rstd_valid) {
+                        bool rstd_valid, bool no_gate = false) {
   const ttv_tower_dims* d = c.d;
   const TowerWs& ws = c.ws;
   const int dm = d->width, dt = d->dtype;
@@ -178,6 +179,7 @@
   a.dtype = dt; a.ldx = dm; a.ldw = dm; a.M = rows; a.N = N; a.K = dm; a.y = y; a.ldy = N;
   if (epi == EPI_QKV_ROPE) {
     a.rope_cs = c.b->rope_cs; a.rope_q_end = dm; a.rope_k_begin = 2 * dm; a.rope_k_end = 2 * dm + d->kv_heads * d->head_dim;
+    if (no_gate) { a.skip_cols_begin = dm; a.skip_cols_end = 2 * dm; }
   }
   if (p.f8) {
     float* const f8_scales = reinterpret_cast<float*>(ws.xn + (((size_t)c.b->total_rows * dm + 255) & ~(size_t)255));
@@ -238,6 +240,9 @@
   static const bool pat_env = ttv_env_flag("TTV_DEC_PATCH_LAST", true);
   const bool pat_last = pat_env && !(g_ttv_debug & TTV_DBG_DEC_ALL_BLOCKS) && d->kind == TTV_DECODER && d->layers >= 2 && b->qblocks_patch &&
                         b->n_qblocks_patch > 0 && !split3 && !b->qblocks_paired;
+  static const bool use_fused_mlp = ttv_env_flag("TTV_FUSED_MLP", true);
+  static const bool use_fused_qkv = ttv_env_flag("TTV_FUSED_QKV", false);
+  static const bool gate_tail_env = ttv_sw_gate_tail();
   bool compacted = false;
   const LayerCtx ctx = {d, b, ws, s, split3, s3img, gen_ok};
   for (int i = 0; i < d->layers; ++i) {
@@ -253,28 +258,32 @@
     xq_valid = false;
     const bool f8_qkv = rows_f8(dt, dm, lw.to_qkv_f8, lw.to_qkv_f8_scale, lw.to_qkv_mx, lw.to_qkv_pn);
     const bool f8_w12 = rows_f8(dt, dm, lw.w12_f8, lw.w12_f8_scale, lw.w12_mx, lw.w12_pn);
+    const bool gate_tail = gate_tail_env && !(g_ttv_debug & TTV_DBG_GATE_IN_QKV) && dt == TTV_BF16 && dm == 256 && !split3 && use_fused_mlp &&
+                           !use_fused_qkv && ttvk_mlp_fused_supported(dt, dm, d->inner) && lw.mlp_pack && (lw.qkv_q_prescaled & 2) && lw.to_qkv_pn &&
+                           !rows_f8(dt, dm, lw.to_qkv_f8, lw.to_qkv_f8_scale, lw.to_qkv_mx, lw.to_qkv_pn) && !qkv_ready;
+    const int attn_gate = gate_tail ? 0 : TTV_ATTN_GATE;
     if (!qkv_ready) {
       const void* w_plain = (dt == TTV_BF16 && lw.to_qkv_qs) ? lw.to_qkv_qs : lw.to_qkv;
       const PreNormW qw = {lw.pre_ln, w_plain, lw.to_qkv_pn, lw.to_qkv_f8, lw.to_qkv_f8_scale, f8_qkv};
-      TTV_TRY(prenorm_proj(ctx, EPI_QKV_ROPE, ws.x, L, qw, nq, ws.qkv, s3img ? 2 : 0, rstd_valid));
+      TTV_TRY(prenorm_proj(ctx, EPI_QKV_ROPE, ws.x, L, qw, nq, ws.qkv, s3img ? 2 : 0, rstd_valid, gate_tail));
     }
-    const bool q_scaled = dt == TTV_BF16 && (lw.to_qkv_pn ? lw.qkv_q_prescaled != 0 : lw.to_qkv_qs != nullptr);
+    const bool q_scaled = dt == TTV_BF16 && (lw.to_qkv_pn ? (lw.qkv_q_prescaled & 1) != 0 : lw.to_qkv_qs != nullptr);
     rstd_valid = false;
     qkv_ready = false;
     const bool lat_now = lat_last && i == d->layers - 1;
     if (lat_now)
       TTV_TRY(ttvk_attention(ws.qkv, nq, ws.ao, dm, b->cu_seqlens, b->qblocks_latent, b->n_qblocks_latent, d->q_heads, d->kv_heads, d->head_dim,
-                             TTV_ATTN_GATE | (b->qblocks_all_full ? TTV_ATTN_ALLFULL : 0) | (q_scaled ? TTV_ATTN_QSCALED : 0) | (split3 ? TTV_ATTN_SPLIT3 : 0) |
+                             attn_gate | (b->qblocks_all_full ? TTV_ATTN_ALLFULL : 0) | (q_scaled ? TTV_ATTN_QSCALED : 0) | (split3 ? TTV_ATTN_SPLIT3 : 0) |
                                  (s3img ? (TTV_ATTN_SPLIT_OUT | TTV_ATTN_SPLIT_IN) : 0), dt, s));
     else if (pat_last && i == d->layers - 1 && dt == TTV_BF16 && !attn_pipe)
       TTV_TRY(ttvk_attention(ws.qkv, nq, ws.ao, dm, b->cu_seqlens, b->qblocks_patch, b->n_qblocks_patch, d->q_heads, d->kv_heads, d->head_dim,
-                             TTV_ATTN_GATE | (b->qblocks_all_full ? TTV_ATTN_ALLFULL : 0) | (q_scaled ? TTV_ATTN_QSCALED : 0), dt, s));
+                             attn_gate | (b->qblocks_all_full ? TTV_ATTN_ALLFULL : 0) | (q_scaled ? TTV_ATTN_QSCALED : 0), dt, s));
     else if (q_scaled && b->items64 && b->n_items64 > 0 && d->head_dim == 64)
       TTV_TRY(ttvk_attention64(ws.qkv, nq, ws.ao, dm, b->cu_seqlens, b->items64, b->n_items64, d->q_heads, d->kv_heads,
-                               TTV_ATTN_GATE | TTV_ATTN_QSCALED, s));
+                               attn_gate | TTV_ATTN_QSCALED, s));
     else
     TTV_TRY(ttvk_attention(ws.qkv, nq, ws.ao, dm, b->cu_seqlens, b->qblocks, b->n_qblocks, d->q_heads, d->kv_heads, d->head_dim,
-                           TTV_ATTN_GATE | (b->qblocks_paired ? TTV_ATTN_PAIRED : 0) | (q_scaled ? TTV_ATTN_QSCALED : 0) |
+                           attn_gate | (b->qblocks_paired ? TTV_ATTN_PAIRED : 0) | (q_scaled ? TTV_ATTN_QSCALED : 0) |
                                (b->qblocks_all_full ? TTV_ATTN_ALLFULL : 0) | (attn_pipe ? TTV_ATTN_PIPE : 0) | (split3 ? TTV_ATTN_SPLIT3 : 0) |
                                (s3img ? (TTV_ATTN_SPLIT_OUT | TTV_ATTN_SPLIT_IN) : 0), dt, s));
     char* cx = ws.x;
@@ -287,14 +296,13 @@
       cx = ws.xl; cao = ws.aol; Lc = b->sum_tokens;
       compacted = true;
     }
-    static const bool use_fused_mlp = ttv_env_flag("TTV_FUSED_MLP", true);
-    static const bool use_fused_qkv = ttv_env_flag("TTV_FUSED_QKV", false);
     if (use_fused_mlp && ttvk_mlp_fused_supported(dt, dm, d->inner) && lw.mlp_pack) {
       MlpNextQkv nx = {};
       const bool back = use_fused_qkv && i + 1 < d->layers && lw.mlp_pack_qkv_rows == nq && nq % 64 == 0 && dm % 64 == 0 && g % 64 == 0;
       if (back) { nx.qkv = ws.qkv; nx.ld = nq; nx.rope_cs = b->rope_cs; nx.rows = nq; nx.rope_q_end = dm; nx.rope_k_begin = 2 * dm; nx.rope_k_end = 2 * dm + g; }
       TTV_TRY(ttvk_mlp_fused(cao, dm, i == 0 ? nullptr : lw.attn_post_ln, i == 0 ? 1.f : d->alpha, cx, dm, lw.mlp_pack, d->inner,
-                             cx, dm, i == 0 ? nullptr : lw.ffd_post_ln, i == 0 ? 1.f : d->alpha, d->eps, Lc, back ? &nx : nullptr, s));
+                             cx, dm, i == 0 ? nullptr : lw.ffd_post_ln, i == 0 ? 1.f : d->alpha, d->eps, Lc, back ? &nx : nullptr, s,
+                             gate_tail ? (const char*)lw.mlp_pack + ttvk_mlp_pack_gate_offset(d->inner, lw.mlp_pack_qkv_rows) : nullptr));
       qkv_ready = back;
       continue;
     }
@@ -443,6 +451,18 @@
   return ttvk_gemm(EPI_QKV_ROPE, a, (hipStream_t)stream);
 }
 
+int ttv_linear_qkv_rope_prenorm(const void* x, int ldx, const void* w_folded, int ldw, void* y, int ldy, int M, int d_model, int gqa_dim,
+                                const float* rope_cs, float eps, int skip_gate, int dtype, void* stream) {
+  TTV_CHECK_ARG(M == 0 || (x && w_folded && y && rope_cs), "linear_qkv_rope_prenorm: null buffer");
+  TTV_CHECK_ARG(dtype == TTV_BF16 && d_model == 256, "linear_qkv_rope_prenorm: bf16, width 256");
+  GemmArgs a = {};
+  a.dtype = dtype; a.x = x; a.ldx = ldx; a.w = w_folded; a.ldw = ldw; a.M = M; a.N = 2 * d_model + 2 * gqa_dim; a.K = d_model;
+  a.y = y; a.ldy = ldy; a.rope_cs = rope_cs; a.rope_q_end = d_model; a.rope_k_begin = 2 * d_model; a.rope_k_end = 2 * d_model + gqa_dim;
+  a.prenorm = 1; a.eps = eps;
+  if (skip_gate) { a.skip_cols_begin = d_model; a.skip_cols_end = 2 * d_model; }
+  return ttvk_gemm(EPI_QKV_ROPE, a, (hipStream_t)stream);
+}
+
 int ttv_linear_geglu(const void* x, int ldx, const void* w, int ldw, void* y, int ldy, int M, int I, int K, int dtype, void* stream) {
   TTV_CHECK_ARG(M == 0 || (x && w && y), "linear_geglu: null buffer");
   GemmArgs a = {};
@@ -481,6 +501,14 @@
     return TTV_ERR_UNSUPPORTED;
   }
   return ttvk_mlp_pack(w12_folded, w3, out_proj, next_qkv_folded, next_qkv_rows, inner, packed, (hipStream_t)stream);
+}
+
+int ttv_mlp_pack_gate(const void* gate_folded, int next_qkv_rows, int inner, int width, int dtype, void* mlp_packed, void* stream) {
+  if (!ttvk_mlp_fused_supported(dtype, width, inner)) {
+    ttv_set_error("mlp_pack_gate: only bf16, width 256, inner %% 32 == 0");
+    return TTV_ERR_UNSUPPORTED;
+  }
+  return ttvk_mlp_pack_gate(gate_folded, next_qkv_rows, inner, mlp_packed, (hipStream_t)stream);
 }
 
 int ttv_mlp_fused(const void* x, int ldx, const void* mlp_packed, int inner, void* y, int ldy, const float* post_gain, float alpha,
@@ -505,6 +533,18 @@
               nx.rope_k_begin = next->rope_k_begin; nx.rope_k_end = next->rope_k_end; }
   return ttvk_mlp_fused(ao, ldao, attn_post_gain, attn_alpha, x, ldx, mlp_packed, inner, y, ldy, ffd_post_gain, ffd_alpha, eps, M,
                         next ? &nx : nullptr, (hipStream_t)stream);
+}
+
+int ttv_layer_tail_gated(const void* ao, int ldao, const float* attn_post_gain, float attn_alpha, const void* x, int ldx,
+                         const void* mlp_packed, int next_qkv_rows, int inner, void* y, int ldy, const float* ffd_post_gain, float ffd_alpha,
+                         float eps, int M, int width, int dtype, void* stream) {
+  if (!ttvk_mlp_fused_supported(dtype, width, inner)) {
+    ttv_set_error("layer_tail_gated: only bf16, width 256, inner %% 32 == 0");
+    return TTV_ERR_UNSUPPORTED;
+  }
+  TTV_CHECK_ARG(ao && mlp_packed, "layer_tail_gated: null buffer");
+  return ttvk_mlp_fused(ao, ldao, attn_post_gain, attn_alpha, x, ldx, mlp_packed, inner, y, ldy, ffd_post_gain, ffd_alpha, eps, M, nullptr,
+                        (hipStream_t)stream, (const char*)mlp_packed + ttvk_mlp_pack_gate_offset(inner, next_qkv_rows));
 }
 
 int ttv_fill_const_rows(void* x, int dtype, int ld, const int32_t* rows_map, int rows, int width, const float* mask_token,
diff --git a/titok_video_amd/csrc/ttv_common.h b/titok_video_amd/csrc/ttv_common.h
--- a/titok_video_amd/csrc/ttv_common.h
+++ b/titok_video_amd/csrc/ttv_common.h
@@ -177,6 +177,7 @@
 bool ttv_sw_keel_f32sum();
 bool ttv_sw_fused_patch();
 bool ttv_sw_attn_pipe();
+bool ttv_sw_gate_tail();
 float ttv_sw_attn_thr();
 
 __device__ __forceinline__ float ttv_cubic_src(int dst, float scale) { return fmaf(scale, (float)dst + 0.5f, -0.5f); }
diff --git a/titok_video_amd/csrc/ttv_gemm.hip b/titok_video_amd/csrc/ttv_gemm.hip
--- a/titok_video_amd/csrc/ttv_gemm.hip
+++ b/titok_video_amd/csrc/ttv_gemm.hip
@@ -30,6 +30,7 @@
   int clip0, pt_shift, ph_shift;
   long long* stamps;
   int resid_rows;
+  int skip_p0, skip_np;
 };
 
 struct PatchDst {
@@ -1871,8 +1872,19 @@
           TTV_CHECK_LAUNCH("qkv256ws");
           return TTV_OK;
         }
-        if (prenorm) hipLaunchKernelGGL((k_qkv256<true>), dim3(grid), dim3(256), 0, s, d, n_panels, total);
-        else hipLaunchKernelGGL((k_qkv256<false>), dim3(grid), dim3(256), 0, s, d, n_panels, total);
+        if (prenorm && d.skip_np > 0) {
+          const int np = n_panels - d.skip_np, tot = np * n_tiles;
+          int gs = tot < 512 ? tot : 512;
+          if (grid_env > 0) gs = tot < grid_env ? tot : grid_env;
+          else if (tot > 512)
+            for (int g = 512; g >= 416; --g)
+              if (tot % g == 0) { gs = g; break; }
+          hipLaunchKernelGGL((k_qkv256<true, true>), dim3(gs), dim3(256), 0, s, d, np, tot);
+          TTV_CHECK_LAUNCH("qkv256 (q | k | v)");
+          return TTV_OK;
+        }
+        if (prenorm) hipLaunchKernelGGL((k_qkv256<true, false>), dim3(grid), dim3(256), 0, s, d, n_panels, total);
+        else hipLaunchKernelGGL((k_qkv256<false, false>), dim3(grid), dim3(256), 0, s, d, n_panels, total);
         TTV_CHECK_LAUNCH("qkv256");
         return TTV_OK;
       }
@@ -2014,6 +2026,12 @@
   d.norm_gain = a.norm_gain;
   d.clip_desc = a.clip_desc; d.patch_rows = a.patch_rows; d.row_seq = a.row_seq; d.clip0 = 0; d.pt_shift = d.ph_shift = 0;
   d.x_rows = a.x_rows;
+  d.skip_p0 = d.skip_np = 0;
+  if (epi == EPI_QKV_ROPE && a.skip_cols_end > a.skip_cols_begin) {
+    TTV_CHECK_ARG(a.skip_cols_begin % 64 == 0 && a.skip_cols_end % 64 == 0 && a.skip_cols_begin >= 0 && a.skip_cols_end <= a.N,
+                  "gemm: skipped to_qkv columns must be whole 64-column panels");
+    d.skip_p0 = a.skip_cols_begin / 64; d.skip_np = (a.skip_cols_end - a.skip_cols_begin) / 64;
+  }
   d.x_scale = nullptr; d.w_scale = nullptr;
   d.row_scale = a.row_scale;
   d.stamps = g_ttv_stamps;
diff --git a/titok_video_amd/csrc/ttv_kernels.h b/titok_video_amd/csrc/ttv_kernels.h
--- a/titok_video_amd/csrc/ttv_kernels.h
+++ b/titok_video_amd/csrc/ttv_kernels.h
@@ -80,6 +80,7 @@
   const int* row_seq;
   int patch_t, patch_h, patch_w;
   int resid_rows;
+  int skip_cols_begin, skip_cols_end;
 };
 struct ClipPtrs { void* p[TTV_MAX_CLIPS_PER_LAUNCH]; };
 int ttvk_gemm(GemmEpilogue epi, const GemmArgs& a, hipStream_t s);
@@ -117,7 +118,10 @@
 int ttvk_mlp_pack(const void* w12_folded, const void* w3, const void* wo, const void* next_qkv_folded, int next_qkv_rows, int inner,
                   void* packed, hipStream_t s);
 int ttvk_mlp_fused(const void* ao, int ldao, const float* front_gain, float front_alpha, const void* x, int ldx, const void* packed,
-                   int inner, void* y, int ldy, const float* post_gain, float alpha, float eps, int M, const MlpNextQkv* nq, hipStream_t s);
+                   int inner, void* y, int ldy, const float* post_gain, float alpha, float eps, int M, const MlpNextQkv* nq, hipStream_t s,
+                   const void* gate_pack = nullptr);
+int64_t ttvk_mlp_pack_gate_offset(int inner, int next_qkv_rows);
+int ttvk_mlp_pack_gate(const void* gate_folded, int next_qkv_rows, int inner, void* packed, hipStream_t s);
 
 int ttvk_l1_loss(void* const* recon, void* const* target, void* const* grad, const int* sizes, int n_clips, int total_clips, int dtype,
                  float* loss, hipStream_t s);
diff --git a/titok_video_amd/csrc/ttv_mlp.hip b/titok_video_amd/csrc/ttv_mlp.hip
--- a/titok_video_amd/csrc/ttv_mlp.hip
+++ b/titok_video_amd/csrc/ttv_mlp.hip
@@ -12,6 +12,7 @@
   const bf16_t* ao; int ldao;
   const float* front_gain;
   float front_alpha;
+  int gate_off;
   bf16_t* qkv; int ldq;
   const float* rope_cs;
   int nqp, rope_q_end, rope_k_begin, rope_k_end;
@@ -62,6 +63,16 @@
     for (int j = 0; j < 8; ++j) v[j] = w3[(size_t)row * I + pn * 32 + (j < 4 ? 4 * kq + j : 16 + 4 * kq + (j - 4))];
     out[o] = __builtin_bit_cast(uint4, v);
   }
+}
+
+__global__ void k_mlp_pack_gate(const bf16_t* __restrict__ wg, uint4* __restrict__ out) {
+  const int o = blockIdx.x * blockDim.x + threadIdx.x;
+  if (o >= MLP_WO_CHUNKS) return;
+  const int gp = o / MLP_W12_CHUNKS, cc = o - gp * MLP_W12_CHUNKS;
+  const int r = cc >> 5, cp = cc & 31;
+  const int ch = (cp & 16) | ((cp & 15) ^ (r & 15));
+  const int s8 = 2 * gp + (r >> 5), u = (r >> 4) & 1, kq = (r >> 2) & 3, e = r & 3;
+  out[o] = *reinterpret_cast<const uint4*>(wg + (size_t)(32 * s8 + 8 * kq + 4 * u + e) * 256 + ch * 8);
 }
 
 typedef uint32_t u32x2_t __attribute__((ext_vector_type(2)));
@@ -103,7 +114,7 @@
 #define MLP_STAMP() do { (void)n_stamp; } while (0)
 #endif
 
-template <int TPB, int T1, int T2, bool GELU_FIRST, bool KEEL, bool FRONT, bool BACK>
+template <int TPB, int T1, int T2, bool GELU_FIRST, bool KEEL, bool FRONT, bool BACK, bool GATE>
 __device__ __forceinline__ void mlp_wave(const MlpDev& p, uint4* l12, uint4* l3, uint4* hb, const float* gl, int tile, int wave, int lane,
                                          int P1F, int P2F, int& n_stamp) {
   constexpr int T1A = T1 > 0 ? T1 : 1, T2A = T2 > 0 ? T2 : 1;
@@ -144,8 +155,100 @@
     const uint32_t dst__ = lds_l12 + ((buf_) * MLP_W12_CHUNKS + wave * 64) * 16;                                   \
     MLP_GLDS_4(src__, dst__);                                                                                      \
   } while (0)
+    bf16x8 abf[T1A][8];
+    if constexpr (GATE) {
+#define GLDS_WG(gp_, buf_)                                                                                         \
+  do {                                                                                                             \
+    const uint4* src__ = p.pack + ((size_t)p.gate_off + (gp_) * MLP_W12_CHUNKS + wave * 64);                                       \
+    const uint32_t dst__ = lds_l12 + ((buf_) * MLP_W12_CHUNKS + wave * 64) * 16;                                   \
+    MLP_GLDS_4(src__, dst__);                                                                                      \
+  } while (0)
+      GLDS_WG(0, 0);
+      float grstd[T1A];
+#pragma unroll
+      for (int j = 0; j < T1; ++j) {
+        const int t = tok0 + 16 * (P1F + j);
+        const int tc = t < p.M ? t : p.M - 1;
+        const uint32_t xoff = ((uint32_t)tc * (uint32_t)p.ldx + kq * 8) * 2u;
+#pragma unroll
+        for (int s8 = 0; s8 < 8; ++s8) abf[j][s8] = *(const __attribute__((address_space(1))) bf16x8*)(gx + xoff + s8 * 64);
+      }
+#pragma unroll
+      for (int j = 0; j < T1; ++j) {
+        float ss = 0.f;
+#pragma unroll
+        for (int s8 = 0; s8 < 8; ++s8)
+#pragma unroll
+          for (int e = 0; e < 8; ++e) {
+            const float v = (float)abf[j][s8][e];
+            ss = fmaf(v, v, ss);
+          }
+        ss = quad16_sum(ss);
+        grstd[j] = 1.0f / sqrtf(ss * (1.0f / 256.0f) + p.eps);
+      }
+      f32x4 gacc[16][T1A];
+      __builtin_amdgcn_s_waitcnt(0x0F70);
+      __syncthreads();
+#pragma unroll
+      for (int gp = 0; gp < 4; ++gp) {
+        if (gp + 1 < 4) GLDS_WG(gp + 1, (gp + 1) & 1); else GLDS_WO(0, 0);
+        const uint4* img = l12 + (gp & 1) * MLP_W12_CHUNKS;
+        bf16x8 a[2][4];
+        if constexpr (T1 > 0) {
+#pragma unroll
+        for (int i = 0; i < 4; ++i) a[0][i] = MLP_LD12(img, i, 0);
+#pragma unroll
+        for (int s8 = 0; s8 < 8; ++s8) {
+          if (s8 + 1 < 8) {
+#pragma unroll
+            for (int i = 0; i < 4; ++i) a[(s8 + 1) & 1][i] = MLP_LD12(img, i, s8 + 1);
+          }
+#pragma unroll
+          for (int i = 0; i < 4; ++i)
+#pragma unroll
+            for (int j = 0; j < T1; ++j)
+              gacc[4 * gp + i][j] = __builtin_amdgcn_mfma_f32_16x16x32_bf16(a[s8 & 1][i], abf[j][s8],
+                                                                             s8 ? gacc[4 * gp + i][j] : (f32x4){0.f, 0.f, 0.f, 0.f}, 0, 0, 0);
+          if (s8 + 1 < 8) __builtin_amdgcn_sched_group_barrier(0x100, 4, 0);
+          __builtin_amdgcn_sched_group_barrier(0x008, 4 * T1A, 0);
+          __builtin_amdgcn_sched_barrier(0);
+        }
+        }
+        __builtin_amdgcn_s_waitcnt(0x0F70);
+        __syncthreads();
+      }
+#undef GLDS_WG
+#pragma unroll
+      for (int j = 0; j < T1; ++j) {
+        const int t = tok0 + 16 * (P1F + j);
+        const int tc = t < p.M ? t : p.M - 1;
+        const uint32_t aoff = ((uint32_t)tc * (uint32_t)p.ldao + kq * 8) * 2u;
+#pragma unroll
+        for (int s8 = 0; s8 < 8; ++s8) abf[j][s8] = *(const __attribute__((address_space(1))) bf16x8*)(gao + aoff + s8 * 64);
+      }
+#pragma unroll
+      for (int j = 0; j < T1; ++j)
+#pragma unroll
+        for (int m = 0; m < 16; ++m)
+#pragma unroll
+          for (int e = 0; e < 4; ++e) {
+            const float gt = (float)(bf16_t)(gacc[m][j][e] * grstd[j]);
+            gacc[m][j][e] = __builtin_amdgcn_rcpf(1.0f + __builtin_amdgcn_exp2f(gt * -1.44269504088896340736f));
+          }
+#pragma unroll
+      for (int j = 0; j < T1; ++j)
+#pragma unroll
+        for (int s8 = 0; s8 < 8; ++s8) {
+          const bf16x8 av = abf[j][s8];
+          bf16x8 gv;
+#pragma unroll
+          for (int u = 0; u < 2; ++u)
+#pragma unroll
+            for (int e = 0; e < 4; ++e) gv[4 * u + e] = (bf16_t)((float)av[4 * u + e] * gacc[2 * s8 + u][j][e]);
+          abf[j][s8] = gv;
+        }
+    } else {
     GLDS_WO(0, 0);
-    bf16x8 abf[T1A][8];
 #pragma unroll
     for (int j = 0; j < T1; ++j) {
       const int t = tok0 + 16 * (P1F + j);
@@ -154,9 +257,10 @@
 #pragma unroll
       for (int s8 = 0; s8 < 8; ++s8) abf[j][s8] = *(const __attribute__((address_space(1))) bf16x8*)(gao + aoff + s8 * 64);
     }
-    f32x4 facc[16][T1A];
     __builtin_amdgcn_s_waitcnt(0x0F70);
     __syncthreads();
+    }
+    f32x4 facc[16][T1A];
 #pragma unroll
     for (int wp = 0; wp < 4; ++wp) {
       if (wp + 1 < 4) GLDS_WO(wp + 1, (wp + 1) & 1);
@@ -535,7 +639,7 @@
 #undef GLDS_W3
 }
 
-template <int TILES, bool KEEL, bool FRONT, bool BACK>
+template <int TILES, bool KEEL, bool FRONT, bool BACK, bool GATE>
 __global__ __launch_bounds__(512, 1) void k_mlp256(MlpDev p) {
   extern __shared__ __attribute__((aligned(16))) uint4 smem[];
   uint4* const l12 = smem;
@@ -551,16 +655,16 @@
   int n_stamp = 0;
   const int tile = blockIdx.x;
   if constexpr (TILES == 9) {
-    if (wave < 4) mlp_wave<9, 2, 0, false, KEEL, FRONT, BACK>(p, l12, l3, hb, gl, tile, wave, lane, 2 * wave, 0, n_stamp);
-    else if (wave < 6) mlp_wave<9, 0, 3, false, KEEL, FRONT, BACK>(p, l12, l3, hb, gl, tile, wave, lane, 0, 3 * (wave - 4), n_stamp);
-    else if (wave == 6) mlp_wave<9, 1, 1, false, KEEL, FRONT, BACK>(p, l12, l3, hb, gl, tile, wave, lane, 8, 6, n_stamp);
-    else mlp_wave<9, 0, 2, false, KEEL, FRONT, BACK>(p, l12, l3, hb, gl, tile, wave, lane, 0, 7, n_stamp);
+    if (wave < 4) mlp_wave<9, 2, 0, false, KEEL, FRONT, BACK, GATE>(p, l12, l3, hb, gl, tile, wave, lane, 2 * wave, 0, n_stamp);
+    else if (wave < 6) mlp_wave<9, 0, 3, false, KEEL, FRONT, BACK, GATE>(p, l12, l3, hb, gl, tile, wave, lane, 0, 3 * (wave - 4), n_stamp);
+    else if (wave == 6) mlp_wave<9, 1, 1, false, KEEL, FRONT, BACK, GATE>(p, l12, l3, hb, gl, tile, wave, lane, 8, 6, n_stamp);
+    else mlp_wave<9, 0, 2, false, KEEL, FRONT, BACK, GATE>(p, l12, l3, hb, gl, tile, wave, lane, 0, 7, n_stamp);
   } else {
     constexpr int NT = TILES / 4;
     constexpr int TA = NT - NT / 2;
     const int g0 = (wave & 3) * NT;
-    if (wave < 4) mlp_wave<TILES, TA, NT - TA, false, KEEL, FRONT, BACK>(p, l12, l3, hb, gl, tile, wave, lane, g0, g0 + TA, n_stamp);
-    else mlp_wave<TILES, NT - TA, TA, false, KEEL, FRONT, BACK>(p, l12, l3, hb, gl, tile, wave, lane, g0 + TA, g0, n_stamp);
+    if (wave < 4) mlp_wave<TILES, TA, NT - TA, false, KEEL, FRONT, BACK, GATE>(p, l12, l3, hb, gl, tile, wave, lane, g0, g0 + TA, n_stamp);
+    else mlp_wave<TILES, NT - TA, TA, false, KEEL, FRONT, BACK, GATE>(p, l12, l3, hb, gl, tile, wave, lane, g0 + TA, g0, n_stamp);
   }
 }
 #undef MLP_LD12
@@ -572,7 +676,22 @@
 
 int64_t ttvk_mlp_pack_bytes(int inner, int next_qkv_rows) {
   if (inner <= 0 || inner % 32 != 0 || next_qkv_rows < 0) return 0;
+  return ttvk_mlp_pack_gate_offset(inner, next_qkv_rows) + (int64_t)MLP_WO_CHUNKS * 16;
+}
+
+int64_t ttvk_mlp_pack_gate_offset(int inner, int next_qkv_rows) {
+  if (inner <= 0 || inner % 32 != 0 || next_qkv_rows < 0) return 0;
   return ((int64_t)(inner / 32) * MLP_PANEL_CHUNKS + MLP_WO_CHUNKS + (int64_t)((next_qkv_rows + 63) / 64) * MLP_W12_CHUNKS) * 16;
+}
+
+int ttvk_mlp_pack_gate(const void* gate_folded, int next_qkv_rows, int inner, void* packed, hipStream_t s) {
+  TTV_CHECK_ARG(gate_folded && packed, "mlp_pack_gate: null buffer");
+  TTV_CHECK_ARG(inner > 0 && inner % 32 == 0 && next_qkv_rows >= 0, "mlp_pack_gate: inner %% 32");
+  TTV_CHECK_ARG(((uintptr_t)gate_folded % 16 == 0) && ((uintptr_t)packed % 16 == 0), "mlp_pack_gate: 16-byte alignment");
+  hipLaunchKernelGGL(k_mlp_pack_gate, dim3(ttv_cdiv(MLP_WO_CHUNKS, 256)), dim3(256), 0, s, (const bf16_t*)gate_folded,
+                     (uint4*)((char*)packed + ttvk_mlp_pack_gate_offset(inner, next_qkv_rows)));
+  TTV_CHECK_LAUNCH("mlp_pack_gate");
+  return TTV_OK;
 }
 
 int ttvk_mlp_pack(const void* w12_folded, const void* w3, const void* wo, const void* next_qkv_folded, int next_qkv_rows, int inner,
@@ -590,8 +709,12 @@
 }
 
 int ttvk_mlp_fused(const void* ao, int ldao, const float* front_gain, float front_alpha, const void* x, int ldx, const void* packed,
-                   int inner, void* y, int ldy, const float* post_gain, float alpha, float eps, int M, const MlpNextQkv* nq, hipStream_t s) {
+                   int inner, void* y, int ldy, const float* post_gain, float alpha, float eps, int M, const MlpNextQkv* nq, hipStream_t s,
+                   const void* gate_pack) {
   if (M == 0) return TTV_OK;
+  TTV_CHECK_ARG(!gate_pack || (ao && !nq && (uintptr_t)gate_pack % 16 == 0 && (const char*)gate_pack > (const char*)packed &&
+                              (const char*)gate_pack - (const char*)packed < ((int64_t)1 << 34)),
+                "mlp_fused: the gate needs the out_proj front, excludes the next-qkv part, and its images live in the pack");
   TTV_CHECK_ARG(x && packed && y, "mlp_fused: null buffer");
   TTV_CHECK_ARG(inner % 32 == 0 && ldx % 8 == 0 && ldy % 8 == 0 && (!ao || ldao % 8 == 0), "mlp_fused: inner %% 32, leading dims %% 8");
   TTV_CHECK_ARG(((uintptr_t)x % 16 == 0) && ((uintptr_t)packed % 16 == 0) && ((uintptr_t)y % 16 == 0) && ((uintptr_t)ao % 16 == 0),
@@ -599,6 +722,7 @@
   MlpDev d;
   d.x = (const bf16_t*)x; d.ldx = ldx; d.pack = (const uint4*)packed; d.I = inner;
   d.ao = (const bf16_t*)ao; d.ldao = ldao; d.front_gain = front_gain; d.front_alpha = front_alpha;
+  d.gate_off = gate_pack ? (int)(((const char*)gate_pack - (const char*)packed) / 16) : 0;
   d.y = (bf16_t*)y; d.ldy = ldy; d.post_gain = post_gain; d.alpha = alpha; d.eps = eps; d.M = M; d.debug = g_ttv_debug; d.stamps = g_ttv_stamps;
   d.qkv = nullptr; d.ldq = 0; d.rope_cs = nullptr; d.nqp = 0; d.rope_q_end = d.rope_k_begin = d.rope_k_end = 0;
   if (nq) {
@@ -626,21 +750,23 @@
   const int grid = d.n_tiles;
   const size_t smem = (size_t)(2 * MLP_W12_CHUNKS + 2 * MLP_W3_CHUNKS + 2 * tiles * 64) * sizeof(uint4) + 2048;
   TtvProfScope prof(TTV_KC_GEMM_GEGLU, s);
-#define LAUNCH_MLP(TILES_, KEEL_, FRONT_, BACK_)                                                                    \
+#define LAUNCH_MLP(TILES_, KEEL_, FRONT_, BACK_, GATE_)                                                             \
   do {                                                                                                              \
-    (void)hipFuncSetAttribute((const void*)k_mlp256<TILES_, KEEL_, FRONT_, BACK_>, hipFuncAttributeMaxDynamicSharedMemorySize, (int)smem); \
-    hipLaunchKernelGGL((k_mlp256<TILES_, KEEL_, FRONT_, BACK_>), dim3(grid), dim3(512), smem, s, d);                \
+    (void)hipFuncSetAttribute((const void*)k_mlp256<TILES_, KEEL_, FRONT_, BACK_, GATE_>, hipFuncAttributeMaxDynamicSharedMemorySize, (int)smem); \
+    hipLaunchKernelGGL((k_mlp256<TILES_, KEEL_, FRONT_, BACK_, GATE_>), dim3(grid), dim3(512), smem, s, d);         \
   } while (0)
 #define LAUNCH_MLP_F(TILES_, KEEL_)                                                                                 \
   do {                                                                                                              \
-    if (ao && nq) LAUNCH_MLP(TILES_, KEEL_, true, true);                                                            \
-    else if (ao) LAUNCH_MLP(TILES_, KEEL_, true, false);                                                            \
-    else LAUNCH_MLP(TILES_, KEEL_, false, false);                                                                   \
+    if (ao && nq) LAUNCH_MLP(TILES_, KEEL_, true, true, false);                                                     \
+    else if (ao && gate_pack) LAUNCH_MLP(TILES_, KEEL_, true, false, true);                                         \
+    else if (ao) LAUNCH_MLP(TILES_, KEEL_, true, false, false);                                                     \
+    else LAUNCH_MLP(TILES_, KEEL_, false, false, false);                                                            \
   } while (0)
 #define LAUNCH_MLP_9(KEEL_)                                                                                         \
   do {                                                                                                              \
-    if (ao) LAUNCH_MLP(9, KEEL_, true, false);                                                                      \
-    else LAUNCH_MLP(9, KEEL_, false, false);                                                                        \
+    if (ao && gate_pack) LAUNCH_MLP(9, KEEL_, true, false, true);                                                   \
+    else if (ao) LAUNCH_MLP(9, KEEL_, true, false, false);                                                          \
+    else LAUNCH_MLP(9, KEEL_, false, false, false);                                                                 \
   } while (0)
   TTV_CHECK_ARG(!nq || ao, "mlp_fused: the next-qkv part needs the out_proj front (ttv_layer_tail_fused)");
   if (post_gain) {
diff --git a/titok_video_amd/csrc/ttv_qkv256.inc b/titok_video_amd/csrc/ttv_qkv256.inc
--- a/titok_video_amd/csrc/ttv_qkv256.inc
+++ b/titok_video_amd/csrc/ttv_qkv256.inc
@@ -22,7 +22,7 @@
 #endif
 typedef unsigned qk_u32x4 __attribute__((ext_vector_type(4)));
 typedef unsigned qk_u32x2 __attribute__((ext_vector_type(2)));
-template <bool PRENORM>
+template <bool PRENORM, bool SKIP>
 __global__ __launch_bounds__(256, 2) void k_qkv256(GemmDev p, int n_panels, int total_items) {
   __shared__ uint4 wl[2][K256_ROWS * 32];
 
@@ -47,6 +47,7 @@
                  : "=&s"(keep__) : "v"(voff__), "s"((src_) + (size_t)(i_) * dstride), "s"((dst_) + (i_) * 1024) : "memory"); \
   } while (0)
 #define QK_PANEL_SRC(panel_) (reinterpret_cast<const char*>(p.w) + ((size_t)(panel_) * 64 + wave * 16) * (size_t)p.ldw * 2)
+#define QK_PHYS(pl_) ((SKIP && (pl_) >= p.skip_p0) ? (pl_) + p.skip_np : (pl_))
 #define QK_PANEL_DST(buf_) (wl_lds + (buf_) * (K256_ROWS * 512) + wave * (16 * 512))
 
   const int r15 = r & 15;
@@ -196,7 +197,7 @@
   do {                                                                                                       \
     const int it__ = (it_);                                                                                  \
     const int buf__ = (it__ - it0) & 1;                                                                      \
-    const int tile__ = it__ / n_panels, panel__ = it__ - tile__ * n_panels;                                  \
+    const int tile__ = it__ / n_panels, panel__ = QK_PHYS(it__ - tile__ * n_panels);                                  \
     if (tile__ != cur_tile) {                                                                                \
       cur_tile = tile__;                                                                                     \
        \
@@ -227,7 +228,7 @@
     }                                                                                                        \
     QK_STAMP(1);                                                                                             \
     const bool has_next__ = it__ + 1 < it1;                                                                  \
-    const char* nsrc__ = QK_PANEL_SRC((it__ + 1) % n_panels);                                                \
+    const char* nsrc__ = QK_PANEL_SRC(QK_PHYS((it__ + 1) % n_panels));                                                \
     const uint32_t ndst__ = QK_PANEL_DST(buf__ ^ 1);                                                         \
     const int f_first__ = panel__ * 64;                                                                      \
     const int rot__ = (f_first__ < p.rope_q_end || (f_first__ >= p.rope_k_begin && f_first__ < p.rope_k_end)) ? 2 : 1; \
@@ -257,7 +258,7 @@
   f32x16 accA[2], accB[2];
   QK_STAMP_DECL;
   {
-    const char* src0 = QK_PANEL_SRC(it0 % n_panels);
+    const char* src0 = QK_PANEL_SRC(QK_PHYS(it0 % n_panels));
     const uint32_t dst0 = QK_PANEL_DST(0);
     QK_DMA_PIECE(dchunk0, 0, src0, dst0); QK_DMA_PIECE(dchunk0, 1, src0, dst0); QK_DMA_PIECE(dchunk0, 2, src0, dst0); QK_DMA_PIECE(dchunk0, 3, src0, dst0);
     QK_DMA_PIECE(dchunk0, 4, src0, dst0); QK_DMA_PIECE(dchunk0, 5, src0, dst0); QK_DMA_PIECE(dchunk0, 6, src0, dst0); QK_DMA_PIECE(dchunk0, 7, src0, dst0);
@@ -285,6 +286,7 @@
 #undef QK_DMA_PIECE
 #undef QK_PANEL_SRC
 #undef QK_PANEL_DST
+#undef QK_PHYS
 #undef QK_AFRAG
 #undef QK_ROT
 #undef QK_PACK
diff --git a/titok_video_amd/model/base/blocks.py b/titok_video_amd/model/base/blocks.py
--- a/titok_video_amd/model/base/blocks.py
+++ b/titok_video_amd/model/base/blocks.py
@@ -360,7 +360,7 @@
             keep.append(t)
             return t.data_ptr()
 
-        def mlp_packed(w12, g, w3, wo, next_attn):
+        def mlp_packed(w12, g, w3, wo, next_attn, attn=None):
             if not fold or w3.shape[1] % 32:
                 return None, 0
             w12f = folded_tensor(w12, g)
@@ -376,6 +376,12 @@
                                                rows, inner, tower.width, _lib.TTV_BF16, out.data_ptr(), _lib.stream_ptr(device)),
                        "mlp_pack")
             keep.extend([w12f, w3c, woc, wq, out])
+            if attn is not None:
+                d = tower.width
+                wg = folded_tensor(attn.to_qkv.weight[d:2 * d], attn.pre_ln.weight)
+                _lib.check(_lib.lib().ttv_mlp_pack_gate(wg.data_ptr(), rows, inner, d, _lib.TTV_BF16, out.data_ptr(), _lib.stream_ptr(device)),
+                           "mlp_pack_gate")
+                keep.append(wg)
             return out.data_ptr(), rows
 
         perm = tower._patch_perm_on(device)
@@ -392,7 +398,7 @@
         for i in range(n):
             a, f = ml.attn_layer[i], ml.ffd_layer[i]
             pack_ptr, pack_rows = mlp_packed(f.w12.weight, f.norm.weight, f.w3.weight, a.out_proj.weight,
-                                             ml.attn_layer[i + 1] if i + 1 < n else None)
+                                             ml.attn_layer[i + 1] if i + 1 < n else None, a)
             if use_mx:
                 qkv8, qkv8s, qkvmx = f8_mx(a.to_qkv.weight, a.pre_ln.weight, q_rows=tower.width)
                 w128, w128s, w12mx = f8_mx(f.w12.weight, f.norm.weight)
@@ -411,7 +417,7 @@
                 attn_post_ln=gain(ml.attn_post_ln[i - 1].weight) if i > 0 else None,
                 ffd_post_ln=gain(ml.ffd_post_ln[i - 1].weight) if i > 0 else None,
                 to_qkv_pn=folded(a.to_qkv.weight, a.pre_ln.weight, q_rows=tower.width), w12_pn=folded(f.w12.weight, f.norm.weight),
-                mlp_pack=pack_ptr, mlp_pack_qkv_rows=pack_rows, qkv_q_prescaled=self.q_prescaled, to_qkv_qs=lin_qs(a.to_qkv.weight))
+                mlp_pack=pack_ptr, mlp_pack_qkv_rows=pack_rows, qkv_q_prescaled=self.q_prescaled | (2 if pack_ptr else 0), to_qkv_qs=lin_qs(a.to_qkv.weight))
         self.struct = _lib.TowerWeights(
             proj_in_w=lin(w_in, tower.kind == _lib.TTV_ENCODER), proj_in_b=lin(tower.proj_in.bias), mask_token=gain(tower.mask_token),
             ln_pre_t=gain(tower.ln_pre_t.weight), ln_pre_p=gain(tower.ln_pre_p.weight), ln_post=gain(tower.ln_post.weight),
```

After: 29700. 0.983x the previous value.
